# 3ickey/ConsensusML

Measured on AMD Instinct MI355X. Metric: samples/sec ResNet-50 + Krum at 1/2/4/8 MI355X; agg overhead vs all-reduce, higher is better.
Workload: dtype bf16

## Files before the change

### consensusml_amd/models/resnet.py

```python
from __future__ import annotations

from typing import List, Optional

import torch
import torch.nn as nn
import torch.nn.functional as F

from ..ops import conv as fconv
from ..ops.bn import BatchNormAct2d, ResidualLink, bn_add_bn_relu, fused_ok, link_tap
from ..ops.pool import bn_relu_max_pool2d, max_pool2d
from ..ops.stem import stem_conv_bn_relu_pool, stem_ok

from ..perf import policy as _P


def recompute_tail_policy(planes: int) -> bool:
    p = _P()
    return (p.recompute_tail and planes <= p.recompute_tail_max_planes
            and fconv.recompute_tail_ok(planes))


def fused_bn3_bwd_policy(planes: int) -> bool:
    from ..ops import conv as _c
    p = _P()
    return p.fused_bn3_bwd and planes <= p.fused_bn3_bwd_max_planes and _c.res_tail_ok(planes)


def fused_conv1x1_policy(cin: int, cout: int, hw_out: int, stride: int, prologue: bool) -> bool:
    if not _P().fused_conv1x1:
        return False
    if prologue:
        return True
    return hw_out >= 784


def conv1x1_policy(cin: int, cout: int, hw: int):
    mode = _P().conv1x1_gemm
    if mode is True or mode == "gemm":
        return True, True
    if mode is False or mode == "miopen":
        return False, False
    if cin == 64 and cout == 64 and _P().c1_dgrad64_gemm:
        return False, True
    return cin >= 1024, (cout < cin) or hw <= 196


class _Conv1x1Fn(torch.autograd.Function):

    @staticmethod
    def forward(ctx, x, w, link, fwd_gemm, dgrad_gemm, own_wgrad=False):
        ctx.save_for_backward(x, w)
        ctx.link = link
        ctx.wt = fconv.cached_wt(w)
        ctx.dgrad_gemm = dgrad_gemm
        ctx.own_wgrad = own_wgrad
        N, C, H, W = x.shape
        if fwd_gemm:
            y = fconv.conv_mm(x.permute(0, 2, 3, 1).reshape(N * H * W, C), w.reshape(w.shape[0], C))
            return y.view(N, H, W, w.shape[0]).permute(0, 3, 1, 2)
        return F.conv2d(x, w)

    @staticmethod
    def backward(ctx, dy):
        x, w = ctx.saved_tensors
        dy = dy.contiguous(memory_format=torch.channels_last)
        N, C, H, W = x.shape
        Co = w.shape[0]
        need_dx = ctx.needs_input_grad[0]
        mio_dx = need_dx and not ctx.dgrad_gemm
        own_dw = ctx.own_wgrad and ctx.needs_input_grad[1]
        mio_dw = ctx.needs_input_grad[1] and not own_dw
        dx_m, dw, h = None, None, None
        if own_dw:
            from ..ops.native import lib
            dw, h = fconv._wgrad_fork(lambda d, a, b: lib().wgrad1x1(d, a, b.dtype).view_as(b),
                                      dy, x, w, conv1x1=True)
        if mio_dx or mio_dw:
            dx_m, dw_m, _ = torch.ops.aten.convolution_backward(
                dy, x, w, None, [1, 1], [0, 0], [1, 1], False, [0, 0], 1,
                [mio_dx, mio_dw, False])
            if mio_dw:
                dw = dw_m
        dx = dx_m if mio_dx else None
        if need_dx and ctx.dgrad_gemm:
            dy2 = dy.permute(0, 2, 3, 1).reshape(N * H * W, Co)
            w2 = w.reshape(Co, C)
            link = ctx.link
            g = link.take() if link is not None else None
            if isinstance(g, fconv.MaskedGrad):
                dx = fconv.masked_link_dgrad(dy, w, g, link, ctx.wt)
                return dx, fconv._wgrad_join(dw, h), None, None, None, None
            if isinstance(g, fconv.S2Grad):
                g = g.materialize()
            w_nk = fconv.dgrad_wnk(dy2, w2, ctx.wt)
            if g is not None:
                dres = g.permute(0, 2, 3, 1).reshape(N * H * W, C) if g.dim() == 4 else g
                if dres.data_ptr() == g.data_ptr() and dres.is_contiguous():
                    d2 = fconv.conv_mm(dy2, w_nk, acc=dres)
                else:
                    d2 = torch.addmm(dres, dy2, w2)
            else:
                d2 = fconv.conv_mm(dy2, w_nk)
            dx = d2.view(N, H, W, C).permute(0, 3, 1, 2)
        return dx, fconv._wgrad_join(dw, h), None, None, None, None


_CORE = {(128, 512), (512, 128), (256, 1024), (512, 2048), (2048, 512)}
_ALL = _CORE | {(256, 128), (512, 256), (1024, 256), (1024, 512)}
_WIDE = _ALL | {(1024, 2048)}
_SETS = {"core": _CORE, "all": _ALL, "wide": _WIDE}


def own_wgrad_ok(cin: int, cout: int) -> bool:
    p = _P()
    return p.own_wgrad1x1 and (cin, cout) in _SETS[p.wgrad1x1_set]


class Conv1x1(nn.Conv2d):

    def __init__(self, cin: int, cout: int, stride: int = 1):
        super().__init__(cin, cout, 1, stride=stride, bias=False)

    def _policy(self, x: torch.Tensor):
        if not (self.stride == (1, 1) and x.is_cuda and x.dim() == 4
                and x.is_contiguous(memory_format=torch.channels_last)):
            return False, False
        return conv1x1_policy(self.in_channels, self.out_channels, x.shape[2] * x.shape[3])

    def link_ok(self, x: torch.Tensor) -> bool:
        return self._policy(x)[1]

    def forward(self, x: torch.Tensor, res_link: Optional[ResidualLink] = None) -> torch.Tensor:
        fwd_gemm, dgrad_gemm = self._policy(x)
        own = (self.stride == (1, 1) and x.is_cuda and x.dtype == torch.bfloat16
               and self.weight.dtype in (torch.bfloat16, torch.float32)
               and x.is_contiguous(memory_format=torch.channels_last)
               and own_wgrad_ok(self.in_channels, self.out_channels))
        if fwd_gemm or dgrad_gemm or own:
            return _Conv1x1Fn.apply(x, self.weight, res_link if dgrad_gemm else None, fwd_gemm,
                                    dgrad_gemm, own)
        return super().forward(x)


class _GlobalAvgPoolFn(torch.autograd.Function):

    @staticmethod
    def forward(ctx, x):
        ctx.shape = x.shape
        return torch.flatten(F.adaptive_avg_pool2d(x, 1), 1)

    @staticmethod
    def backward(ctx, g):
        N, C, H, W = ctx.shape
        if g.is_cuda and g.dtype == torch.bfloat16 and C % 8 == 0:
            from ..ops.native import lib
            return lib().avgpool_bwd(g, H, W)
        gs = (g.float() / (H * W)).to(g.dtype).contiguous()
        return torch.cat([gs] * (H * W), dim=1).view(N, H, W, C).permute(0, 3, 1, 2)


def global_avg_pool(x: torch.Tensor) -> torch.Tensor:
    if _P().nhwc_avgpool and x.is_cuda and x.dim() == 4 \
            and x.is_contiguous(memory_format=torch.channels_last):
        return _GlobalAvgPoolFn.apply(x)
    return torch.flatten(F.adaptive_avg_pool2d(x, 1), 1)


class Bottleneck(nn.Module):
    expansion = 4

    def __init__(self, inplanes: int, planes: int, stride: int = 1, downsample: bool = False):
        super().__init__()
        self.conv1 = Conv1x1(inplanes, planes)
        self.bn1 = BatchNormAct2d(planes, relu=True)
        self.conv2 = nn.Conv2d(planes, planes, 3, stride=stride, padding=1, bias=False)
        self.bn2 = BatchNormAct2d(planes, relu=True)
        self.conv3 = Conv1x1(planes, planes * 4)
        self.bn3 = BatchNormAct2d(planes * 4, relu=True)
        if downsample:
            self.down_conv = Conv1x1(inplanes, planes * 4, stride=stride)
            self.down_bn = BatchNormAct2d(planes * 4, relu=False)
        else:
            self.down_conv = None

    def _conv2(self, x: torch.Tensor) -> torch.Tensor:
        if _P().own_dgrad3x3 and self.training:
            return fconv.conv3x3(x, self.conv2)
        return self.conv2(x)

    def _down_s2_compact_ok(self, x: torch.Tensor, dlink) -> bool:
        c = self.down_conv
        return (dlink is not None and _P().down_s2_compact and c.stride == (2, 2)
                and x.is_cuda and x.dtype == torch.bfloat16 and x.shape[1] % 8 == 0
                and x.shape[2] % 2 == 0 and x.shape[3] % 2 == 0
                and x.is_contiguous(memory_format=torch.channels_last))

    def _down_conv_s2_compact(self, x: torch.Tensor, dlink) -> torch.Tensor:
        c = self.down_conv
        xs = fconv.subsample2_link(x, dlink)
        fwd, dg = conv1x1_policy(c.in_channels, c.out_channels, xs.shape[2] * xs.shape[3])
        return _Conv1x1Fn.apply(xs, c.weight, None, fwd, dg,
                                own_wgrad_ok(c.in_channels, c.out_channels))

    def _fused_ok(self, x: torch.Tensor) -> bool:
        return (_P().fused_conv1x1 and self.training and torch.is_grad_enabled()
                and fconv.fused_conv_ok(x, self.conv1.weight)
                and fused_ok(x, self.bn3.weight))

    def _conv_bn(self, x, conv: "Conv1x1", bn, link=None):
        st = conv.stride[0]
        hw = (x.shape[2] // st) * (x.shape[3] // st)
        if fused_conv1x1_policy(conv.in_channels, conv.out_channels, hw, st, False):
            dg = st == 1 and conv1x1_policy(conv.in_channels, conv.out_channels, hw)[1]
            own = own_wgrad_ok(conv.in_channels, conv.out_channels) if st == 1 else True
            z, m, i = fconv.conv1x1_bn_stats(x, conv, bn, st, dg, own, link if dg else None)
            return z, (m, i)
        if st == 1:
            return conv(x, res_link=link if conv.link_ok(x) else None), None
        return conv(x), None

    def _tap(self, x: torch.Tensor, dlink, use_links: bool) -> torch.Tensor:
        tlink = dlink if dlink is not None else \
            (getattr(x, "_cml_pool_link", None) if use_links else None)
        return link_tap(x, tlink) if tlink is not None else x

    def _head(self, x: torch.Tensor, use_links: bool):
        link = dlink = None
        if self.down_conv is None:
            link = getattr(x, "_cml_link", None) if use_links else None
        elif use_links and self.conv1.link_ok(x):
            dlink = ResidualLink()
        z1, st1 = self._conv_bn(x, self.conv1, self.bn1, link if dlink is None else dlink)
        return z1, st1, link, dlink

    def _conv2_fused(self, z1: torch.Tensor, st1, fuse3: bool):
        pol = _P()
        s1 = self.conv2.stride == (1, 1)
        on = (pol.conv3x3_bn_stats and pol.own_dgrad3x3) if s1 else pol.own_conv3x3_s2
        own3 = fuse3 and on and fconv.conv3x3_ok(z1, self.conv2)
        pro = (own3 and pol.bn1_dgrad_sums and self.bn1.training
               and fused_ok(z1, self.bn1.weight))
        if pro and s1 and st1 is None and pol.bn1_sums_lib_conv1:
            st1 = fconv.bn_stats(z1, self.bn1)
        if pro and st1 is not None:
            return fconv.bnrelu_conv3x3_bn_stats(z1, self.bn1, st1, self.conv2, self.bn2)
        out = self.bn1(z1, stats=st1)
        if own3:
            return fconv.conv3x3_bn_stats(out, self.conv2, self.bn2)
        z2 = self._conv2(out)
        return z2, (fconv.bn_stats(z2, self.bn2) if fuse3 else None)

    def _tail_fused(self, x, z2, st2, fuse3: bool, hw2: int, link, dlink, use_links: bool,
                    out_link) -> torch.Tensor:
        planes = self.conv3.in_channels
        down = self.down_conv
        if not fuse3:
            z, st3 = self.conv3(self.bn2(z2)), None
        else:
            if down is None:
                rec = recompute_tail_policy(planes)
                if rec or fused_bn3_bwd_policy(planes):
                    tail = fconv.bnrelu_conv1x1_bn_res_recompute if rec \
                        else fconv.bnrelu_conv1x1_bn_res
                    return tail(z2, self.bn2, st2, self.conv3, self.bn3, x, link, out_link)
            elif _P().recompute_down_tail and self.bn3.eps == self.down_bn.eps:
                xd = None
                if fconv.down_tail_recompute_s2_ok(x, planes, down):
                    xd = fconv.subsample2_link(x, dlink)
                elif fconv.down_tail_recompute_ok(x, planes, down):
                    xd = self._tap(x, dlink, use_links)
                if xd is not None:
                    return fconv.down_tail_recompute(z2, self.bn2, st2, self.conv3, self.bn3, xd,
                                                     down, self.down_bn, out_link)
            dg = conv1x1_policy(planes, planes * 4, hw2)[1]
            z, m3, i3 = fconv.bnrelu_conv1x1_bn_stats(z2, self.bn2, st2, self.conv3, self.bn3, dg,
                                                      own_wgrad_ok(planes, planes * 4)
                                                      or planes == 64)
            st3 = (m3, i3)
        if down is None:
            return self.bn3(z, residual=x, res_link=link, out_link=out_link, stats=st3)
        if self._down_s2_compact_ok(x, dlink):
            zd, std = self._down_conv_s2_compact(x, dlink), None
        else:
            zd, std = self._conv_bn(self._tap(x, dlink, use_links), down, self.down_bn)
        if (st3 is None) != (std is None):
            return self.bn3(z, residual=self.down_bn(zd, stats=std), out_link=out_link, stats=st3)
        stats = None if st3 is None else st3 + std
        return bn_add_bn_relu(z, self.bn3, zd, self.down_bn, out_link, stats=stats)

    def _forward_fused(self, x: torch.Tensor, use_links: bool) -> torch.Tensor:
        z1, st1, link, dlink = self._head(x, use_links)
        planes, s = self.conv3.in_channels, self.conv2.stride[0]
        hw2 = (z1.shape[2] // s) * (z1.shape[3] // s)
        fuse3 = fused_conv1x1_policy(planes, planes * 4, hw2, 1, True)
        z2, st2 = self._conv2_fused(z1, st1, fuse3)
        out_link = ResidualLink() if use_links else None
        y = self._tail_fused(x, z2, st2, fuse3, hw2, link, dlink, use_links, out_link)
        if out_link is not None:
            y._cml_link = out_link
        return y

    def forward(self, x: torch.Tensor) -> torch.Tensor:
        use_links = _P().residual_link and torch.is_grad_enabled() and self.training
        if self._fused_ok(x):
            return self._forward_fused(x, use_links)
        if self.down_conv is None:
            link = getattr(x, "_cml_link", None) if use_links else None
            out = self.bn1(self.conv1(x, res_link=link if self.conv1.link_ok(x) else None))
            out = self.bn2(self._conv2(out))
            z = self.conv3(out)
            fused = fused_ok(z, self.bn3.weight)
            out_link = ResidualLink() if use_links and fused else None
            y = self.bn3(z, residual=x, res_link=link if fused else None, out_link=out_link)
        else:
            dlink = ResidualLink() if use_links and self.conv1.link_ok(x) else None
            out = self.bn1(self.conv1(x, res_link=dlink))
            out = self.bn2(self._conv2(out))
            z = self.conv3(out)
            zd = self.down_conv(self._tap(x, dlink, use_links))
            out_link = ResidualLink() if use_links and fused_ok(z, self.bn3.weight) else None
            y = bn_add_bn_relu(z, self.bn3, zd, self.down_bn, out_link) if _P().fuse_down_bn \
                else self.bn3(z, residual=self.down_bn(zd), out_link=out_link)
        if out_link is not None:
            y._cml_link = out_link
        return y


class ResNet(nn.Module):
    def __init__(self, layers: List[int], num_classes: int = 1000, width: int = 64):
        super().__init__()
        self.inplanes = width
        self.conv1 = nn.Conv2d(3, width, 7, stride=2, padding=3, bias=False)
        self.bn1 = BatchNormAct2d(width, relu=True)
        self.layer1 = self._make(width, layers[0], 1)
        self.layer2 = self._make(width * 2, layers[1], 2)
        self.layer3 = self._make(width * 4, layers[2], 2)
        self.layer4 = self._make(width * 8, layers[3], 2)
        self.fc = nn.Linear(width * 8 * 4, num_classes)
        for m in self.modules():
            if isinstance(m, nn.Conv2d):
                nn.init.kaiming_normal_(m.weight, mode="fan_out", nonlinearity="relu")
        for m in self.modules():
            if isinstance(m, Bottleneck):
                nn.init.zeros_(m.bn3.weight)

    def stem(self, x: torch.Tensor) -> torch.Tensor:
        w = self.conv1.weight
        if (_P().stem_pad4 and x.is_cuda and x.dtype == torch.bfloat16 and x.shape[1] == 3
                and x.is_contiguous(memory_format=torch.channels_last) and not x.requires_grad):
            from ..ops.native import lib
            x4 = lib().pad_c4(x)
            w4 = F.pad(w, (0, 0, 0, 0, 0, 1)).contiguous(memory_format=torch.channels_last)
            return F.conv2d(x4, w4, stride=2, padding=3)
        return self.conv1(x)

    def _make(self, planes: int, blocks: int, stride: int) -> nn.Sequential:
        down = stride != 1 or self.inplanes != planes * 4
        mods = [Bottleneck(self.inplanes, planes, stride, down)]
        self.inplanes = planes * 4
        mods += [Bottleneck(self.inplanes, planes) for _ in range(1, blocks)]
        return nn.Sequential(*mods)

    def forward(self, x: torch.Tensor) -> torch.Tensor:
        pol = _P()
        if pol.fuse_stem_conv and stem_ok(x, self.conv1, self.bn1):
            plink = ResidualLink() if (pol.pool_link and pol.residual_link and self.training
                                       and torch.is_grad_enabled()) else None
            x = stem_conv_bn_relu_pool(x, self.conv1, self.bn1, plink)
            if plink is not None:
                x._cml_pool_link = plink
        elif pol.fuse_stem_pool:
            x = bn_relu_max_pool2d(self.stem(x), self.bn1, 3, 2, 1)
        else:
            x = max_pool2d(self.bn1(self.stem(x)), 3, 2, 1)
        blocks = [b for layer in (self.layer1, self.layer2, self.layer3, self.layer4)
                  for b in layer]
        ws = [b.conv2.weight for b in blocks] + [b.conv1.weight for b in blocks]
        batched = (pol.batch_wlayouts and self.training and torch.is_grad_enabled()
                   and not fconv.params_pending(self, ws) and fconv.prefetch_wlayouts(ws))
        try:
            x = self.layer4(self.layer3(self.layer2(self.layer1(x))))
        finally:
            if batched:
                fconv.clear_wlayouts()
        return self.fc(global_avg_pool(x))


def resnet50(num_classes: int = 1000) -> ResNet:
    return ResNet([3, 4, 6, 3], num_classes)


def resnet_tiny(num_classes: int = 10) -> ResNet:
    return ResNet([1, 1, 1, 1], num_classes, width=8)
```

### consensusml_amd/ops/bn.py

```python
from __future__ import annotations

from typing import Optional

import torch
import torch.nn as nn
import torch.nn.functional as F

from ..perf import policy as _P
from .native import lib


class ResidualLink:
    __slots__ = ("grad", "closed", "bn_ctx", "sums")

    def __init__(self):
        self.grad = None
        self.closed = False
        self.bn_ctx = None
        self.sums = None

    def take(self):
        g, self.grad = self.grad, None
        self.closed = True
        return g

    def take_tensor(self):
        g = self.take()
        return g.materialize() if hasattr(g, "materialize") else g


class MaskedGrad:
    __slots__ = ("g", "mask")

    def __init__(self, g: torch.Tensor, mask: torch.Tensor):
        self.g = g
        self.mask = mask

    def materialize(self) -> torch.Tensor:
        g = self.g
        N, C, H, W = g.shape
        shifts = torch.arange(8, device=g.device, dtype=torch.uint8)
        bits = (self.mask.view(-1, C // 8, 1) >> shifts) & 1
        rows = g.permute(0, 2, 3, 1).reshape(-1, C) * bits.view(-1, C).to(g.dtype)
        return rows.view(N, H, W, C).permute(0, 3, 1, 2)


TAP_STATS = {"parked": 0, "fallback": 0}


class _LinkTapFn(torch.autograd.Function):

    @staticmethod
    def forward(ctx, x, link):
        ctx.link = link
        return x.view_as(x)

    @staticmethod
    def backward(ctx, g):
        link = ctx.link
        if link.closed or link.grad is not None:
            TAP_STATS["fallback"] += 1
            return g, None
        TAP_STATS["parked"] += 1
        link.grad = g.contiguous(memory_format=torch.channels_last) if g.dim() == 4 else g.contiguous()
        return None, None


def link_tap(x: torch.Tensor, link: "ResidualLink") -> torch.Tensor:
    return _LinkTapFn.apply(x, link)


class _BNActFn(torch.autograd.Function):
    @staticmethod
    def forward(ctx, x, gamma, beta, res, rmean, rvar, mean_in, invstd_in, eps, momentum, relu,
                training, res_link, out_link):
        has_res = res is not None
        want_mask = has_res and relu and any(ctx.needs_input_grad[:4])
        y, mean, invstd, mask = lib().bn_fwd(x, res, gamma, beta, rmean, rvar, mean_in,
                                             invstd_in, eps, momentum, relu, training, want_mask)
        ctx.save_for_backward(x, mask if want_mask else None, gamma, beta, mean, invstd)
        ctx.relu = relu
        ctx.has_res = has_res
        ctx.res_link = res_link
        ctx.out_link = out_link
        return y

    @staticmethod
    def backward(ctx, dy):
        x, mask, gamma, beta, mean, invstd = ctx.saved_tensors
        dy2 = ctx.out_link.take_tensor() if ctx.out_link is not None else None
        dx, dg, db, dres = lib().bn_bwd(dy, dy2, x, mask, gamma, beta, mean, invstd, ctx.relu,
                                        ctx.has_res)
        if ctx.has_res and ctx.res_link is not None:
            ctx.res_link.grad = dres
            dres = None
        return (dx, dg, db, dres if ctx.has_res else None, None, None, None, None, None, None,
                None, None, None, None)


class _BNAddBNActFn(torch.autograd.Function):

    @staticmethod
    def forward(ctx, x1, g1, b1, x2, g2, b2, rm1, rv1, rm2, rv2, stats_in, eps, momentum,
                training, out_link):
        want_mask = any(ctx.needs_input_grad[:6])
        m1 = i1 = m2 = i2 = None
        if not training:
            m1, i1, m2, i2 = stats_in
        y, m1, i1, m2, i2, mask = lib().bn_fwd2(x1, x2, g1, b1, g2, b2, rm1, rv1, rm2, rv2, m1,
                                                i1, m2, i2, eps, momentum, training, want_mask)
        ctx.save_for_backward(x1, x2, mask if want_mask else None, g1, g2, m1, i1, m2, i2)
        ctx.out_link = out_link
        return y

    @staticmethod
    def backward(ctx, dy):
        x1, x2, mask, g1, g2, m1, i1, m2, i2 = ctx.saved_tensors
        dy2 = ctx.out_link.take_tensor() if ctx.out_link is not None else None
        dx1, dg1, db1, dx2, dg2, db2 = lib().bn_bwd2(dy, dy2, x1, x2, mask, g1, g2, m1, i1, m2, i2)
        return (dx1, dg1, db1, dx2, dg2, db2) + (None,) * 9


def bn_add_bn_relu(x1: torch.Tensor, bn1: "BatchNormAct2d", x2: torch.Tensor,
                   bn2: "BatchNormAct2d", out_link: Optional[ResidualLink] = None,
                   stats: Optional[tuple] = None) -> torch.Tensor:
    if (_fused_ok(x1, bn1.weight) and _fused_ok(x2, bn2.weight) and x1.shape == x2.shape
            and not bn2.relu and bn1.relu and bn1.eps == bn2.eps and bn1.momentum == bn2.momentum):
        if stats is not None and bn1.training:
            return _BNAddBNActFn.apply(x1, bn1.weight, bn1.bias, x2, bn2.weight, bn2.bias, None,
                                       None, None, None, tuple(stats), bn1.eps, bn1.momentum,
                                       False, out_link)
        stats = None
        if not bn1.training:
            stats = (bn1.running_mean.float(), torch.rsqrt(bn1.running_var.float() + bn1.eps),
                     bn2.running_mean.float(), torch.rsqrt(bn2.running_var.float() + bn2.eps))
        return _BNAddBNActFn.apply(x1, bn1.weight, bn1.bias, x2, bn2.weight, bn2.bias,
                                   bn1.running_mean if bn1.training else None,
                                   bn1.running_var if bn1.training else None,
                                   bn2.running_mean if bn2.training else None,
                                   bn2.running_var if bn2.training else None, stats, bn1.eps,
                                   bn1.momentum, bn1.training, out_link)
    return bn1(x1, residual=bn2(x2), out_link=out_link)


def fused_ok(x: torch.Tensor, gamma: torch.Tensor) -> bool:
    return _fused_ok(x, gamma)


def _fused_ok(x: torch.Tensor, gamma: torch.Tensor) -> bool:
    if not (x.is_cuda and x.dtype == torch.bfloat16 and gamma.dtype == torch.bfloat16):
        return False
    if not _P().fused_bn:
        return False
    C = x.shape[1]
    if C % 8 or C > 2048 or 256 % (C // 8):
        return False
    return x.dim() == 4 and x.is_contiguous(memory_format=torch.channels_last)


def bn_act(x: torch.Tensor, gamma: torch.Tensor, beta: torch.Tensor,
           running_mean: Optional[torch.Tensor], running_var: Optional[torch.Tensor],
           residual: Optional[torch.Tensor] = None, relu: bool = True, training: bool = True,
           momentum: float = 0.1, eps: float = 1e-5,
           res_link: Optional[ResidualLink] = None,
           out_link: Optional[ResidualLink] = None,
           stats: Optional[tuple] = None) -> torch.Tensor:
    if _fused_ok(x, gamma) and (residual is None or residual.is_contiguous(
            memory_format=torch.channels_last)):
        if training and stats is not None:
            return _BNActFn.apply(x, gamma, beta, residual, None, None, stats[0], stats[1], eps,
                                  momentum, relu, False, res_link, out_link)
        if training:
            return _BNActFn.apply(x, gamma, beta, residual, running_mean, running_var, None, None,
                                  eps, momentum, relu, True, res_link, out_link)
        invstd = torch.rsqrt(running_var.float() + eps)
        return _BNActFn.apply(x, gamma, beta, residual, None, None, running_mean.float(), invstd,
                              eps, momentum, relu, False, res_link, out_link)
    y = F.batch_norm(x, running_mean, running_var, gamma, beta, training, momentum, eps) \
        if running_mean is None or running_mean.dtype == x.dtype else \
        _bn_mixed(x, gamma, beta, running_mean, running_var, training, momentum, eps)
    if residual is not None:
# ... 42 lines not shown
```

### consensusml_amd/ops/conv.py

```python
from __future__ import annotations

import weakref
from typing import Optional, Tuple, Dict

import torch
import torch.nn.functional as F

from ..perf import policy as _P
from .bn import MaskedGrad
from .native import lib


def fused_conv_ok(x: torch.Tensor, w: torch.Tensor) -> bool:
    return (x.is_cuda and x.dtype == torch.bfloat16 and w.dtype == torch.bfloat16 and x.dim() == 4
            and x.is_contiguous(memory_format=torch.channels_last) and x.shape[1] % 64 == 0
            and w.shape[0] % 64 == 0 and w.shape[2] == 1 and w.shape[3] == 1)


def _nt_tile(a: torch.Tensor, M: int, N: int, K: int) -> int:
    if not (_P().own_gemm_conv1x1 and a.is_cuda and a.dtype == torch.bfloat16):
        return 0
    try:
        t = int(lib().gemm_nt_pick(M, N, K))
    except Exception:
        return 0
    if t == 256:
        return 256 if (M // 256) * (N // 256) >= 128 else 0
    return 128 if t == 128 and _P().own_gemm128 else 0


CONV_MM_STATS = {"own": 0, "own128": 0, "blas": 0}


def dgrad_wnk(a: torch.Tensor, w2: torch.Tensor, wt: Optional[torch.Tensor]) -> torch.Tensor:
    if wt is not None and _nt_tile(a, a.shape[0], w2.shape[1], w2.shape[0]):
        return wt
    return w2.t()


def conv_mm(a: torch.Tensor, w_nk: torch.Tensor, acc: Optional[torch.Tensor] = None) -> torch.Tensor:
    M, K = a.shape
    N = w_nk.shape[0]
    tile = _nt_tile(a, M, N, K)
    if (tile and a.is_contiguous() and a.data_ptr() % 16 == 0
            and (acc is None or (acc.is_contiguous() and acc.data_ptr() % 16 == 0))):
        w = (lib().transpose_bf16(w_nk.t()) if (w_nk.stride(0) == 1 and w_nk.dim() == 2)
             else w_nk.contiguous())
        CONV_MM_STATS["own"] += 1
        if tile == 128:
            CONV_MM_STATS["own128"] += 1
        if acc is not None:
            return lib().gemm_nt(a, w, 0, out=acc, cin=acc, tile=tile)
        return lib().gemm_nt(a, w, 0, tile=tile)
    CONV_MM_STATS["blas"] += 1
    if acc is not None:
        return acc.addmm_(a, w_nk.t()) if acc.is_contiguous() else torch.addmm(acc, a, w_nk.t())
    return torch.mm(a, w_nk.t())


def _dgrad(dy: torch.Tensor, x: torch.Tensor, w: torch.Tensor, stride: int, gemm: bool,
           link, wt: Optional[torch.Tensor] = None) -> torch.Tensor:
    N, C, H, W = x.shape
    Co = w.shape[0]
    if gemm and stride == 1:
        dy2 = dy.permute(0, 2, 3, 1).reshape(N * H * W, Co)
        w2 = w.reshape(Co, C)
        g = link.take() if link is not None else None
        if isinstance(g, MaskedGrad):
            return masked_link_dgrad(dy, w, g, link, wt)
        if isinstance(g, S2Grad):
            if (_P().s2_link_dgrad and dy.dtype == torch.bfloat16 and C % 64 == 0 and Co % 64 == 0
                    and g.H == H and g.W == W):
                if wt is None:
                    wt = w.reshape(Co, C).t().contiguous()
                return lib().conv1x1_link_s2(dy.contiguous(memory_format=torch.channels_last), wt,
                                             g.g)
            g = g.materialize()
        w_nk = dgrad_wnk(dy2, w2, wt)
        if (g is not None and g.dim() == 4 and _P().link_dgrad_plain and dy.dtype == torch.bfloat16
                and g.dtype == torch.bfloat16 and C % 64 == 0 and Co % 64 == 0
                and g.is_contiguous(memory_format=torch.channels_last)
                and not _nt_tile(dy2, N * H * W, C, Co)):
            wt2 = wt if wt is not None else w2.t().contiguous()
            return lib().conv1x1_link(dy.contiguous(memory_format=torch.channels_last), wt2, g,
                                      None)[0]
        if g is not None:
            dres = g.permute(0, 2, 3, 1).reshape(N * H * W, C) if g.dim() == 4 else g
            if dres.data_ptr() == g.data_ptr() and dres.is_contiguous():
                d2 = conv_mm(dy2, w_nk, acc=dres)
            else:
                d2 = torch.addmm(dres, dy2, w2)
        else:
            d2 = conv_mm(dy2, w_nk)
        return d2.view(N, H, W, C).permute(0, 3, 1, 2)
    dx, _, _ = torch.ops.aten.convolution_backward(
        dy, x, w, None, [stride, stride], [0, 0], [1, 1], False, [0, 0], 1, [True, False, False])
    return dx


def masked_link_dgrad(dy: torch.Tensor, w: torch.Tensor, mg: MaskedGrad, link,
                      wt: Optional[torch.Tensor] = None) -> torch.Tensor:
    Co, Ci = w.shape[0], w.shape[1]
    if wt is None:
        wt = w.reshape(Co, Ci).t().contiguous()
    bctx = link.bn_ctx if link is not None else None
    if bctx is not None:
        z, mask, mean, invstd = bctx
        dx, sdz, sdzx = lib().conv1x1_link(dy, wt, mg.g, mg.mask, z, mask, mean, invstd)
        link.sums = (sdz, sdzx, dx.data_ptr())
        return dx
    return lib().conv1x1_link(dy, wt, mg.g, mg.mask)[0]


def _wgrad(dy: torch.Tensor, x: torch.Tensor, w: torch.Tensor, stride: int, own: bool,
           pro: Optional[Tuple[torch.Tensor, torch.Tensor]] = None) -> torch.Tensor:
    if own and stride == 1:
        sc, bi = pro if pro is not None else (None, None)
        return lib().wgrad1x1(dy, x, w.dtype, sc, bi).view_as(w)
    if pro is not None:
        sc, bi = pro
        x = torch.relu(x.float() * sc.view(1, -1, 1, 1) + bi.view(1, -1, 1, 1)).to(x.dtype)
        x = x.contiguous(memory_format=torch.channels_last)
    N, Ci, H, W = x.shape
    if (own and stride == 2 and _P().own_wgrad1x1_s2 and x.is_cuda
            and dy.dtype == torch.bfloat16 and x.dtype == torch.bfloat16
            and x.is_contiguous(memory_format=torch.channels_last)
            and lib().wgrad3x3s2_ok(N, H, W, dy.shape[1], Ci, 1)):
        return lib().wgrad3x3s2(dy, x, w.dtype, _zero_row(dy.device), taps=1).reshape(w.shape)
    _, dw, _ = torch.ops.aten.convolution_backward(
        dy, x, w, None, [stride, stride], [0, 0], [1, 1], False, [0, 0], 1, [False, True, False])
    return dw


class _Conv1x1BNStatsFn(torch.autograd.Function):
    @staticmethod
    def forward(ctx, x, w, rmean, rvar, stride, eps, momentum, dgrad_gemm, own_wgrad, link,
                aff=None):
        out = lib().conv1x1_bn_fwd(x, w, None, None, rmean, rmean, rvar, stride, True, eps,
                                   momentum, *(aff or (None, None)))
        y, mean, invstd = out[:3]
        if aff is not None:
            _stash_affine(mean, out[3], out[4], aff)
        ctx.wt = cached_wt(w)
        ctx.save_for_backward(x, w)
        ctx.stride, ctx.dgrad_gemm, ctx.own_wgrad, ctx.link = stride, dgrad_gemm, own_wgrad, link
        ctx.mark_non_differentiable(mean, invstd)
        ctx.set_materialize_grads(False)
        return y, mean, invstd

    @staticmethod
    def backward(ctx, dy, _dm, _di):
        x, w = ctx.saved_tensors
        dy = dy.contiguous(memory_format=torch.channels_last)
        dw, h = _wgrad_fork(lambda d, a, b: _wgrad(d, a, b, ctx.stride, ctx.own_wgrad), dy, x, w,
                            conv1x1=True) if ctx.needs_input_grad[1] else (None, None)
        dx = _dgrad(dy, x, w, ctx.stride, ctx.dgrad_gemm, ctx.link, ctx.wt) \
            if ctx.needs_input_grad[0] else None
        dw = _wgrad_join(dw, h)
        return dx, dw, None, None, None, None, None, None, None, None, None


class _BNReLUConv1x1BNStatsFn(torch.autograd.Function):

    @staticmethod
    def forward(ctx, z, gamma, beta, mean, invstd, w, rmean, rvar, eps, momentum, dgrad_gemm,
                own_wgrad):
        sc, bi = _affine(gamma, beta, mean, invstd)
        y, m3, i3 = lib().conv1x1_bn_fwd(z, w, sc, bi, rmean, rmean, rvar, 1, True, eps, momentum)
        ctx.save_for_backward(z, gamma, beta, mean, invstd, w, sc, bi)
        ctx.dgrad_gemm, ctx.own_wgrad = dgrad_gemm, own_wgrad
        ctx.mark_non_differentiable(m3, i3)
        ctx.set_materialize_grads(False)
        return y, m3, i3

    @staticmethod
    def backward(ctx, dz3, _dm, _di):
        z, gamma, beta, mean, invstd, w, sc, bi = ctx.saved_tensors
        dz3 = dz3.contiguous(memory_format=torch.channels_last)
        dw = _wgrad(dz3, z, w, 1, ctx.own_wgrad, (sc, bi)) if ctx.needs_input_grad[5] else None
        dy2 = _dgrad(dz3, z, w, 1, ctx.dgrad_gemm, None)
        dz, dg, db, _ = lib().bn_bwd(dy2, None, z, None, gamma, beta, mean, invstd, True, False)
        return dz, dg, db, None, None, dw, None, None, None, None, None, None


def _take_out_link(ol, gy: torch.Tensor):
    gy = gy.contiguous(memory_format=torch.channels_last)
    sums = None
    if ol is not None:
        extra = ol.take_tensor()
        if ol.sums is not None and extra is None and ol.sums[2] == gy.data_ptr():
            sums = ol.sums
        ol.sums = ol.bn_ctx = None
        if extra is not None:
            gy = (gy + extra).contiguous(memory_format=torch.channels_last)
    return gy, sums


def _park_masked(gy: torch.Tensor, mask: torch.Tensor, res_link) -> Optional[torch.Tensor]:
    mg = MaskedGrad(gy, mask)
    if res_link is not None and not res_link.closed and res_link.grad is None:
        res_link.grad = mg
        return None
    return mg.materialize()


class _BNReLUConv1x1BNResFn(torch.autograd.Function):

    @staticmethod
    def forward(ctx, z, g2, b2, mean2, invstd2, w, g3, b3, res, rmean3, rvar3, eps, momentum,
                res_link, out_link):
        sc, bi = _affine(g2, b2, mean2, invstd2)
        z3, m3, i3 = lib().conv1x1_bn_fwd(z, w, sc, bi, rmean3, rmean3, rvar3, 1, True, eps,
                                          momentum)
        y, _, _, mask = lib().bn_fwd(z3, res, g3, b3, None, None, m3, i3, eps, momentum, True,
                                     False, True)
        ctx.save_for_backward(z, g2, b2, mean2, invstd2, w, sc, bi, z3, mask, g3, b3, m3, i3)
        ctx.res_link, ctx.out_link = res_link, out_link
        if out_link is not None:
            out_link.bn_ctx = (z3, mask, m3, i3)
        return y

    @staticmethod
    def backward(ctx, gy):
        z, g2, b2, mean2, invstd2, w, sc, bi, z3, mask, g3, b3, m3, i3 = ctx.saved_tensors
        gy, sums = _take_out_link(ctx.out_link, gy)
        M = gy.numel() // gy.shape[1]
        if sums is None:
            sums = lib().bn_bwd_sums(gy, None, z3, mask, g3, b3, m3, i3, True)
        ca, cb, cc, dg3, db3 = lib().bn_bwd_coeffs(sums[0], sums[1], g3, m3, i3, M)
        Co, Ci = w.shape[0], w.shape[1]
        dw = None
        if ctx.needs_input_grad[5]:
            dw = lib().wgrad1x1(gy, z, w.dtype, sc, bi, z3, mask, ca, cb, cc).view_as(w)
        dy2 = lib().conv1x1_bnbwd(gy, z3, mask, ca, cb, cc, w.reshape(Co, Ci).t().contiguous())
        dz, dg2, db2, _ = lib().bn_bwd(dy2, None, z, None, g2, b2, mean2, invstd2, True, False)
        dres = _park_masked(gy, mask, ctx.res_link) if ctx.needs_input_grad[8] else None
        return (dz, dg2, db2, None, None, dw, dg3, db3, dres) + (None,) * 6


def _fin_aff(bn):
    g, b = bn.weight, bn.bias
    if (_P().fin_affine and _P().bn_affine_kernel and g is not None and b is not None
            and g.dtype == torch.bfloat16 and b.dtype == torch.bfloat16
            and g.is_contiguous() and b.is_contiguous()):
        return g, b
    return None


def _stash_affine(mean: torch.Tensor, sc: torch.Tensor, bi: torch.Tensor, aff) -> None:
    g, b = aff
    mean._cml_affine = (sc, bi, g.data_ptr(), b.data_ptr(), g._version, b._version)


def _cached_affine(gamma: torch.Tensor, beta: torch.Tensor, mean: torch.Tensor):
    a = getattr(mean, "_cml_affine", None)
    if (a is not None and a[2] == gamma.data_ptr() and a[3] == beta.data_ptr()
            and a[4] == gamma._version and a[5] == beta._version):
        return a[0], a[1]
    return None


def _affine(gamma: torch.Tensor, beta: torch.Tensor, mean: torch.Tensor, invstd: torch.Tensor):
    a = _cached_affine(gamma, beta, mean)
    if a is not None:
        return a
    if not _P().bn_affine_kernel:
        sc = gamma.float() * invstd
        return sc, beta.float() - mean * sc
    ab = lib().bn_affine(gamma, beta, mean, invstd)
    return ab[0], ab[1]


def _stats_gram_affine(L, gram, cy, w, M, rmean, rvar, eps, momentum, gamma, beta):
    if _P().bn_affine_kernel:
        m, i, sc, bi = L.bn_stats_gram(gram, cy, w, M, rmean, rvar, eps, momentum, gamma, beta)
        return m, i, sc, bi
    m, i = L.bn_stats_gram(gram, cy, w, M, rmean, rvar, eps, momentum)
    return (m, i) + _affine(gamma, beta, m, i)


_CONST = {}


def _const(n: int, v: float, device) -> torch.Tensor:
    key = (n, v, device)
    t = _CONST.get(key)
    if t is None:
        t = _CONST[key] = torch.full((n,), v, dtype=torch.float32, device=device)
    return t




def scaled_cat(w1: torch.Tensor, s1: torch.Tensor, w2: torch.Tensor, s2: torch.Tensor):
    k1 = w1.shape[1]
    out = torch.empty(w1.shape[0], k1 + w2.shape[1], dtype=torch.bfloat16, device=w1.device)
    torch.mul(w1, s1[:, None], out=out[:, :k1])
    torch.mul(w2, s2[:, None], out=out[:, k1:])
    return out


def fold_cat(w1: torch.Tensor, a: torch.Tensor, c: torch.Tensor, w2: torch.Tensor):
    w_cat = torch.cat([w1 * a[None, :], w2], 1).to(torch.bfloat16).contiguous()
    return w_cat, torch.mv(w1, c)


def _own_dgb(gamma: torch.Tensor, beta: torch.Tensor) -> bool:
    return (_P().fin_dgamma and gamma.dtype == torch.bfloat16 and beta.dtype == torch.bfloat16
            and gamma.is_contiguous() and beta.is_contiguous())


def _cat_dgrad_bn2(L, gy, mask, z, sc, bi, w_cat, bias, g2, b2, mean2, invstd2):
# ... 244 lines not shown
_ZERO_ROWS = {}


def _zero_row(device: torch.device) -> torch.Tensor:
    z = _ZERO_ROWS.get(device)
    if z is None:
        z = _ZERO_ROWS[device] = torch.zeros(256, dtype=torch.bfloat16, device=device)
    return z


_SIDE_STREAMS: Dict[torch.device, "torch.cuda.Stream"] = {}


def _wgrad_fork(fn, *args, conv1x1: bool = False):
    dev = args[0].device
    pol = _P()
    if not (pol.side_wgrad and dev.type == "cuda" and args[0].shape[0] >= pol.side_wgrad_min_batch
            and (pol.side_wgrad_1x1 or not conv1x1)):
        return fn(*args), None
    side = _SIDE_STREAMS.get(dev)
    if side is None:
        side = _SIDE_STREAMS[dev] = torch.cuda.Stream(device=dev)
    main = torch.cuda.current_stream(dev)
    side.wait_stream(main)
    with torch.cuda.stream(side):
        dw = fn(*args)
    return dw, (main, side)


def _wgrad_join(dw: Optional[torch.Tensor], handle) -> Optional[torch.Tensor]:
    if handle is None:
        return dw
    main, side = handle
    main.wait_stream(side)
    if dw is not None:
        dw.record_stream(main)
    return dw




def _wgrad3x3(dy: torch.Tensor, x: torch.Tensor, w: torch.Tensor) -> torch.Tensor:
    N, Ci, H, W = x.shape
    Co = dy.shape[1]
    if _P().own_wgrad3x3 and lib().wgrad3x3_direct_ok(N, H, W, Co, Ci):
        return lib().wgrad3x3(dy, x, w.dtype, _zero_row(dy.device))
    return torch.ops.aten.convolution_backward(
        dy, x, w, None, [1, 1], [1, 1], [1, 1], False, [0, 0], 1, [False, True, False])[1]


_WL_BATCH = {}


def prefetch_wlayouts(ws) -> bool:
    ws = [w for w in ws if w.is_cuda and w.dtype == torch.bfloat16 and w.dim() == 4
          and w.shape[2] == w.shape[3] and w.shape[2] in (1, 3)]
    if len(ws) < 2:
        return False
    for w, (wf, wr) in zip(ws, lib().conv_wlayouts_multi(ws)):
        _WL_BATCH[id(w)] = (w, wf, wr)
    return True


def clear_wlayouts() -> None:
    _WL_BATCH.clear()


_PENDING_QUERY = weakref.WeakKeyDictionary()


def set_pending_query(model: torch.nn.Module, query) -> None:
    if query is None:
        _PENDING_QUERY.pop(model, None)
    else:
        _PENDING_QUERY[model] = weakref.WeakMethod(query)


def params_pending(model: torch.nn.Module, params) -> bool:
    ref = _PENDING_QUERY.get(model)
    query = ref() if ref is not None else None
    return query is not None and query(params)


def cached_wt(w: torch.Tensor) -> Optional[torch.Tensor]:
    e = _WL_BATCH.get(id(w))
    return e[2] if e is not None and e[0] is w and w.shape[2] == 1 else None


def _w3x3_layouts(w: torch.Tensor, want_wf: bool):
    e = _WL_BATCH.get(id(w))
    if e is not None and e[0] is w:
        return (e[1] if want_wf else None), e[2]
    if w.is_cuda and w.dtype == torch.bfloat16:
        wf, wr = lib().conv3x3_wlayouts(w, want_wf)
        return wf, wr
    Co, Ci = w.shape[0], w.shape[1]
    wf = w.permute(0, 2, 3, 1).reshape(Co, 9 * Ci).contiguous() if want_wf else None
    return wf, w.flip(2, 3).permute(1, 2, 3, 0).reshape(Ci, 9 * Co).contiguous()


class _Conv3x3Fn(torch.autograd.Function):

    @staticmethod
    def forward(ctx, x, w):
        ctx.save_for_backward(x, w)
        return F.conv2d(x, w, padding=1)

    @staticmethod
    def backward(ctx, dy):
        x, w = ctx.saved_tensors
        dy = dy.contiguous(memory_format=torch.channels_last)
        dgrad, wgrad = _BWD3X3[getattr(ctx, "stride", 1)]
        dx = dw = None
        if ctx.needs_input_grad[0]:
            wr = getattr(ctx, "wr", None)
            if wr is None:
                wr = _w3x3_layouts(w, False)[1]
            dx = dgrad(dy, wr)[0]
        if ctx.needs_input_grad[1]:
            dw = wgrad(dy, x, w)
        return dx, dw


class _Conv3x3BNStatsFn(torch.autograd.Function):

    @staticmethod
    def forward(ctx, x, w, rmean, rvar, eps, momentum, stride=1, aff=None):
        wf, wr = _w3x3_layouts(w, True)
        y, mean, invstd = _conv_gemm_bn(x, wf, rmean, rvar, eps, momentum, stride, aff)
        ctx.save_for_backward(x, w)
        ctx.wr, ctx.stride = wr, stride
        ctx.mark_non_differentiable(mean, invstd)
        ctx.set_materialize_grads(False)
        return y, mean, invstd

    @staticmethod
    def backward(ctx, dy, _dm, _di):
        dx, dw = _Conv3x3Fn.backward(ctx, dy)
        return dx, dw, None, None, None, None, None, None


def _conv_gemm_bn(x, wf, rmean, rvar, eps, momentum, stride, aff):
    out = lib().conv_gemm_bn(x, wf, 9, _zero_row(x.device), rmean, rmean, rvar, eps, momentum,
                             stride, *(aff or (None, None)))
    if aff is not None:
        _stash_affine(out[1], out[3], out[4], aff)
    return out[0], out[1], out[2]


class _BNReLUConv3x3BNStatsFn(torch.autograd.Function):

    @staticmethod
    def forward(ctx, z1, g1, b1, mean1, invstd1, eps1, w, rmean, rvar, eps, momentum, stride=1,
                aff=None):
        L = lib()
        y1 = L.bn_fwd(z1, None, g1, b1, None, None, mean1, invstd1, eps1, momentum, True, False,
                      False)[0]
        wf, wr = _w3x3_layouts(w, True)
        z2, m2, i2 = _conv_gemm_bn(y1, wf, rmean, rvar, eps, momentum, stride, aff)
        ctx.save_for_backward(z1, g1, b1, mean1, invstd1, y1, w)
        ctx.wr, ctx.stride = wr, stride
        ctx.aff1 = _cached_affine(g1, b1, mean1)
        ctx.mark_non_differentiable(m2, i2)
        ctx.set_materialize_grads(False)
        return z2, m2, i2

    @staticmethod
    def backward(ctx, dz2, _dm, _di):
        z1, g1, b1, mean1, invstd1, y1, w = ctx.saved_tensors
        dz2 = dz2.contiguous(memory_format=torch.channels_last)
        L = lib()
        dgrad, wgrad = _BWD3X3[ctx.stride]
        dw, h = _wgrad_fork(wgrad, dz2, y1, w) if ctx.needs_input_grad[6] else (None, None)
        sc, bi = ctx.aff1 or _affine(g1, b1, mean1, invstd1)
        bn1 = (z1, sc, bi, mean1, invstd1)
        if _own_dgb(g1, b1):
            dg1, db1 = torch.empty_like(g1), torch.empty_like(b1)
            dy1, s1, q1 = dgrad(dz2, ctx.wr, *bn1, dg1, db1)
        else:
            dy1, s1, q1 = dgrad(dz2, ctx.wr, *bn1)
            M = z1.numel() // z1.shape[1]
            _, _, _, dg1, db1 = L.bn_bwd_coeffs(s1, q1, g1, mean1, invstd1, M)
        dz1 = L.bn_bwd_apply(dy1, z1, g1, b1, mean1, invstd1, s1, q1)
        dw = _wgrad_join(dw, h)
        return dz1, dg1, db1, None, None, None, dw, None, None, None, None, None, None


def _wgrad3x3_s2(dy: torch.Tensor, x: torch.Tensor, w: torch.Tensor) -> torch.Tensor:
    N, Ci, H, W = x.shape
    if (_P().own_wgrad3x3_s2 and Ci >= _P().wgrad3x3_s2_min_ci and x.is_cuda
            and dy.dtype == torch.bfloat16
            and x.dtype == torch.bfloat16
            and lib().wgrad3x3s2_ok(N, H, W, dy.shape[1], Ci)):
        return lib().wgrad3x3s2(dy, x.contiguous(memory_format=torch.channels_last), w.dtype,
                                _zero_row(dy.device))
    return torch.ops.aten.convolution_backward(
        dy, x, w, None, [2, 2], [1, 1], [1, 1], False, [0, 0], 1, [False, True, False])[1]


def _dgrad3x3(dy: torch.Tensor, wr: torch.Tensor, *bn):
    if bn:
        return lib().conv_gemm_bnsums(dy, wr, 9, _zero_row(dy.device), *bn)
    return (lib().conv_gemm(dy, wr, 9, _zero_row(dy.device)),)


def _dgrad3x3_s2(dy: torch.Tensor, wr: torch.Tensor, *bn):
    return lib().conv_gemm_s2dgrad(dy, wr, _zero_row(dy.device), *bn)


_BWD3X3 = {1: (_dgrad3x3, _wgrad3x3), 2: (_dgrad3x3_s2, _wgrad3x3_s2)}




def bnrelu_conv3x3_bn_stats(z1: torch.Tensor, bn_a, stats_a, conv, bn):
    z, m, i = _BNReLUConv3x3BNStatsFn.apply(z1, bn_a.weight, bn_a.bias, stats_a[0], stats_a[1],
                                            bn_a.eps, conv.weight, bn.running_mean, bn.running_var,
                                            bn.eps, bn.momentum, conv.stride[0], _fin_aff(bn))
    return z, (m, i)


def conv3x3_bn_stats(x: torch.Tensor, conv, bn):
    z, m, i = _Conv3x3BNStatsFn.apply(x, conv.weight, bn.running_mean, bn.running_var, bn.eps,
                                      bn.momentum, conv.stride[0], _fin_aff(bn))
    return z, (m, i)


def conv3x3_ok(x: torch.Tensor, conv) -> bool:
    return (x.is_cuda and x.dtype == torch.bfloat16 and conv.weight.dtype == torch.bfloat16
            and x.dim() == 4 and x.is_contiguous(memory_format=torch.channels_last)
            and conv.kernel_size == (3, 3) and conv.padding == (1, 1)
            and (conv.stride == (1, 1) or (conv.stride == (2, 2) and x.shape[2] % 2 == 0
                                           and x.shape[3] % 2 == 0))
            and conv.dilation == (1, 1) and conv.groups == 1 and conv.bias is None
            and conv.in_channels % 64 == 0 and conv.out_channels % 64 == 0)


def conv3x3(x: torch.Tensor, conv) -> torch.Tensor:
    if conv.stride == (1, 1) and conv3x3_ok(x, conv) and torch.is_grad_enabled():
        return _Conv3x3Fn.apply(x, conv.weight)
    return conv(x)


def conv1x1_bn_stats(x: torch.Tensor, conv, bn, stride: int = 1, dgrad_gemm: bool = False,
                     own_wgrad: bool = False, link=None):
    return _Conv1x1BNStatsFn.apply(x, conv.weight, bn.running_mean, bn.running_var, stride,
                                   bn.eps, bn.momentum, dgrad_gemm, own_wgrad, link, _fin_aff(bn))


def bnrelu_conv1x1_bn_stats(z: torch.Tensor, bn_a, stats_a, conv, bn_b, dgrad_gemm: bool = False,
                            own_wgrad: bool = True):
    mean, invstd = stats_a
    return _BNReLUConv1x1BNStatsFn.apply(z, bn_a.weight, bn_a.bias, mean, invstd, conv.weight,
                                         bn_b.running_mean, bn_b.running_var, bn_b.eps,
                                         bn_b.momentum, dgrad_gemm, own_wgrad)


def bn_stats(z: torch.Tensor, bn) -> Tuple[torch.Tensor, torch.Tensor]:
    return tuple(lib().bn_stats(z, bn.running_mean, bn.running_var, bn.eps, bn.momentum))


def reference_conv1x1_bn(x: torch.Tensor, w: torch.Tensor, stride: int = 1,
                         pro: Optional[Tuple[torch.Tensor, torch.Tensor]] = None):
    xf = x.float()
    if pro is not None:
        xf = torch.relu(xf * pro[0].view(1, -1, 1, 1) + pro[1].view(1, -1, 1, 1))
        xf = xf.to(torch.bfloat16).float()
    y = F.conv2d(xf, w.float(), stride=stride)
    yb = y.to(torch.bfloat16).float()
    return y, yb.mean((0, 2, 3)), yb.var((0, 2, 3), unbiased=False)
```

### consensusml_amd/perf.py

```python
from __future__ import annotations

import contextlib
import dataclasses
import os
from dataclasses import dataclass, fields
from typing import Any, Dict, Iterator


def _env_bool(name: str, default: bool) -> bool:
    v = os.environ.get(name)
    return default if v is None else v == "1"


def _env_int(name: str, default: int) -> int:
    v = os.environ.get(name)
    return default if v is None else int(v)


def _env_str(name: str, default: str) -> str:
    return os.environ.get(name, default)


@dataclass
class PerfPolicy:
    fused_bn: bool = True
    residual_link: bool = True
    fuse_stem_conv: bool = True
    fuse_stem_pool: bool = True
    pool_link: bool = True
    stem_pool_gather: bool = True
    stem_pad4: bool = True
    nhwc_avgpool: bool = True
    conv1x1_gemm: str = "auto"
    fused_conv1x1: bool = True
    conv1x1g: str = "auto"
    own_wgrad1x1: bool = True
    wgrad1x1_set: str = "wide"
    fused_bn3_bwd: bool = True
    fused_bn3_bwd_max_planes: int = 128
    recompute_tail: bool = True
    recompute_tail_max_planes: int = 256
    recompute_down_tail: bool = True
    recompute_down_tail_s2: bool = True
    down_tail_s2_max_cin: int = 512
    fuse_down_bn: bool = True
    gram_stats: bool = True
    cat_bnsums: bool = True
    cat_bnsums_maxc: int = 256
    s2_link_dgrad: bool = True
    down_s2_compact: bool = True
    bn_affine_kernel: bool = True
    own_dgrad3x3: bool = True
    conv3x3_bn_stats: bool = True
    bn1_dgrad_sums: bool = True
    bn1_sums_lib_conv1: bool = False
    own_wgrad3x3: bool = True
    own_wgrad3x3_s2: bool = True
    wgrad3x3_s2_min_ci: int = 256
    own_wgrad1x1_s2: bool = True
    c1_dgrad64_gemm: bool = True
    own_conv3x3_s2: bool = True
    side_wgrad: bool = True
    side_wgrad_min_batch: int = 1024
    link_dgrad_plain: bool = True
    side_wgrad_1x1: bool = False
    fin_dgamma: bool = True
    fin_affine: bool = True
    batch_wlayouts: bool = True
    attn_kernel: bool = True
    flash_attn: bool = True
    multi_copy: bool = True
    batched_workers: bool = True
    own_gemm: bool = True
    own_gemm128: bool = True
    fused_ffn: bool = True
    padded_logits: bool = True
    own_gemm_conv1x1: bool = True
    nt_wgrad: bool = True
    own_linear_wgrad: bool = True

    @classmethod
    def from_env(cls) -> "PerfPolicy":
        return cls(
            fused_bn=_env_bool("CML_FUSED_BN", True),
            fuse_stem_conv=_env_bool("CML_FUSE_STEM_CONV", True),
            fuse_stem_pool=_env_bool("CML_FUSE_STEM_POOL", True),
            pool_link=_env_bool("CML_POOL_LINK", True),
            stem_pool_gather=_env_bool("CML_STEM_POOL_GATHER", True),
            stem_pad4=_env_bool("CML_STEM_PAD4", True),
            nhwc_avgpool=_env_bool("CML_NHWC_AVGPOOL", True),
            conv1x1_gemm=_env_str("CML_CONV1X1_GEMM", "auto"),
            fused_conv1x1=_env_bool("CML_FUSED_CONV1X1", True),
            conv1x1g={"0": "regstage", "3": "quad"}.get(os.environ.get("CML_C1G", ""), "auto"),
            own_wgrad1x1=_env_bool("CML_WGRAD1X1", True),
            wgrad1x1_set=_env_str("CML_WGRAD1X1_SET", "wide"),
            fused_bn3_bwd=_env_bool("CML_FUSED_BN3_BWD", True),
            fused_bn3_bwd_max_planes=_env_int("CML_FUSED_BN3_BWD_MAX_PLANES", 128),
            recompute_tail=_env_bool("CML_RECOMPUTE_TAIL", True),
            recompute_tail_max_planes=_env_int("CML_RECOMPUTE_TAIL_MAX_PLANES", 256),
            recompute_down_tail=_env_bool("CML_RECOMPUTE_DOWN_TAIL", True),
            recompute_down_tail_s2=_env_bool("CML_RECOMPUTE_DOWN_TAIL_S2", True),
            down_tail_s2_max_cin=_env_int("CML_DOWN_TAIL_S2_MAX_CIN", 512),
            fuse_down_bn=_env_bool("CML_FUSE_DOWN_BN", True),
            gram_stats=_env_bool("CML_GRAM_STATS", True),
            cat_bnsums=_env_bool("CML_CAT_BNSUMS", True),
            cat_bnsums_maxc=_env_int("CML_CAT_BNSUMS_MAXC", 256),
            s2_link_dgrad=_env_bool("CML_S2_LINK_DGRAD", True),
            down_s2_compact=_env_bool("CML_DOWN_S2_COMPACT", True),
            bn_affine_kernel=_env_bool("CML_BN_AFFINE_KERNEL", True),
            own_dgrad3x3=_env_bool("CML_DGRAD3X3", True),
            conv3x3_bn_stats=_env_bool("CML_CONV3X3_BN_STATS", True),
            bn1_dgrad_sums=_env_bool("CML_BN1_DGRAD_SUMS", True),
            bn1_sums_lib_conv1=_env_bool("CML_BN1_SUMS_LIB_CONV1", False),
            own_wgrad3x3=_env_bool("CML_WGRAD3X3", True),
            own_wgrad3x3_s2=_env_bool("CML_WGRAD3X3_S2", True),
            wgrad3x3_s2_min_ci=int(os.environ.get("CML_WGRAD3X3_S2_MIN_CI", "256")),
            own_wgrad1x1_s2=_env_bool("CML_WGRAD1X1_S2", True),
            c1_dgrad64_gemm=_env_bool("CML_C1_DGRAD64", True),
            own_conv3x3_s2=_env_bool("CML_CONV3X3_S2", True),
            side_wgrad=_env_bool("CML_SIDE_WGRAD", True),
            side_wgrad_min_batch=_env_int("CML_SIDE_WGRAD_MIN_BATCH", 1024),
            side_wgrad_1x1=_env_bool("CML_SIDE_WGRAD_1X1", False),
            link_dgrad_plain=_env_bool("CML_LINK_DGRAD_PLAIN", True),
            fin_dgamma=_env_bool("CML_FIN_DGAMMA", True),
            fin_affine=_env_bool("CML_FIN_AFFINE", True),
            batch_wlayouts=_env_bool("CML_BATCH_WLAYOUTS", True),
            attn_kernel=_env_bool("CML_ATTN_KERNEL", True),
            flash_attn=_env_bool("CML_FLASH_ATTN", True),
            multi_copy=_env_bool("CML_MULTI_COPY", True),
            batched_workers=_env_bool("CML_BATCHED_WORKERS", True),
            own_gemm=_env_bool("CML_OWN_GEMM", True),
            own_gemm128=_env_bool("CML_OWN_GEMM128", True),
            fused_ffn=_env_bool("CML_FUSED_FFN", True),
            own_gemm_conv1x1=_env_bool("CML_OWN_GEMM_CONV1X1", True),
            own_linear_wgrad=_env_bool("CML_OWN_LINEAR_WGRAD", True),
            nt_wgrad=_env_bool("CML_NT_WGRAD", True),
            padded_logits=_env_bool("CML_PADDED_LOGITS", True),
        )

    @classmethod
    def library(cls) -> "PerfPolicy":
        off: Dict[str, Any] = {}
        for f in fields(cls):
            if f.type in ("bool", bool):
                off[f.name] = False
        off.update(conv1x1_gemm="miopen", conv1x1g="regstage")
        return cls(**off)

    def replace(self, **kw) -> "PerfPolicy":
        return dataclasses.replace(self, **kw)

    def to_dict(self) -> Dict[str, Any]:
        return dataclasses.asdict(self)

    def validate(self) -> "PerfPolicy":
        if self.conv1x1_gemm not in ("auto", "gemm", "miopen"):
            raise ValueError(f"conv1x1_gemm must be auto | gemm | miopen, not {self.conv1x1_gemm!r}")
        if self.conv1x1g not in ("auto", "quad", "regstage"):
            raise ValueError(f"conv1x1g must be auto | quad | regstage, not "
                             f"{self.conv1x1g!r}")
        if self.wgrad1x1_set not in ("core", "all", "wide"):
            raise ValueError(f"wgrad1x1_set must be core | all | wide, not "
                             f"{self.wgrad1x1_set!r}")
        return self


_CURRENT = PerfPolicy.from_env().validate()
_NATIVE_SYNCED = None


def env_switches() -> Dict[str, str]:
    return {k: v for k, v in sorted(os.environ.items())
            if k.startswith("CML_") and not k.startswith("CML_BENCH_")}


def policy() -> PerfPolicy:
    return _CURRENT


def _sync_native(p: PerfPolicy) -> None:
    global _NATIVE_SYNCED
    mode = {"regstage": 0, "auto": 2, "quad": 3}[p.conv1x1g]
    if _NATIVE_SYNCED == mode:
        return
    try:
        from .ops.native import lib
        L = lib()
    except Exception:
        return
    L.set_conv1x1g_mode(mode)
    _NATIVE_SYNCED = mode


def set_policy(p: PerfPolicy) -> PerfPolicy:
    global _CURRENT
    prev = _CURRENT
    _CURRENT = p.validate()
    if prev.conv1x1g != p.conv1x1g or _NATIVE_SYNCED is not None:
        _sync_native(p)
    return prev


def ensure_native_synced() -> None:
    _sync_native(_CURRENT)


@contextlib.contextmanager
def use_policy(p: PerfPolicy) -> Iterator[PerfPolicy]:
    prev = set_policy(p)
    try:
        yield p
    finally:
        set_policy(prev)
```

### csrc/bindings.cpp

```cpp
#include <torch/extension.h>
#include <array>
#include <climits>
#include <ATen/hip/HIPContext.h>
#include <c10/core/DeviceGuard.h>

#include "kernels/kernels.h"

namespace {

using at::Tensor;
using c10::optional;

#define CML_CHECK_HIP(expr)                                                               \
  do {                                                                                    \
    hipError_t _e = (expr);                                                               \
    TORCH_CHECK(_e == hipSuccess, "consensusml_amd HIP error: ", hipGetErrorString(_e), " at " \
                #expr " (bindings.cpp:", __LINE__, ")");                                  \
  } while (0)

hipStream_t cur_stream() { return c10::hip::getCurrentHIPStream().stream(); }

int dtype_of(const Tensor& t) {
  if (t.scalar_type() == at::kBFloat16) return cml::DT_BF16;
  TORCH_CHECK(t.scalar_type() == at::kFloat, "expected bf16 or fp32 tensor, got ", t.scalar_type());
// ... 1093 lines not shown
                              M, static_cast<int>(K), static_cast<int>(Co), pro))}, f32);
  CML_CHECK_HIP(cml::launch_conv1x1_bn_fwd(
      x.data_ptr(), w.data_ptr(), nullptr, part.data_ptr<float>(),
      opt_ptr<const float>(pro_sc, at::kFloat, "pro_sc", K),
      opt_ptr<const float>(pro_bi, at::kFloat, "pro_bi", K),
      opt_ptr<const float>(shift, at::kFloat, "shift", Co), M, static_cast<int>(K),
      static_cast<int>(Co), 1, 0, 0, mean.data_ptr<float>(), invstd.data_ptr<float>(),
      opt_ptr<float>(rmean, at::kFloat, "running_mean", Co),
      opt_ptr<float>(rvar, at::kFloat, "running_var", Co), static_cast<float>(eps),
      static_cast<float>(momentum), cur_stream()));
  return {mean, invstd};
}

std::vector<Tensor> conv1x1_bnres(const Tensor& x, const Tensor& w, const Tensor& pro_sc,
                                  const Tensor& pro_bi, const Tensor& ep_sc, const Tensor& ep_bi,
                                  const Tensor& res) {
  check_nhwc(x, "x");
  check_nhwc(res, "res");
  TORCH_CHECK(x.dim() == 4 && w.scalar_type() == at::kBFloat16 && w.dim() == 4 && w.size(2) == 1 &&
                  w.size(3) == 1 && w.size(1) == x.size(1) && w.is_contiguous(),
              "conv1x1_bnres: x NHWC, w contiguous bf16 [Cout, Cin, 1, 1]");
  const int64_t N = x.size(0), K = x.size(1), H = x.size(2), W = x.size(3), Co = w.size(0);
  const int64_t M = N * H * W;
  TORCH_CHECK(res.dim() == 4 && res.size(0) == N && res.size(1) == Co && res.size(2) == H &&
                  res.size(3) == W, "conv1x1_bnres: res shape");
  TORCH_CHECK(K % 64 == 0 && Co % 64 == 0, "conv1x1_bnres: channels multiples of 64");
  const c10::DeviceGuard guard(x.device());
  Tensor y = at::empty({N, Co, H, W}, x.options().memory_format(at::MemoryFormat::ChannelsLast));
  Tensor mask = at::empty({M, Co / 8}, x.options().dtype(at::kByte));
  CML_CHECK_HIP(cml::launch_conv1x1_bnres(
      x.data_ptr(), w.data_ptr(), y.data_ptr(), mask.data_ptr<uint8_t>(),
      opt_ptr<const float>(pro_sc, at::kFloat, "pro_sc", K),
      opt_ptr<const float>(pro_bi, at::kFloat, "pro_bi", K),
      opt_ptr<const float>(ep_sc, at::kFloat, "ep_sc", Co),
      opt_ptr<const float>(ep_bi, at::kFloat, "ep_bi", Co), res.data_ptr(), M,
      static_cast<int>(K), static_cast<int>(Co), cur_stream()));
  return {y, mask};
}

namespace {
std::array<int64_t, 8> cat_shape(const Tensor& x1, const Tensor& x2, const Tensor& w,
                                 const char* what) {
  check_nhwc(x1, "x1");
  check_nhwc(x2, "x2");
  const int64_t N = x1.size(0), K1 = x1.size(1), H = x1.size(2), W = x1.size(3), K2 = x2.size(1);
  TORCH_CHECK(x2.dim() == 4 && x2.size(0) == N && x2.size(2) == H && x2.size(3) == W, what,
              ": x2 shape");
  TORCH_CHECK(w.is_cuda() && w.scalar_type() == at::kBFloat16 && w.dim() == 2 &&
                  w.size(1) == K1 + K2 && w.is_contiguous() && w.size(0) % 64 == 0 &&
                  K1 % 64 == 0 && K2 % 64 == 0,
              what, ": w contiguous bf16 [Cout, K1 + K2], channels multiples of 64");
  return {N, K1, H, W, K2, N * H * W, K1 + K2, w.size(0)};
}
}

std::vector<Tensor> conv1x1_cat_bnres(const Tensor& x1, const Tensor& x2, const Tensor& sc1,
                                      const Tensor& bi1, const optional<Tensor>& sc2,
                                      const optional<Tensor>& bi2, const Tensor& w,
                                      const Tensor& ep_sc, const Tensor& ep_bi) {
  const auto [N, K1, H, W, K2, M, K, Co] = cat_shape(x1, x2, w, "conv1x1_cat_bnres");
  const c10::DeviceGuard guard(x1.device());
  Tensor y = at::empty({N, Co, H, W}, x1.options().memory_format(at::MemoryFormat::ChannelsLast));
  Tensor mask = at::empty({M, Co / 8}, x1.options().dtype(at::kByte));
  CML_CHECK_HIP(cml::launch_conv1x1_cat_bnres(
      x1.data_ptr(), x2.data_ptr(), opt_ptr<const float>(sc1, at::kFloat, "sc1", K1),
      opt_ptr<const float>(bi1, at::kFloat, "bi1", K1),
      opt_ptr<const float>(sc2, at::kFloat, "sc2", K2),
      opt_ptr<const float>(bi2, at::kFloat, "bi2", K2), w.data_ptr(),
      opt_ptr<const float>(ep_sc, at::kFloat, "ep_sc", Co),
      opt_ptr<const float>(ep_bi, at::kFloat, "ep_bi", Co), nullptr, y.data_ptr(),
      mask.data_ptr<uint8_t>(), M, static_cast<int>(K1), static_cast<int>(K),
      static_cast<int>(Co), cur_stream()));
  return {y, mask};
}

Tensor conv1x1_cat(const Tensor& g, const Tensor& mask, const Tensor& x2,
                   const optional<Tensor>& sc2, const optional<Tensor>& bi2, const Tensor& w,
                   const optional<Tensor>& bias) {
  const auto [N, K1, H, W, K2, M, K, Co] = cat_shape(g, x2, w, "conv1x1_cat");
  const c10::DeviceGuard guard(g.device());
  Tensor y = at::empty({N, Co, H, W}, g.options().memory_format(at::MemoryFormat::ChannelsLast));
  CML_CHECK_HIP(cml::launch_conv1x1_cat(
      g.data_ptr(), opt_ptr<const uint8_t>(mask, at::kByte, "mask", M * K1 / 8), x2.data_ptr(),
      opt_ptr<const float>(sc2, at::kFloat, "sc2", K2),
      opt_ptr<const float>(bi2, at::kFloat, "bi2", K2),
      opt_ptr<const float>(bias, at::kFloat, "bias", Co), w.data_ptr(), y.data_ptr(), M,
      static_cast<int>(K1), static_cast<int>(K), static_cast<int>(Co), cur_stream()));
  return y;
}

std::vector<Tensor> conv1x1_cat_bnsums(const Tensor& g, const Tensor& mask, const Tensor& x2,
                                       const Tensor& sc2, const Tensor& bi2, const Tensor& w,
                                       const optional<Tensor>& bias, const Tensor& mean,
                                       const Tensor& invstd, const optional<Tensor>& dgamma_out,
                                       const optional<Tensor>& dbeta_out) {
  const auto [N, K1, H, W, K2, M, K, Co] = cat_shape(g, x2, w, "conv1x1_cat_bnsums");
  TORCH_CHECK(Co == K2, "conv1x1_cat_bnsums: w must be [K2, K1 + K2]");
  const c10::DeviceGuard guard(g.device());
  auto f32 = g.options().dtype(at::kFloat);
  Tensor y = at::empty({N, Co, H, W}, g.options().memory_format(at::MemoryFormat::ChannelsLast));
  Tensor part = at::empty({static_cast<int64_t>(cml::conv1x1_cat_part_floats(M, K, Co))}, f32);
  Tensor sdz = at::empty({Co}, f32), sdzx = at::empty({Co}, f32);
  const auto [dg, db] = dgb_ptrs(dgamma_out, dbeta_out, Co, g, "conv1x1_cat_bnsums");
  CML_CHECK_HIP(cml::launch_conv1x1_cat(
      g.data_ptr(), opt_ptr<const uint8_t>(mask, at::kByte, "mask", M * K1 / 8), x2.data_ptr(),
      opt_ptr<const float>(sc2, at::kFloat, "sc2", K2),
      opt_ptr<const float>(bi2, at::kFloat, "bi2", K2),
      opt_ptr<const float>(bias, at::kFloat, "bias", Co), w.data_ptr(), y.data_ptr(), M,
      static_cast<int>(K1), static_cast<int>(K), static_cast<int>(Co), cur_stream(),
      opt_ptr<const float>(mean, at::kFloat, "mean", Co),
      opt_ptr<const float>(invstd, at::kFloat, "invstd", Co), part.data_ptr<float>(),
      sdz.data_ptr<float>(), sdzx.data_ptr<float>(), dg, db));
  return {y, sdz, sdzx};
}

Tensor bn_affine(const Tensor& gamma, const Tensor& beta, const Tensor& mean, const Tensor& invstd) {
  const int64_t C = gamma.numel();
  TORCH_CHECK(gamma.scalar_type() == at::kBFloat16 && beta.scalar_type() == at::kBFloat16 &&
                  gamma.is_contiguous() && beta.is_contiguous() && beta.numel() == C && C > 0,
              "bn_affine: contiguous bf16 gamma / beta [C]");
  check_dev(gamma, "gamma");
  check_dev(beta, "beta");
  const c10::DeviceGuard guard(gamma.device());
  Tensor out = at::empty({2, C}, gamma.options().dtype(at::kFloat));
  CML_CHECK_HIP(cml::launch_bn_affine(gamma.data_ptr(), beta.data_ptr(),
                                      opt_ptr<const float>(mean, at::kFloat, "mean", C),
                                      opt_ptr<const float>(invstd, at::kFloat, "invstd", C),
                                      static_cast<int>(C), out.data_ptr<float>(),
                                      out.data_ptr<float>() + C, cur_stream()));
  return out;
}

Tensor bn_bwd_apply(const Tensor& dy_in, const Tensor& x, const Tensor& gamma, const Tensor& beta,
                    const Tensor& mean, const Tensor& invstd, const Tensor& sdz,
                    const Tensor& sdzx) {
  check_nhwc(x, "x");
  Tensor dy = x.dim() == 4 ? dy_in.contiguous(at::MemoryFormat::ChannelsLast) : dy_in.contiguous();
  check_nhwc(dy, "dy");
  TORCH_CHECK(dy.sizes() == x.sizes(), "bn_bwd_apply: dy shape mismatch");
  const int64_t C = x.size(1);
  const int64_t M = x.numel() / C;
  TORCH_CHECK(gamma.scalar_type() == at::kBFloat16 && beta.scalar_type() == at::kBFloat16 &&
                  gamma.numel() == C && beta.numel() == C,
              "bn_bwd_apply: bf16 gamma / beta [C]");
  const c10::DeviceGuard guard(x.device());
  Tensor dx = at::empty_like(x);
  CML_CHECK_HIP(cml::launch_bn_bwd_apply(
      dy.data_ptr(), x.data_ptr(), dx.data_ptr(), M, static_cast<int>(C), gamma.data_ptr(),
      beta.data_ptr(), opt_ptr<const float>(mean, at::kFloat, "mean", C),
      opt_ptr<const float>(invstd, at::kFloat, "invstd", C),
      opt_ptr<const float>(sdz, at::kFloat, "sdz", C),
      opt_ptr<const float>(sdzx, at::kFloat, "sdzx", C), cur_stream()));
  return dx;
}

Tensor conv1x1_link_s2(const Tensor& x, const Tensor& w, const Tensor& link_in) {
  check_nhwc(x, "x");
  TORCH_CHECK(x.dim() == 4, "conv1x1_link_s2: 4-D NHWC input");
  const int64_t N = x.size(0), K = x.size(1), H = x.size(2), W = x.size(3);
  check_w2(w, K, "conv1x1_link_s2");
  const int64_t No = w.size(0);
  Tensor link = link_in.contiguous(at::MemoryFormat::ChannelsLast);
  check_nhwc(link, "link");
  TORCH_CHECK(link.dim() == 4 && link.size(0) == N && link.size(1) == No &&
                  link.size(2) == (H + 1) / 2 && link.size(3) == (W + 1) / 2,
              "conv1x1_link_s2: link [N, No, ceil(H/2), ceil(W/2)]");
  const c10::DeviceGuard guard(x.device());
  Tensor y = at::empty({N, No, H, W}, x.options().memory_format(at::MemoryFormat::ChannelsLast));
  CML_CHECK_HIP(cml::launch_conv1x1_link_s2(x.data_ptr(), w.data_ptr(), y.data_ptr(),
                                            link.data_ptr(), static_cast<int>(N),
                                            static_cast<int>(H), static_cast<int>(W),
                                            static_cast<int>(K), static_cast<int>(No),
                                            cur_stream()));
  return y;
}

Tensor subsample2(const Tensor& x) {
  check_nhwc(x, "x");
  TORCH_CHECK(x.dim() == 4 && x.size(1) % 8 == 0, "subsample2: 4-D NHWC, C % 8 == 0");
  const int64_t N = x.size(0), C = x.size(1), H = x.size(2), W = x.size(3);
  const c10::DeviceGuard guard(x.device());
  Tensor y = at::empty({N, C, (H + 1) / 2, (W + 1) / 2},
                       x.options().memory_format(at::MemoryFormat::ChannelsLast));
  CML_CHECK_HIP(cml::launch_subsample2(x.data_ptr(), y.data_ptr(), static_cast<int>(N),
                                       static_cast<int>(H), static_cast<int>(W),
                                       static_cast<int>(C), cur_stream()));
  return y;
}

Tensor upsample2_scatter(const Tensor& g_in, int64_t H, int64_t W) {
  Tensor g = g_in.contiguous(at::MemoryFormat::ChannelsLast);
  check_nhwc(g, "g");
  const int64_t N = g.size(0), C = g.size(1);
  TORCH_CHECK(g.dim() == 4 && C % 8 == 0 && g.size(2) == (H + 1) / 2 && g.size(3) == (W + 1) / 2,
              "upsample2_scatter: g [N, C, ceil(H/2), ceil(W/2)], C % 8 == 0");
  const c10::DeviceGuard guard(g.device());
  Tensor dx = at::empty({N, C, H, W}, g.options().memory_format(at::MemoryFormat::ChannelsLast));
  CML_CHECK_HIP(cml::launch_upsample2_scatter(g.data_ptr(), dx.data_ptr(), static_cast<int>(N),
                                              static_cast<int>(H), static_cast<int>(W),
                                              static_cast<int>(C), cur_stream()));
  return dx;
}


Tensor wgrad3x3(const Tensor& dy_in, const Tensor& x, at::ScalarType dtype,
                const optional<Tensor>& zero_in) {
  check_nhwc(x, "x");
  Tensor dy = dy_in.contiguous(at::MemoryFormat::ChannelsLast);
  check_nhwc(dy, "dy");
  TORCH_CHECK(x.dim() == 4 && dy.dim() == 4 && dy.size(0) == x.size(0) && dy.size(2) == x.size(2) &&
                  dy.size(3) == x.size(3), "wgrad3x3: dy / x shapes");
  TORCH_CHECK(dtype == at::kBFloat16 || dtype == at::kFloat, "wgrad3x3: bf16 or fp32 output");
  const int64_t N = x.size(0), Ci = x.size(1), H = x.size(2), W = x.size(3), Co = dy.size(1);
  const c10::DeviceGuard guard(x.device());
  int S = 1, T = 0;
  TORCH_CHECK(cml::wgrad3x3_direct_plan(static_cast<int>(N), static_cast<int>(H),
                                        static_cast<int>(W), static_cast<int>(Co),
                                        static_cast<int>(Ci), &S, &T),
              "wgrad3x3: no plan for this shape (check wgrad3x3_direct_ok first)");
  Tensor zero;
  if (zero_in.has_value() && zero_in->defined()) {
    zero = *zero_in;
    TORCH_CHECK(zero.is_cuda() && zero.device() == x.device() && zero.scalar_type() == at::kBFloat16 &&
                    zero.is_contiguous() && zero.numel() >= 8, "wgrad3x3: zero must be >= 8 bf16");
  } else {
    zero = at::zeros({64}, x.options());
  }
  Tensor part = at::empty({S, Co, 9, Ci}, x.options().dtype(at::kFloat));
  Tensor dw = at::empty({Co, 3, 3, Ci}, x.options().dtype(dtype));
  CML_CHECK_HIP(cml::launch_wgrad3x3_direct(dy.data_ptr(), x.data_ptr(), zero.data_ptr(),
                                            part.data_ptr<float>(), dw.data_ptr(),
                                            dtype == at::kBFloat16, static_cast<int>(N),
                                            static_cast<int>(H), static_cast<int>(W),
                                            static_cast<int>(Co), static_cast<int>(Ci),
                                            cur_stream()));
  return dw.permute({0, 3, 1, 2});
}

bool wgrad3x3s2_ok(int64_t N, int64_t H, int64_t W, int64_t Co, int64_t Ci, int64_t taps) {
  int S = 0;
  return N < (1 << 30) && H < (1 << 15) && W < (1 << 15) && Co < (1 << 20) && Ci < (1 << 20) &&
         (taps == 9 || taps == 1) &&
         cml::wgrad3x3s2_plan(static_cast<int>(N), static_cast<int>(H), static_cast<int>(W),
                              static_cast<int>(Co), static_cast<int>(Ci), &S, static_cast<int>(taps));
}

Tensor wgrad3x3s2(const Tensor& dy_in, const Tensor& x, at::ScalarType dtype,
                  const optional<Tensor>& zero_in, int64_t taps) {
  check_nhwc(x, "x");
  Tensor dy = dy_in.contiguous(at::MemoryFormat::ChannelsLast);
  check_nhwc(dy, "dy");
  TORCH_CHECK(x.dim() == 4 && dy.dim() == 4 && dy.size(0) == x.size(0) &&
                  x.size(2) % 2 == 0 && x.size(3) % 2 == 0 && dy.size(2) * 2 == x.size(2) &&
                  dy.size(3) * 2 == x.size(3), "wgrad3x3s2: dy [N, Co, H/2, W/2], x [N, Ci, H, W]");
  TORCH_CHECK(dtype == at::kBFloat16 || dtype == at::kFloat, "wgrad3x3s2: bf16 or fp32 output");
  const int64_t N = x.size(0), Ci = x.size(1), H = x.size(2), W = x.size(3), Co = dy.size(1);
  TORCH_CHECK(wgrad3x3s2_ok(N, H, W, Co, Ci, taps),
              "wgrad3x3s2: no plan for this shape (check wgrad3x3s2_ok first)");
  const c10::DeviceGuard guard(x.device());
  int S = 1;
  cml::wgrad3x3s2_plan(static_cast<int>(N), static_cast<int>(H), static_cast<int>(W),
                       static_cast<int>(Co), static_cast<int>(Ci), &S, static_cast<int>(taps));
  Tensor zero;
  if (zero_in.has_value() && zero_in->defined()) {
    zero = *zero_in;
    TORCH_CHECK(zero.is_cuda() && zero.device() == x.device() && zero.scalar_type() == at::kBFloat16 &&
                    zero.is_contiguous() && zero.numel() >= 256 && zero.data_ptr() != nullptr &&
                    reinterpret_cast<uintptr_t>(zero.data_ptr()) % 16 == 0,
                "wgrad3x3s2: zero must be >= 256 contiguous 16-B aligned bf16");
  } else {
    zero = at::zeros({256}, x.options());
  }
  const int64_t k = taps == 1 ? 1 : 3;
  Tensor part = at::empty({S, Co, taps, Ci}, x.options().dtype(at::kFloat));
  Tensor dw = at::empty({Co, k, k, Ci}, x.options().dtype(dtype));
  CML_CHECK_HIP(cml::launch_wgrad3x3s2(dy.data_ptr(), x.data_ptr(), zero.data_ptr(),
                                       part.data_ptr<float>(), dw.data_ptr(),
                                       dtype == at::kBFloat16, static_cast<int>(N),
                                       static_cast<int>(H), static_cast<int>(W),
                                       static_cast<int>(Co), static_cast<int>(Ci), cur_stream(),
                                       static_cast<int>(taps)));
  return dw.permute({0, 3, 1, 2});
}

std::vector<Tensor> conv3x3_wlayouts(const Tensor& w, bool want_wf) {
  TORCH_CHECK(w.is_cuda() && w.scalar_type() == at::kBFloat16 && w.dim() == 4 && w.size(2) == 3 &&
                  w.size(3) == 3, "conv3x3_wlayouts: bf16 [Co, Ci, 3, 3] CUDA weight");
  const int64_t Co = w.size(0), Ci = w.size(1);
  const c10::DeviceGuard guard(w.device());
  Tensor wr = at::empty({Ci, 9 * Co}, w.options().memory_format(at::MemoryFormat::Contiguous));
  Tensor wf;
  if (want_wf) wf = at::empty({Co, 9 * Ci}, w.options().memory_format(at::MemoryFormat::Contiguous));
  CML_CHECK_HIP(cml::launch_conv3x3_wlayouts(w.data_ptr(), static_cast<int>(Co),
                                             static_cast<int>(Ci), w.stride(0), w.stride(1),
                                             w.stride(2), w.stride(3),
                                             want_wf ? wf.data_ptr() : nullptr, wr.data_ptr(),
                                             cur_stream()));
  return {wf, wr};
}

Tensor avgpool_bwd(const Tensor& g_in, int64_t H, int64_t W) {
  Tensor g = g_in.contiguous();
  TORCH_CHECK(g.is_cuda() && g.scalar_type() == at::kBFloat16 && g.dim() == 2 && g.size(1) % 8 == 0,
              "avgpool_bwd: bf16 [N, C] CUDA gradient, C % 8 == 0");
  const c10::DeviceGuard guard(g.device());
  const int64_t N = g.size(0), C = g.size(1);
// ... 1088 lines not shown
void colsum_seg(const Tensor& x_in, int64_t nseg, Tensor& out) {
  Tensor x = x_in.contiguous();
  check_bf16c(x, "x");
  const int64_t N = x.size(-1);
  const int64_t M = x.numel() / N;
  TORCH_CHECK(out.is_cuda() && out.device() == x.device() && out.scalar_type() == at::kBFloat16 &&
                  out.dim() == 2 && out.size(0) == nseg && out.size(1) == N && out.stride(1) == 1,
              "colsum_seg: out must be bf16 [nseg, N] with unit column stride");
  const c10::DeviceGuard guard(x.device());
  Tensor work = at::empty({static_cast<int64_t>(cml::colsum_workspace_bytes(M, static_cast<int>(N)) / 4 + 1)},
                          x.options().dtype(at::kFloat));
  CML_CHECK_HIP(cml::launch_colsum_seg(x.data_ptr(), M, static_cast<int>(N), static_cast<int>(nseg),
                                       out.data_ptr(), out.stride(0), work.data_ptr(), cur_stream()));
}

Tensor norm_bwd_seg(const Tensor& dy_in, const optional<Tensor>& dres_in, const Tensor& x,
                    const Tensor& w, const optional<Tensor>& mean, const Tensor& rstd,
                    int64_t nseg, Tensor& dw_out, const optional<Tensor>& db_out) {
  check_bf16c(x, "x");
  const int64_t D = x.size(-1);
  const int64_t M = x.numel() / D;
  Tensor dy = dy_in.contiguous();
  check_bf16c(dy, "dy");
  TORCH_CHECK(dy.sizes() == x.sizes(), "dy shape mismatch");
  Tensor dres;
  if (dres_in.has_value() && dres_in->defined()) {
    dres = dres_in->contiguous();
    check_bf16c(dres, "dres");
    TORCH_CHECK(dres.sizes() == x.sizes(), "dres shape mismatch");
  }
  check_bf16c(w, "w");
  const bool ln = mean.has_value() && mean->defined();
  TORCH_CHECK(rstd.is_cuda() && rstd.scalar_type() == at::kFloat && rstd.numel() == M, "rstd: fp32 [M]");
  if (ln) TORCH_CHECK(mean->scalar_type() == at::kFloat && mean->numel() == M, "mean: fp32 [M]");
  TORCH_CHECK(D % 8 == 0 && D <= 4096, "norm: D % 8 == 0 and D <= 4096");
  TORCH_CHECK(nseg >= 1 && M % nseg == 0, "norm_bwd_seg: rows must split into nseg equal segments");
  auto chk = [&](const Tensor& o, const char* nm) {
    TORCH_CHECK(o.is_cuda() && o.device() == x.device() && o.scalar_type() == at::kBFloat16 &&
                    o.dim() == 2 && o.size(0) == nseg && o.size(1) == D && o.stride(1) == 1,
                nm, ": bf16 [nseg, D] with unit column stride");
  };
  chk(dw_out, "dw_out");
  void* dbp = nullptr;
  if (ln) {
    TORCH_CHECK(db_out.has_value() && db_out->defined(), "norm_bwd_seg: LayerNorm needs db_out");
    chk(*db_out, "db_out");
    TORCH_CHECK(db_out->stride(0) == dw_out.stride(0), "dw_out / db_out: one row stride");
    dbp = db_out->data_ptr();
  }
  const c10::DeviceGuard guard(x.device());
  Tensor dx = at::empty_like(x);
  Tensor work = at::empty({static_cast<int64_t>(cml::norm_workspace_bytes_seg(M, static_cast<int>(D),
                                                                              static_cast<int>(nseg)) / 4 + 1)},
                          x.options().dtype(at::kFloat));
  CML_CHECK_HIP(cml::launch_norm_bwd_seg(ln ? 1 : 0, dy.data_ptr(), dres.defined() ? dres.data_ptr() : nullptr,
                                         x.data_ptr(), w.data_ptr(), ln ? mean->data_ptr<float>() : nullptr,
                                         rstd.data_ptr<float>(), dx.data_ptr(), dw_out.data_ptr(), dbp,
                                         M, static_cast<int>(D), static_cast<int>(nseg),
                                         dw_out.stride(0), work.data_ptr(), cur_stream()));
  return dx;
}

}

PYBIND11_MODULE(TORCH_EXTENSION_NAME, m) {
  m.doc() = "consensusml_amd native HIP kernels for gfx950 (MI355X)";
  m.def("agg_update", &agg_update, "fused robust aggregation + optimizer update (mix: a linear "
        "pre-mix of the rows ahead of the sorted combine)",
        py::arg("X"), py::arg("n"), py::arg("D"), py::arg("rows"), py::arg("combine"),
        py::arg("lo"), py::arg("cnt"), py::arg("w"), py::arg("opt"), py::arg("master"),
        py::arg("s1"), py::arg("s2"), py::arg("param_out"), py::arg("gout"), py::arg("lr"),
        py::arg("momentum"), py::arg("weight_decay"), py::arg("beta1"), py::arg("beta2"),
        py::arg("eps"), py::arg("step_size"), py::arg("inv_sqrt_bc2"), py::arg("gscale"),
        py::arg("nesterov"), py::arg("first"), py::arg("mix") = py::none(),
        py::arg("keep") = 0);
  m.def("gram_workspace_bytes", &gram_workspace_bytes);
  m.def("gram", &gram, "G = X X^T (fp64) on MFMA; center: rows relative to that row",
        py::arg("X"), py::arg("n"), py::arg("D"), py::arg("rows"), py::arg("work"), py::arg("G"),
        py::arg("accumulate"), py::arg("center") = py::none(), py::arg("grid_cap") = 0);
  m.def("gram_center", &gram_center, "medoid of the finite rows of a Gram matrix");
  m.def("robust_weights", &robust_weights, "robust weights from a Gram matrix (+ selection counts, "
        "next center and the centered-pass guard in the same launch)",
        py::arg("G"), py::arg("rule"), py::arg("n"), py::arg("f"), py::arg("m"), py::arg("iters"),
        py::arg("eps"), py::arg("tol"), py::arg("tau"), py::arg("w"), py::arg("scores"),
        py::arg("sel"), py::arg("guard") = false, py::arg("center_out") = py::none(),
        py::arg("sel_counts") = py::none(), py::arg("pre") = 0, py::arg("mix_out") = py::none());
  m.def("gram_sum", &gram_sum, "sum of per-bucket Gram partials in bucket order");
  m.def("gram_partial", &gram_partial, "Gram stage 1 into a per-bucket workspace (block count)",
        py::arg("X"), py::arg("n"), py::arg("D"), py::arg("work"), py::arg("center") = py::none(),
        py::arg("grid_cap") = 0);
  m.def("gram_reduce_multi", &gram_reduce_multi,
        "reduce several buckets' Gram partials into G in one launch (bucket order)");
  m.def("agg_update_multi", &agg_update_multi,
        "fused robust aggregation + optimizer step over several buckets in one launch",
        py::arg("Xs"), py::arg("Ds"), py::arg("offs"), py::arg("pouts"), py::arg("n"),
        py::arg("rows"), py::arg("combine"), py::arg("lo"), py::arg("cnt"), py::arg("w"),
        py::arg("opt"), py::arg("master"), py::arg("s1"), py::arg("s2"), py::arg("gout"),
        py::arg("lr"), py::arg("momentum"), py::arg("weight_decay"), py::arg("beta1"),
        py::arg("beta2"), py::arg("eps"), py::arg("step_size"), py::arg("inv_sqrt_bc2"),
        py::arg("gscale"), py::arg("nesterov"), py::arg("first"), py::arg("mix") = py::none(),
        py::arg("keep") = 0);
  m.def("gossip_workspace_bytes", &gossip_workspace_bytes);
  m.def("gossip_mix", &gossip_mix, "ring gossip mixing with neighbour clipping");
  m.def("gossip_mix_k", &gossip_mix_k, "k-neighbour gossip mixing with neighbour clipping (optional "
        "second parameter output: the delayed-gossip send buffer)", py::arg("master"),
        py::arg("param_out"), py::arg("nbrs"), py::arg("w"), py::arg("w0"), py::arg("clip"),
        py::arg("work"), py::arg("param_out2") = py::none(), py::arg("grid_cap") = 0);
  m.def("colsum_seg", &colsum_seg, "per-segment column sums into strided rows");
  m.def("norm_bwd_seg", &norm_bwd_seg, "LayerNorm / RMSNorm backward with per-segment dgamma / dbeta");
  m.def("conv1x1g_mode", &cml::conv1x1g_mode, "fused 1x1 kernel family: 0 old, 1 glds, 2 auto");
  m.def("set_conv1x1g_mode", &cml::set_conv1x1g_mode, "select the fused 1x1 kernel family");
  m.def("set_conv1x1g_ablate", &cml::set_conv1x1g_ablate, "diagnostics: quad kernel ablation bits");
  m.def("fault", &fault, "Byzantine fault injection");
  m.def("worker_momentum", &worker_momentum,
        "worker-side momentum: mom <- beta mom + rows, rows <- mom, in place over an [R, L] window",
        py::arg("rows"), py::arg("mom"), py::arg("beta"), py::arg("grid_cap") = 0);
  m.def("sq_norm_workspace", &sq_norm_workspace, "fp64 partials sq_norm writes for these lengths",
        py::arg("bf16_rows"), py::arg("lens"), py::arg("grid_cap") = 0);
  m.def("sq_norm", &sq_norm, "out[0] = sum of (float(x) * scale)^2 over the segments, in fp64",
        py::arg("segments"), py::arg("scale"), py::arg("work"), py::arg("out"),
        py::arg("grid_cap") = 0);
  m.def("clip_coef", &clip_coef, "global-norm clipping coefficient as a device weight + stats",
        py::arg("norm2"), py::arg("max_norm"), py::arg("base"), py::arg("w_out"), py::arg("stats"),
        py::arg("reduced") = py::none());
  m.def("bn_fwd", &bn_fwd, "fused NHWC BatchNorm(+res)(+ReLU) forward");
  m.def("bn_bwd", &bn_bwd, "fused NHWC BatchNorm(+res)(+ReLU) backward");
  m.def("bn_fwd2", &bn_fwd2, "relu(BN(x1) + BN(x2)) forward (downsample-block tail)");
  m.def("bn_bwd2", &bn_bwd2, "relu(BN(x1) + BN(x2)) backward");
  m.def("bn_relu_maxpool_fwd", &bn_relu_maxpool_fwd, "maxpool(relu(BN(x))) forward (stem)");
  m.def("stem_conv_fwd", &stem_conv_fwd, "ResNet stem 7x7/s2 conv + BN statistics (MFMA)");
  m.def("stem_wgrad", &stem_wgrad, "ResNet stem weight gradient through BN (MFMA, one pass)");
  m.def("maxpool_fwd", &maxpool_fwd, "NHWC bf16 max-pool forward (uint8 argmax)");
  m.def("maxpool_bwd", &maxpool_bwd, "NHWC bf16 max-pool backward (gather)");
  m.def("conv1x1_bn_fwd", &conv1x1_bn_fwd, py::arg("x"), py::arg("w"), py::arg("pro_sc"),
        py::arg("pro_bi"), py::arg("shift"), py::arg("running_mean"), py::arg("running_var"),
        py::arg("stride"), py::arg("stats"), py::arg("eps"), py::arg("momentum"),
        py::arg("gamma") = py::none(), py::arg("beta") = py::none(),
        "fused 1x1 conv forward (MFMA) + BN statistics epilogue + optional BN-ReLU prologue "
        "(+ with gamma / beta that BN's affine sc, bi from the statistics' finalize)");
  m.def("bn_stats", &bn_stats, "training BatchNorm statistics (mean, invstd) only");
  m.def("wgrad1x1", &wgrad1x1, py::arg("dy"), py::arg("x"), py::arg("dtype"),
        py::arg("pro_sc") = py::none(), py::arg("pro_bi") = py::none(),
        py::arg("dz_z") = py::none(), py::arg("dz_mask") = py::none(), py::arg("dz_a") = py::none(),
        py::arg("dz_b") = py::none(), py::arg("dz_c") = py::none(), py::arg("out") = py::none(),
        "weight gradient of a stride-1 1x1 conv (MFMA, split-K)");
  m.def("wgrad3x3s2_ok", &wgrad3x3s2_ok, py::arg("N"), py::arg("H"), py::arg("W"),
        py::arg("Co"), py::arg("Ci"), py::arg("taps") = 9);
  m.def("wgrad3x3s2", &wgrad3x3s2, py::arg("dy"), py::arg("x"), py::arg("dtype"),
        py::arg("zero") = py::none(), py::arg("taps") = 9);
  m.def("wgrad3x3", &wgrad3x3, py::arg("dy"), py::arg("x"), py::arg("dtype"),
        py::arg("zero") = py::none(),
        "weight gradient of a 3x3 stride-1 conv (MFMA, split-K, all nine taps per workgroup: "
        "wgrad3x3.hip) for shapes with wgrad3x3_direct_ok");
  m.def("conv1x1_link_s2", &conv1x1_link_s2,
        "1x1 data gradient + a stride-2 conv's compact data gradient at the even pixels");
  m.def("subsample2", &subsample2, "x[:, :, ::2, ::2] of an NHWC bf16 tensor, dense NHWC");
  m.def("upsample2_scatter", &upsample2_scatter, py::arg("g"), py::arg("H"), py::arg("W"),
        "full-resolution NHWC tensor with g at the even pixels, zeros elsewhere");
  m.def("wgrad3x3_direct_ok", [](int64_t B, int64_t H, int64_t W, int64_t Co, int64_t Ci) {
    int S, T;
    return cml::wgrad3x3_direct_plan(static_cast<int>(B), static_cast<int>(H), static_cast<int>(W),
                                     static_cast<int>(Co), static_cast<int>(Ci), &S, &T);
  }, "whether wgrad3x3 takes the nine-tap kernel for this shape");
  m.def("conv_gemm_bnsums", &conv_gemm_bnsums, py::arg("x"), py::arg("w"), py::arg("taps"),
        py::arg("zero"), py::arg("z"), py::arg("sc"), py::arg("bi"), py::arg("mean"),
        py::arg("invstd"), py::arg("dgamma_out") = py::none(), py::arg("dbeta_out") = py::none(),
        "stride-1 conv_gemm + the sums of the BN + ReLU backward its output feeds (+ optionally "
        "that BN's parameter gradients)");
  m.def("conv_gemm_s2dgrad", &conv_gemm_s2dgrad, py::arg("dy"), py::arg("wr"), py::arg("zero"),
        py::arg("z") = py::none(), py::arg("sc") = py::none(), py::arg("bi") = py::none(),
        py::arg("mean") = py::none(), py::arg("invstd") = py::none(),
        py::arg("dgamma_out") = py::none(), py::arg("dbeta_out") = py::none(),
        "stride-2 3x3 data gradient as four parity-class implicit GEMMs (+ BN + ReLU backward sums, "
        "+ optionally that BN's parameter gradients)");
  m.def("conv_gemm", &conv_gemm, py::arg("x"), py::arg("w"), py::arg("taps"),
        py::arg("zero") = py::none(), py::arg("stride") = 1,
        "implicit-GEMM NHWC conv (1x1 / 3x3 padding 1, stride 1 or 2), glds staging");
  m.def("conv1x1_bn_stats_only", &conv1x1_bn_stats_only, py::arg("x"), py::arg("w"),
        py::arg("pro_sc"), py::arg("pro_bi"), py::arg("shift") = py::none(),
        py::arg("running_mean") = py::none(), py::arg("running_var") = py::none(),
        py::arg("eps") = 1e-5, py::arg("momentum") = 0.1,
        "BN statistics of conv1x1(bnrelu(x)) without storing the product");
  m.def("conv1x1_bnres", &conv1x1_bnres, "recomputed conv1x1 + BN apply + residual + ReLU -> {y, mask}");
  m.def("conv1x1_cat_bnres", &conv1x1_cat_bnres,
        "two BN'd 1x1 convs summed + ReLU in one K-concatenated GEMM -> {y, mask}");
  m.def("conv1x1_cat_bnsums", &conv1x1_cat_bnsums, py::arg("g"), py::arg("mask"), py::arg("x2"),
        py::arg("sc2"), py::arg("bi2"), py::arg("w"), py::arg("bias"), py::arg("mean"),
        py::arg("invstd"), py::arg("dgamma_out") = py::none(), py::arg("dbeta_out") = py::none(),
        "conv1x1_cat + the sums of the BN + ReLU backward its output feeds (+ optionally that "
        "BN's parameter gradients)");
  m.def("bn_affine", &bn_affine, "BN affine (gamma invstd, beta - mean sc) of batch statistics");
  m.def("bn_bwd_apply", &bn_bwd_apply, "apply half of a BN + ReLU backward from its sums");
  m.def("split_search_sampled", &split_search_sampled,
        "tree split search with in-kernel candidate sampling, <= 128 bins -> {gain, feature, bin}");
  m.def("tail_bwd_prep", &tail_bwd_prep,
        "recompute-tail backward algebra: {w_cat, bias, dW, dgamma, dbeta}");
  m.def("conv1x1_cat", &conv1x1_cat, "two-source (masked | BN-ReLU or identity) 1x1 conv along K, + bias");
  m.def("split_fold", &split_fold, "fixed-order fold of a split-K partial slab");
  m.def("wgrad1x1_ex", &wgrad1x1_ex, py::arg("dy"), py::arg("x"), py::arg("pro_sc") = py::none(),
        py::arg("pro_bi") = py::none(), py::arg("dmode") = 0, py::arg("dz_mask") = py::none(),
        py::arg("dz_a") = py::none(), py::arg("dz_b") = py::none(), py::arg("dz_c") = py::none(),
        py::arg("colsum") = false, "1x1 weight gradient with dy prologue modes and column sums");
  m.def("conv_gemm_bn", &conv_gemm_bn, py::arg("x"), py::arg("w"), py::arg("taps"),
        py::arg("zero") = py::none(), py::arg("shift") = py::none(),
        py::arg("running_mean") = py::none(), py::arg("running_var") = py::none(),
        py::arg("eps") = 1e-5, py::arg("momentum") = 0.1, py::arg("stride") = 1,
        py::arg("gamma") = py::none(), py::arg("beta") = py::none(),
        "implicit-GEMM conv + BN statistics of the output in the epilogue -> {y, mean, invstd} "
        "(+ sc, bi: the BN's affine from the finalize, with gamma / beta)");
  m.def("conv1x1_bnbwd", &conv1x1_bnbwd, "1x1 data gradient through a BN + ReLU backward prologue");
  m.def("conv1x1_link", &conv1x1_link, py::arg("x"), py::arg("w"), py::arg("link"),
        py::arg("lmask"), py::arg("sz") = py::none(), py::arg("smask") = py::none(),
        py::arg("mean") = py::none(), py::arg("invstd") = py::none(),
        "1x1 data gradient + masked residual gradient (lmask None: plain residual add) (+ the "
        "consumer BN's backward sums)");
  m.def("bn_stats_gram", &bn_stats_gram, py::arg("G"), py::arg("cy"), py::arg("w"), py::arg("M"),
        py::arg("running_mean") = py::none(), py::arg("running_var") = py::none(),
        py::arg("eps") = 1e-5, py::arg("momentum") = 0.1, py::arg("gamma") = py::none(),
        py::arg("beta") = py::none(),
        "BN statistics of a 1x1 conv's output from its input's Gram matrix and column sums "
        "(+ the BN affine sc, bi when gamma / beta are given)");
  m.def("bn_bwd_coeffs", &bn_bwd_coeffs, "BN + ReLU backward coefficients from its sums");
  m.def("bn_bwd_sums", &bn_bwd_sums, "reduction half of a BN (+ ReLU) backward");
  m.def("stem_wgrad_pool", &stem_wgrad_pool, py::arg("dy"), py::arg("idx"), py::arg("dy2"),
        py::arg("z"), py::arg("x"), py::arg("mean"), py::arg("invstd"), py::arg("gamma"),
        py::arg("bf16_out") = false,
        "stem backward (conv weight gradient through BN, dgamma, dbeta) from the pool output "
        "gradient, the pool input gradient gathered inside the kernel");
  m.def("avgpool_bwd", &avgpool_bwd, py::arg("g"), py::arg("H"), py::arg("W"),
        "global-average-pool backward into NHWC in one write-only pass");
  m.def("conv_wlayouts_multi", &conv_wlayouts_multi, py::arg("ws"),
        "GEMM layouts of several 3x3 / 1x1 conv weights in one launch -> [(wf, wr), ...]");
  m.def("scaled_cat_bias", &scaled_cat_bias, py::arg("w1"), py::arg("s1"), py::arg("w2"),
        py::arg("s2"), py::arg("b1"), py::arg("b2"),
        "[diag(s1) w1 | diag(s2) w2] (bf16) and b1 + b2 in one launch");
  m.def("conv3x3_wlayouts", &conv3x3_wlayouts, py::arg("w"), py::arg("want_wf"),
        "forward / data-gradient GEMM layouts of a 3x3 conv weight in one launch");
  m.def("maxpool_bwd_sum", &maxpool_bwd_sum, "3x3/s2 max-pool backward + channel sums of dx",
        py::arg("dy"), py::arg("idx"), py::arg("H"), py::arg("W"), py::arg("dy2") = py::none());
  m.def("multi_copy", &multi_copy, "multi-tensor copy in one launch per 32 tensors");
  m.def("pad_c4", &pad_c4, "NHWC bf16 channel zero-padding to 4");
  m.def("ce_fwd", &ce_fwd, "fused cross-entropy forward over bf16 logits (lse, per-row loss)");
  m.def("ce_bwd", &ce_bwd, py::arg("logits"), py::arg("labels"), py::arg("lse"), py::arg("scale"),
        py::arg("ignore"), py::arg("div") = py::none(),
        "fused cross-entropy backward (bf16 logits gradient; scale / div when div is given)");
  m.def("ce_bwd_cs", &ce_bwd_cs, py::arg("logits"), py::arg("labels"), py::arg("lse"),
        py::arg("scale"), py::arg("ignore"), py::arg("div") = py::none(),
        "cross-entropy backward over row-strided logits + bias-gradient column partials");
  m.def("ce_mean", &ce_mean, py::arg("loss"), py::arg("labels"), py::arg("ignore"),
        "{mean loss, n_valid} from ce_fwd's per-row losses in one launch");
  m.def("transpose_bf16", &transpose_bf16, "w.t().contiguous() (LDS-tiled bf16 transpose)");
  m.def("gelu_bwd", &gelu_bwd, "dh = da * gelu'(h) (erf GELU), bf16");
  m.def("ce_part_fold", &ce_part_fold, "per-segment fold of ce_bwd_cs's column partials");
  m.def("norm_fwd", &norm_fwd, "LayerNorm / RMSNorm (+ residual add) forward");
  m.def("norm_bwd", &norm_bwd, "LayerNorm / RMSNorm backward (+ residual gradient)");
  m.def("rope_fwd", &rope_fwd, "QKV split + RoPE into head-major q / k / v");
  m.def("rope_bwd", &rope_bwd, "inverse of rope_fwd (grp > 1: sums per-query-head dk / dv)",
        py::arg("dq"), py::arg("dk"), py::arg("dv"), py::arg("cos"), py::arg("sin"),
        py::arg("grp") = 1);
  m.def("flash_fwd", &flash_fwd, "flash attention forward, head dim 128, GQA, causal / full",
        py::arg("q"), py::arg("k"), py::arg("v"), py::arg("causal"), py::arg("scale"),
        py::arg("rescale_thr") = 8.0);
  m.def("flash_bwd", &flash_bwd, "flash attention backward (dq, per-query-head dk / dv)");
  m.def("swiglu_fwd", &swiglu_fwd, "silu(a) * b over [a | b]");
  m.def("swiglu_bwd", &swiglu_bwd, "SwiGLU backward");
  m.def("attn_fwd", &attn_fwd, "short-sequence MFMA attention forward (fused qkv in)");
  m.def("attn_bwd", &attn_bwd, "short-sequence MFMA attention backward (fused dqkv out)");
  m.def("split_search", &split_search, "tree-ensemble histogram split search (one level)");
  m.def("svm_smo", &svm_smo, "batched dual C-SVC SMO (one wave per problem)");
  m.def("smo_max_n", &cml::smo_max_n);
  m.def("lasso_resid", &lasso_resid, "batched logistic-lasso residual (+ intercept gradient)");
  m.def("lasso_step", &lasso_step, "batched FISTA prox / restart / momentum step");
  m.def("lasso_slices", &lasso_slices);
  m.def("colsum", &colsum, "column sums of a bf16 matrix (bias gradient)");
  m.def("gemm_nt", &gemm_nt, "NT GEMM with fused epilogues (bias / bias+GELU / GELU backward + "
        "column sums)", py::arg("a"), py::arg("b"), py::arg("ep"), py::arg("bias") = py::none(),
        py::arg("aux") = py::none(), py::arg("out") = py::none(),
        py::arg("colsum_out") = py::none(), py::arg("cin") = py::none(), py::arg("tile") = 0);
  m.def("gemm_w4", &gemm_w4, "GEMM on 4-wave 256 x 256 tiles, any operand layout (mode bit 0: a is "
        "[K, M], bit 1: b is [K, N])", py::arg("a"), py::arg("b"), py::arg("mode") = 0,
        py::arg("out") = py::none(), py::arg("bias") = py::none(), py::arg("cin") = py::none());
  m.def("gemm_nt_ok", &gemm_nt_ok, "shape eligibility of gemm_nt's 256 x 256 kernel");
  m.def("gemm_conv_tm", &gemm_conv_tm, "m-tile of gemm.hip's 3x3 conv mode for M x N, C (256, 512, 0)");
  m.def("gemm_nt_pick", &gemm_nt_pick, "EP_STORE tile choice of gemm_nt: 256, 128 or 0 (none)");
  m.attr("CMB_SORTED") = static_cast<int>(cml::CMB_SORTED);
  m.attr("CMB_WEIGHTED") = static_cast<int>(cml::CMB_WEIGHTED);
  m.attr("OPT_NONE") = static_cast<int>(cml::OPT_NONE);
  m.attr("OPT_SGD") = static_cast<int>(cml::OPT_SGD);
  m.attr("OPT_ADAM") = static_cast<int>(cml::OPT_ADAM);
  m.attr("RULE_MEAN") = static_cast<int>(cml::RULE_MEAN);
  m.attr("RULE_KRUM") = static_cast<int>(cml::RULE_KRUM);
  m.attr("RULE_MULTI_KRUM") = static_cast<int>(cml::RULE_MULTI_KRUM);
  m.attr("RULE_GEOMED") = static_cast<int>(cml::RULE_GEOMED);
  m.attr("RULE_CCLIP") = static_cast<int>(cml::RULE_CCLIP);
  m.attr("RULE_BULYAN_SELECT") = static_cast<int>(cml::RULE_BULYAN_SELECT);
}
```

### csrc/kernels/bn_act.hip

```cpp
#include <cstdlib>

#include "common.h"
#include "kernels.h"

namespace cml {
namespace {

constexpr int kBT = 256;

struct BNGeom {
  int tpr;
  int rpi;
  int nb;
  int64_t rpb;
};

BNGeom geom(int64_t M, int C) {
  BNGeom g;
  g.tpr = C / 8;
  g.rpi = kBT / g.tpr;
  const int64_t iters = (M + g.rpi - 1) / g.rpi;
  int64_t nb = (iters + 15) / 16;
  if (nb > 1024) nb = 1024;
  if (nb < 1) nb = 1;
// ... 18 lines not shown
  }
}
void bn_nt_init() {
  static const bool done = [] {
    const char* e = getenv("CML_BN_NT");
    const int v = e ? atoi(e) : 0;
    if (v) (void)hipMemcpyToSymbol(HIP_SYMBOL(g_bn_nt), &v, sizeof(int));
    return true;
  }();
  (void)done;
}

__device__ __forceinline__ void block_partial(float (&a)[8], float (&b)[8], int tpr, int C,
                                              float* __restrict__ part) {
  __shared__ float sa[kBT * 8];
  __shared__ float sb[kBT * 8];
  const int t = threadIdx.x;
#pragma unroll
  for (int v = 0; v < 8; ++v) {
    sa[t * 8 + v] = a[v];
    sb[t * 8 + v] = b[v];
  }
  __syncthreads();
  const int rpi = kBT / tpr;
  float* pa = part + static_cast<int64_t>(blockIdx.x) * 2 * C;
  float* pb = pa + C;
  for (int c = t; c < C; c += kBT) {
    const int g = c >> 3, v = c & 7;
    float x = 0.f, y = 0.f;
    for (int r = 0; r < rpi; ++r) {
      x += sa[(r * tpr + g) * 8 + v];
      y += sb[(r * tpr + g) * 8 + v];
    }
    pa[c] = x;
    pb[c] = y;
  }
}

__global__ __launch_bounds__(kBT) void bn_stats_kernel(const bf16* __restrict__ x, int64_t M, int C,
                                                      int64_t rpb, float* __restrict__ part) {
  const int tpr = C / 8;
  const int rpi = kBT / tpr;
  const int g = threadIdx.x % tpr;
  const int r0 = threadIdx.x / tpr;
  float sh[8];
  ld8(x + 8 * g, sh);
  float s[8] = {0, 0, 0, 0, 0, 0, 0, 0}, q[8] = {0, 0, 0, 0, 0, 0, 0, 0};
  const int64_t lo = static_cast<int64_t>(blockIdx.x) * rpb;
  const int64_t hi = lo + rpb < M ? lo + rpb : M;
  int64_t r = lo + r0;
  for (; r + 3 * rpi < hi; r += 4 * rpi) {
    float v[4][8];
#pragma unroll
    for (int u = 0; u < 4; ++u) ld8(x + (r + u * rpi) * C + 8 * g, v[u]);
#pragma unroll
    for (int u = 0; u < 4; ++u)
#pragma unroll
      for (int k = 0; k < 8; ++k) {
        const float d = v[u][k] - sh[k];
        s[k] += d;
        q[k] = fmaf(d, d, q[k]);
      }
  }
  for (; r < hi; r += rpi) {
    float v[8];
    ld8(x + r * C + 8 * g, v);
#pragma unroll
    for (int k = 0; k < 8; ++k) {
      const float d = v[k] - sh[k];
      s[k] += d;
      q[k] = fmaf(d, d, q[k]);
    }
  }
  block_partial(s, q, tpr, C, part);
}

constexpr int kFC = 8;
constexpr int kFS = kBT / kFC;
__device__ __forceinline__ bool fold_partials(const float* __restrict__ part, int nb, int C,
                                              double& s_out, double& q_out, int& c_out) {
  __shared__ double ls[kFS][kFC], lq[kFS][kFC];
  const int cl = threadIdx.x % kFC, sl = threadIdx.x / kFC;
  const int c = blockIdx.x * kFC + cl;
  double S = 0.0, Q = 0.0;
  if (c < C) {
    int b = sl;
    for (; b + 7 * kFS < nb; b += 8 * kFS) {
      float s[8], q[8];
#pragma unroll
      for (int u = 0; u < 8; ++u) {
        const float* p = part + static_cast<int64_t>(b + u * kFS) * 2 * C;
        s[u] = p[c];
        q[u] = p[C + c];
      }
#pragma unroll
      for (int u = 0; u < 8; ++u) {
        S += s[u];
        Q += q[u];
      }
    }
    for (; b < nb; b += kFS) {
      const float* p = part + static_cast<int64_t>(b) * 2 * C;
      S += p[c];
      Q += p[C + c];
    }
  }
  ls[sl][cl] = S;
  lq[sl][cl] = Q;
  __syncthreads();
  if (sl != 0 || c >= C) return false;
  S = 0.0;
  Q = 0.0;
#pragma unroll
  for (int k = 0; k < kFS; ++k) {
    S += ls[k][cl];
    Q += lq[k][cl];
  }
  s_out = S;
  q_out = Q;
  c_out = c;
  return true;
}

__global__ __launch_bounds__(kBT) void bn_finalize_kernel(const float* __restrict__ part, int nb,
                                                         const bf16* __restrict__ x, int64_t M,
                                                         int C, float eps, float momentum,
                                                         float* __restrict__ mean,
                                                         float* __restrict__ invstd,
                                                         float* __restrict__ rmean,
                                                         float* __restrict__ rvar) {
  double s, q;
  int c;
  if (!fold_partials(part, nb, C, s, q, c)) return;
  const double ms = s / static_cast<double>(M);
  double var = q / static_cast<double>(M) - ms * ms;
  if (var < 0.0) var = 0.0;
  const double mu = static_cast<double>(bf2f(reinterpret_cast<const uint16_t*>(x)[c])) + ms;
  mean[c] = static_cast<float>(mu);
  invstd[c] = static_cast<float>(1.0 / sqrt(var + static_cast<double>(eps)));
  if (rmean) {
    const double unb = M > 1 ? var * static_cast<double>(M) / static_cast<double>(M - 1) : var;
    rmean[c] = static_cast<float>((1.0 - momentum) * rmean[c] + momentum * mu);
    rvar[c] = static_cast<float>((1.0 - momentum) * rvar[c] + momentum * unb);
  }
}

__device__ __forceinline__ void chan_affine(int g, const float* mean, const float* invstd,
                                            const bf16* gamma, const bf16* beta, float (&sc)[8],
                                            float (&bi)[8]) {
  float ga[8], be[8];
  ld8(gamma + 8 * g, ga);
  ld8(beta + 8 * g, be);
#pragma unroll
  for (int k = 0; k < 8; ++k) {
    sc[k] = invstd[8 * g + k] * ga[k];
    bi[k] = be[k] - mean[8 * g + k] * sc[k];
  }
}

template <bool RES, bool RELU, bool MASK>
__global__ __launch_bounds__(kBT) void bn_apply_kernel(const bf16* __restrict__ x,
                                                      const bf16* __restrict__ res,
                                                      bf16* __restrict__ y,
                                                      uint8_t* __restrict__ mask, int64_t M, int C,
                                                      const float* __restrict__ mean,
                                                      const float* __restrict__ invstd,
                                                      const bf16* __restrict__ gamma,
                                                      const bf16* __restrict__ beta) {
  const int tpr = C / 8;
  const int g = threadIdx.x % tpr;
  float sc[8], bi[8];
  chan_affine(g, mean, invstd, gamma, beta, sc, bi);
  const int64_t rstride = static_cast<int64_t>(gridDim.x) * (kBT / tpr);
  for (int64_t r = static_cast<int64_t>(blockIdx.x) * (kBT / tpr) + threadIdx.x / tpr; r < M;
       r += 2 * rstride) {
    const bool two = r + rstride < M;
    float v[2][8], rv[2][8];
    ld8(x + r * C + 8 * g, v[0]);
    if constexpr (RES) ld8(res + r * C + 8 * g, rv[0]);
    if (two) {
      ld8(x + (r + rstride) * C + 8 * g, v[1]);
      if constexpr (RES) ld8(res + (r + rstride) * C + 8 * g, rv[1]);
    }
#pragma unroll
    for (int u = 0; u < 2; ++u) {
      if (u == 1 && !two) break;
      const int64_t ru = r + u * rstride;
      uint32_t bits = 0;
#pragma unroll
      for (int k = 0; k < 8; ++k) {
        float z = fmaf(v[u][k], sc[k], bi[k]);
        if constexpr (RES) z += rv[u][k];
        if constexpr (MASK) bits |= (z > 0.f ? 1u : 0u) << k;
        if constexpr (RELU) z = fmaxf(z, 0.f);
        v[u][k] = z;
      }
      store_bf16<8>(y + ru * C + 8 * g, v[u]);
      if constexpr (MASK) mask[ru * tpr + g] = static_cast<uint8_t>(bits);
    }
  }
}

enum { RM_NONE = 0, RM_RECOMP = 1, RM_MASK = 2 };

template <int RM, bool DY2>
__device__ __forceinline__ void load_dz(const bf16* __restrict__ dy, const bf16* __restrict__ dy2,
                                        const uint8_t* __restrict__ mask, int64_t r, int C, int g,
                                        const float (&v)[8], const float (&sc)[8],
                                        const float (&bi)[8], float (&dz)[8]) {
  ld8(dy + r * C + 8 * g, dz);
  if constexpr (DY2) {
    float d2[8];
    ld8(dy2 + r * C + 8 * g, d2);
#pragma unroll
    for (int k = 0; k < 8; ++k) dz[k] += d2[k];
  }
  if constexpr (RM == RM_MASK) {
    const uint32_t bits = mask[r * (C / 8) + g];
#pragma unroll
    for (int k = 0; k < 8; ++k) dz[k] = ((bits >> k) & 1u) ? dz[k] : 0.f;
  } else if constexpr (RM == RM_RECOMP) {
#pragma unroll
    for (int k = 0; k < 8; ++k) dz[k] = fmaf(v[k], sc[k], bi[k]) > 0.f ? dz[k] : 0.f;
  }
}

template <int RM, bool DY2>
__global__ __launch_bounds__(kBT) void bn_bwd_reduce_kernel(const bf16* __restrict__ dy,
                                                           const bf16* __restrict__ dy2,
                                                           const bf16* __restrict__ x,
                                                           const uint8_t* __restrict__ mask,
                                                           int64_t M, int C, int64_t rpb,
                                                           const float* __restrict__ mean,
                                                           const float* __restrict__ invstd,
                                                           const bf16* __restrict__ gamma,
                                                           const bf16* __restrict__ beta,
                                                           float* __restrict__ part) {
  const int tpr = C / 8;
  const int rpi = kBT / tpr;
  const int g = threadIdx.x % tpr;
  float sc[8], bi[8], mu[8], is[8];
  chan_affine(g, mean, invstd, gamma, beta, sc, bi);
#pragma unroll
  for (int k = 0; k < 8; ++k) {
    mu[k] = mean[8 * g + k];
    is[k] = invstd[8 * g + k];
  }
  float s[8] = {0, 0, 0, 0, 0, 0, 0, 0}, q[8] = {0, 0, 0, 0, 0, 0, 0, 0};
  const int64_t lo = static_cast<int64_t>(blockIdx.x) * rpb;
  const int64_t hi = lo + rpb < M ? lo + rpb : M;
  int64_t r = lo + threadIdx.x / tpr;
  for (; r + rpi < hi; r += 2 * rpi) {
    float v[2][8], dz[2][8];
    ld8(x + r * C + 8 * g, v[0]);
    ld8(x + (r + rpi) * C + 8 * g, v[1]);
    load_dz<RM, DY2>(dy, dy2, mask, r, C, g, v[0], sc, bi, dz[0]);
    load_dz<RM, DY2>(dy, dy2, mask, r + rpi, C, g, v[1], sc, bi, dz[1]);
#pragma unroll
    for (int u = 0; u < 2; ++u)
#pragma unroll
      for (int k = 0; k < 8; ++k) {
        s[k] += dz[u][k];
        q[k] = fmaf(dz[u][k], (v[u][k] - mu[k]) * is[k], q[k]);
      }
  }
  for (; r < hi; r += rpi) {
    float v[8], dz[8];
    ld8(x + r * C + 8 * g, v);
    load_dz<RM, DY2>(dy, dy2, mask, r, C, g, v, sc, bi, dz);
#pragma unroll
    for (int k = 0; k < 8; ++k) {
      s[k] += dz[k];
      q[k] = fmaf(dz[k], (v[k] - mu[k]) * is[k], q[k]);
    }
  }
  block_partial(s, q, tpr, C, part);
}

__global__ __launch_bounds__(kBT) void bn_bwd_finalize_kernel(const float* __restrict__ part, int nb,
                                                             int C, float* __restrict__ sdz,
                                                             float* __restrict__ sdzx,
                                                             bf16* __restrict__ dgamma,
                                                             bf16* __restrict__ dbeta) {
  double s, q;
  int c;
  if (!fold_partials(part, nb, C, s, q, c)) return;
  sdz[c] = static_cast<float>(s);
  sdzx[c] = static_cast<float>(q);
  reinterpret_cast<uint16_t*>(dbeta)[c] = f2bf(static_cast<float>(s));
  reinterpret_cast<uint16_t*>(dgamma)[c] = f2bf(static_cast<float>(q));
}

template <int RM, bool DRES, bool DY2>
__global__ __launch_bounds__(kBT) void bn_bwd_apply_kernel(const bf16* __restrict__ dy,
                                                          const bf16* __restrict__ dy2,
                                                          const bf16* __restrict__ x,
                                                          const uint8_t* __restrict__ mask,
                                                          bf16* __restrict__ dx,
                                                          bf16* __restrict__ dres, int64_t M, int C,
                                                          const float* __restrict__ mean,
                                                          const float* __restrict__ invstd,
                                                          const bf16* __restrict__ gamma,
                                                          const bf16* __restrict__ beta,
                                                          const float* __restrict__ sdz,
                                                          const float* __restrict__ sdzx) {
  const int tpr = C / 8;
  const int g = threadIdx.x % tpr;
  float sc[8], bi[8], mu[8], is[8], a[8], b[8];
  chan_affine(g, mean, invstd, gamma, beta, sc, bi);
  const float invM = 1.0f / static_cast<float>(M);
#pragma unroll
  for (int k = 0; k < 8; ++k) {
    mu[k] = mean[8 * g + k];
    is[k] = invstd[8 * g + k];
    a[k] = sdz[8 * g + k] * invM;
    b[k] = sdzx[8 * g + k] * invM;
  }
  const int64_t rstride = static_cast<int64_t>(gridDim.x) * (kBT / tpr);
  for (int64_t r = static_cast<int64_t>(blockIdx.x) * (kBT / tpr) + threadIdx.x / tpr; r < M;
       r += 2 * rstride) {
    const bool two = r + rstride < M;
    float v[2][8], dz[2][8];
    ld8(x + r * C + 8 * g, v[0]);
    if (two) ld8(x + (r + rstride) * C + 8 * g, v[1]);
    load_dz<RM, DY2>(dy, dy2, mask, r, C, g, v[0], sc, bi, dz[0]);
    if (two) load_dz<RM, DY2>(dy, dy2, mask, r + rstride, C, g, v[1], sc, bi, dz[1]);
#pragma unroll
    for (int u = 0; u < 2; ++u) {
      if (u == 1 && !two) break;
      const int64_t ru = r + u * rstride;
      float o[8];
#pragma unroll
      for (int k = 0; k < 8; ++k) {
        const float xh = (v[u][k] - mu[k]) * is[k];
        o[k] = sc[k] * (dz[u][k] - a[k] - xh * b[k]);
      }
      store_bf16<8>(dx + ru * C + 8 * g, o);
      if constexpr (DRES) store_bf16<8>(dres + ru * C + 8 * g, dz[u]);
    }
  }
}

template <bool MASK>
__global__ __launch_bounds__(kBT) void bn_apply2_kernel(const bf16* __restrict__ x1,
                                                       const bf16* __restrict__ x2,
                                                       bf16* __restrict__ y,
                                                       uint8_t* __restrict__ mask, int64_t M, int C,
                                                       const float* __restrict__ mean1,
                                                       const float* __restrict__ invstd1,
                                                       const bf16* __restrict__ gamma1,
                                                       const bf16* __restrict__ beta1,
                                                       const float* __restrict__ mean2,
                                                       const float* __restrict__ invstd2,
                                                       const bf16* __restrict__ gamma2,
                                                       const bf16* __restrict__ beta2) {
  const int tpr = C / 8;
  const int g = threadIdx.x % tpr;
  float sc1[8], bi1[8], sc2[8], bi2[8];
  chan_affine(g, mean1, invstd1, gamma1, beta1, sc1, bi1);
  chan_affine(g, mean2, invstd2, gamma2, beta2, sc2, bi2);
#pragma unroll
  for (int k = 0; k < 8; ++k) bi1[k] += bi2[k];
  const int64_t rstride = static_cast<int64_t>(gridDim.x) * (kBT / tpr);
  for (int64_t r = static_cast<int64_t>(blockIdx.x) * (kBT / tpr) + threadIdx.x / tpr; r < M;
       r += 2 * rstride) {
    const bool two = r + rstride < M;
    float a[2][8], b[2][8];
    ld8(x1 + r * C + 8 * g, a[0]);
    ld8(x2 + r * C + 8 * g, b[0]);
    if (two) {
      ld8(x1 + (r + rstride) * C + 8 * g, a[1]);
      ld8(x2 + (r + rstride) * C + 8 * g, b[1]);
    }
#pragma unroll
    for (int u = 0; u < 2; ++u) {
      if (u == 1 && !two) break;
      const int64_t ru = r + u * rstride;
      uint32_t bits = 0;
#pragma unroll
      for (int k = 0; k < 8; ++k) {
        const float z = fmaf(a[u][k], sc1[k], fmaf(b[u][k], sc2[k], bi1[k]));
        if constexpr (MASK) bits |= (z > 0.f ? 1u : 0u) << k;
        a[u][k] = fmaxf(z, 0.f);
      }
      store_bf16<8>(y + ru * C + 8 * g, a[u]);
      if constexpr (MASK) mask[ru * tpr + g] = static_cast<uint8_t>(bits);
    }
  }
}

template <bool DY2>
__global__ __launch_bounds__(kBT) void bn_bwd_reduce2_kernel(const bf16* __restrict__ dy,
                                                            const bf16* __restrict__ dy2,
                                                            const bf16* __restrict__ x1,
                                                            const bf16* __restrict__ x2,
                                                            const uint8_t* __restrict__ mask,
                                                            int64_t M, int C, int64_t rpb,
                                                            const float* __restrict__ mean1,
                                                            const float* __restrict__ invstd1,
                                                            const float* __restrict__ mean2,
                                                            const float* __restrict__ invstd2,
                                                            float* __restrict__ part1,
                                                            float* __restrict__ part2) {
  const int tpr = C / 8;
  const int rpi = kBT / tpr;
  const int g = threadIdx.x % tpr;
  float mu1[8], is1[8], mu2[8], is2[8], dummy[8];
#pragma unroll
  for (int k = 0; k < 8; ++k) {
    mu1[k] = mean1[8 * g + k];
    is1[k] = invstd1[8 * g + k];
    mu2[k] = mean2[8 * g + k];
    is2[k] = invstd2[8 * g + k];
    dummy[k] = 0.f;
  }
  float s[8] = {0, 0, 0, 0, 0, 0, 0, 0}, q1[8] = {0, 0, 0, 0, 0, 0, 0, 0};
  float q2[8] = {0, 0, 0, 0, 0, 0, 0, 0};
  const int64_t lo = static_cast<int64_t>(blockIdx.x) * rpb;
  const int64_t hi = lo + rpb < M ? lo + rpb : M;
  for (int64_t r = lo + threadIdx.x / tpr; r < hi; r += rpi) {
    float a[8], b[8], dz[8];
    ld8(x1 + r * C + 8 * g, a);
    ld8(x2 + r * C + 8 * g, b);
    load_dz<RM_MASK, DY2>(dy, dy2, mask, r, C, g, a, dummy, dummy, dz);
#pragma unroll
    for (int k = 0; k < 8; ++k) {
      s[k] += dz[k];
      q1[k] = fmaf(dz[k], (a[k] - mu1[k]) * is1[k], q1[k]);
      q2[k] = fmaf(dz[k], (b[k] - mu2[k]) * is2[k], q2[k]);
    }
  }
  block_partial(s, q1, tpr, C, part1);
  __syncthreads();
  block_partial(s, q2, tpr, C, part2);
}

template <bool DY2>
__global__ __launch_bounds__(kBT) void bn_bwd_apply2_kernel(const bf16* __restrict__ dy,
                                                           const bf16* __restrict__ dy2,
                                                           const bf16* __restrict__ x1,
                                                           const bf16* __restrict__ x2,
                                                           const uint8_t* __restrict__ mask,
                                                           bf16* __restrict__ dx1,
                                                           bf16* __restrict__ dx2, int64_t M, int C,
                                                           const float* __restrict__ mean1,
                                                           const float* __restrict__ invstd1,
                                                           const bf16* __restrict__ gamma1,
                                                           const float* __restrict__ mean2,
                                                           const float* __restrict__ invstd2,
                                                           const bf16* __restrict__ gamma2,
                                                           const float* __restrict__ sdz,
                                                           const float* __restrict__ sdzx1,
                                                           const float* __restrict__ sdzx2) {
  const int tpr = C / 8;
  const int g = threadIdx.x % tpr;
  const float invM = 1.0f / static_cast<float>(M);
  float g1[8], g2[8], mu1[8], is1[8], mu2[8], is2[8], c1[8], c2[8], av[8], b1[8], b2[8], dummy[8];
  ld8(gamma1 + 8 * g, g1);
  ld8(gamma2 + 8 * g, g2);
#pragma unroll
  for (int k = 0; k < 8; ++k) {
    mu1[k] = mean1[8 * g + k];
    is1[k] = invstd1[8 * g + k];
    mu2[k] = mean2[8 * g + k];
    is2[k] = invstd2[8 * g + k];
    c1[k] = g1[k] * is1[k];
    c2[k] = g2[k] * is2[k];
    av[k] = sdz[8 * g + k] * invM;
    b1[k] = sdzx1[8 * g + k] * invM;
    b2[k] = sdzx2[8 * g + k] * invM;
    dummy[k] = 0.f;
  }
  const int64_t rstride = static_cast<int64_t>(gridDim.x) * (kBT / tpr);
  for (int64_t r = static_cast<int64_t>(blockIdx.x) * (kBT / tpr) + threadIdx.x / tpr; r < M;
       r += rstride) {
    float a[8], b[8], dz[8], o1[8], o2[8];
    ld8(x1 + r * C + 8 * g, a);
    ld8(x2 + r * C + 8 * g, b);
    load_dz<RM_MASK, DY2>(dy, dy2, mask, r, C, g, a, dummy, dummy, dz);
#pragma unroll
    for (int k = 0; k < 8; ++k) {
      const float d0 = dz[k] - av[k];
      o1[k] = c1[k] * (d0 - (a[k] - mu1[k]) * is1[k] * b1[k]);
      o2[k] = c2[k] * (d0 - (b[k] - mu2[k]) * is2[k] * b2[k]);
    }
    store_bf16<8>(dx1 + r * C + 8 * g, o1);
    store_bf16<8>(dx2 + r * C + 8 * g, o2);
  }
}
// ... 237 lines not shown
```

### csrc/kernels/common.h

```cpp
#pragma once
#include <hip/hip_runtime.h>
#include <hip/hip_bf16.h>
#include <stdint.h>

namespace cml {

constexpr int kWave = 64;

using bf16 = __hip_bfloat16;
typedef float f32x4 __attribute__((ext_vector_type(4)));
typedef short bf16x8 __attribute__((ext_vector_type(8)));

__device__ __forceinline__ float bf2f(uint16_t b) {
  return __uint_as_float(static_cast<uint32_t>(b) << 16);
}
__device__ __forceinline__ uint16_t f2bf(float f) {
  bf16 h = __float2bfloat16(f);
  return *reinterpret_cast<uint16_t*>(&h);
}

typedef __bf16 bf16x2_t __attribute__((ext_vector_type(2)));
typedef float f32x2 __attribute__((ext_vector_type(2)));
typedef short i16x2 __attribute__((ext_vector_type(2)));

__device__ __forceinline__ uint32_t pk_bf16(float lo, float hi) {
  const f32x2 v = {lo, hi};
  return __builtin_bit_cast(uint32_t, __builtin_convertvector(v, bf16x2_t));
}
__device__ __forceinline__ uint32_t relu_pk(uint32_t w) {
  const i16x2 z = {0, 0};
  return __builtin_bit_cast(uint32_t, __builtin_elementwise_max(__builtin_bit_cast(i16x2, w), z));
}
__device__ __forceinline__ uint32_t bnrelu_pk(uint32_t w, f32x2 sc, f32x2 bi) {
  const f32x2 x = {__uint_as_float(w << 16), __uint_as_float(w & 0xffff0000u)};
  const f32x2 y = __builtin_elementwise_fma(x, sc, bi);
  return relu_pk(pk_bf16(y.x, y.y));
}
template <int I>
__device__ __forceinline__ uint32_t mask_pk(uint32_t w, uint32_t bits) {
  uint32_t lo, hi, m;
  asm("v_bfe_i32 %0, %1, %2, 1" : "=v"(lo) : "v"(bits), "i"(2 * I));
  asm("v_bfe_i32 %0, %1, %2, 1" : "=v"(hi) : "v"(bits), "i"(2 * I + 1));
  asm("v_bfi_b32 %0, %1, %2, %3" : "=v"(m) : "v"(0xffffu), "v"(lo), "v"(hi));
  return w & m;
}

template <typename T, int VEC>
__device__ __forceinline__ void load_vec(const T* __restrict__ p, float (&out)[VEC]);

template <>
__device__ __forceinline__ void load_vec<bf16, 8>(const bf16* __restrict__ p, float (&o)[8]) {
  uint4 u = *reinterpret_cast<const uint4*>(p);
  uint32_t w[4] = {u.x, u.y, u.z, u.w};
#pragma unroll
  for (int i = 0; i < 4; ++i) {
    o[2 * i] = __uint_as_float(w[i] << 16);
    o[2 * i + 1] = __uint_as_float(w[i] & 0xffff0000u);
  }
}
template <>
__device__ __forceinline__ void load_vec<bf16, 4>(const bf16* __restrict__ p, float (&o)[4]) {
  uint2 u = *reinterpret_cast<const uint2*>(p);
  o[0] = __uint_as_float(u.x << 16);
  o[1] = __uint_as_float(u.x & 0xffff0000u);
  o[2] = __uint_as_float(u.y << 16);
  o[3] = __uint_as_float(u.y & 0xffff0000u);
}
template <>
__device__ __forceinline__ void load_vec<bf16, 2>(const bf16* __restrict__ p, float (&o)[2]) {
  uint32_t u = *reinterpret_cast<const uint32_t*>(p);
  o[0] = __uint_as_float(u << 16);
  o[1] = __uint_as_float(u & 0xffff0000u);
}
template <>
__device__ __forceinline__ void load_vec<bf16, 1>(const bf16* __restrict__ p, float (&o)[1]) {
  o[0] = bf2f(*reinterpret_cast<const uint16_t*>(p));
}
template <>
__device__ __forceinline__ void load_vec<float, 8>(const float* __restrict__ p, float (&o)[8]) {
  float4 a = *reinterpret_cast<const float4*>(p);
  float4 b = *reinterpret_cast<const float4*>(p + 4);
  o[0] = a.x; o[1] = a.y; o[2] = a.z; o[3] = a.w;
  o[4] = b.x; o[5] = b.y; o[6] = b.z; o[7] = b.w;
}
template <>
__device__ __forceinline__ void load_vec<float, 4>(const float* __restrict__ p, float (&o)[4]) {
  float4 a = *reinterpret_cast<const float4*>(p);
  o[0] = a.x; o[1] = a.y; o[2] = a.z; o[3] = a.w;
}
template <>
__device__ __forceinline__ void load_vec<float, 2>(const float* __restrict__ p, float (&o)[2]) {
  float2 a = *reinterpret_cast<const float2*>(p);
  o[0] = a.x; o[1] = a.y;
}
template <>
__device__ __forceinline__ void load_vec<float, 1>(const float* __restrict__ p, float (&o)[1]) {
  o[0] = *p;
}

template <int VEC>
__device__ __forceinline__ void store_f32(float* __restrict__ p, const float (&v)[VEC]) {
  if constexpr (VEC % 4 == 0) {
#pragma unroll
    for (int i = 0; i < VEC; i += 4)
      *reinterpret_cast<float4*>(p + i) = make_float4(v[i], v[i + 1], v[i + 2], v[i + 3]);
  } else if constexpr (VEC == 2) {
    *reinterpret_cast<float2*>(p) = make_float2(v[0], v[1]);
  } else {
#pragma unroll
    for (int i = 0; i < VEC; ++i) p[i] = v[i];
  }
}

template <int VEC>
__device__ __forceinline__ void store_bf16(bf16* __restrict__ p, const float (&v)[VEC]) {
  if constexpr (VEC == 8) {
    uint4 u;
    u.x = f2bf(v[0]) | (uint32_t(f2bf(v[1])) << 16);
    u.y = f2bf(v[2]) | (uint32_t(f2bf(v[3])) << 16);
    u.z = f2bf(v[4]) | (uint32_t(f2bf(v[5])) << 16);
    u.w = f2bf(v[6]) | (uint32_t(f2bf(v[7])) << 16);
    *reinterpret_cast<uint4*>(p) = u;
  } else if constexpr (VEC == 4) {
    uint2 u;
    u.x = f2bf(v[0]) | (uint32_t(f2bf(v[1])) << 16);
    u.y = f2bf(v[2]) | (uint32_t(f2bf(v[3])) << 16);
    *reinterpret_cast<uint2*>(p) = u;
  } else if constexpr (VEC == 2) {
    *reinterpret_cast<uint32_t*>(p) = f2bf(v[0]) | (uint32_t(f2bf(v[1])) << 16);
  } else {
#pragma unroll
    for (int i = 0; i < VEC; ++i) reinterpret_cast<uint16_t*>(p)[i] = f2bf(v[i]);
  }
}

typedef unsigned short u16x2 __attribute__((ext_vector_type(2)));

__device__ __forceinline__ float vmin(float x, float y) { return fminf(x, y); }
__device__ __forceinline__ float vmax(float x, float y) { return fmaxf(x, y); }
__device__ __forceinline__ u16x2 vmin(u16x2 x, u16x2 y) { return __builtin_elementwise_min(x, y); }
__device__ __forceinline__ u16x2 vmax(u16x2 x, u16x2 y) { return __builtin_elementwise_max(x, y); }

template <typename E, int VEC>
__device__ __forceinline__ void cswap(E (&x)[VEC], E (&y)[VEC]) {
#pragma unroll
  for (int v = 0; v < VEC; ++v) {
    E lo = vmin(x[v], y[v]);
    E hi = vmax(x[v], y[v]);
    x[v] = lo;
    y[v] = hi;
  }
}

template <typename E, int NP, int VEC, int LO, int HI, int R>
struct OEMerge {
  static __device__ __forceinline__ void run(E (&a)[NP][VEC]) {
    constexpr int STEP = R * 2;
    if constexpr (STEP < HI - LO) {
      OEMerge<E, NP, VEC, LO, HI, STEP>::run(a);
      OEMerge<E, NP, VEC, LO + R, HI, STEP>::run(a);
#pragma unroll
      for (int i = LO + R; i < HI - R; i += STEP) cswap<E, VEC>(a[i], a[i + R]);
    } else {
      cswap<E, VEC>(a[LO], a[LO + R]);
    }
  }
};

template <typename E, int NP, int VEC, int LO, int HI>
struct OESort {
  static __device__ __forceinline__ void run(E (&a)[NP][VEC]) {
    if constexpr (HI - LO >= 1) {
      constexpr int MID = LO + (HI - LO) / 2;
      OESort<E, NP, VEC, LO, MID>::run(a);
      OESort<E, NP, VEC, MID + 1, HI>::run(a);
      OEMerge<E, NP, VEC, LO, HI, 1>::run(a);
    }
  }
};

template <typename E, int NP, int VEC>
__device__ __forceinline__ void sort_columns(E (&a)[NP][VEC]) {
  OESort<E, NP, VEC, 0, NP - 1>::run(a);
}

constexpr unsigned short kKeyInf = 0xFF01;

__device__ __forceinline__ u16x2 bf16_key(uint32_t w) {
  const u16x2 x = __builtin_bit_cast(u16x2, w);
  typedef short s16x2 __attribute__((ext_vector_type(2)));
  const u16x2 sgn = __builtin_bit_cast(u16x2, __builtin_bit_cast(s16x2, x) >> 15);
  const u16x2 k = (x ^ (sgn | static_cast<unsigned short>(0x8000))) - static_cast<unsigned short>(127);
  return vmin(k, u16x2{kKeyInf, kKeyInf});
}

__device__ __forceinline__ void bf16_unkey(u16x2 k, float& lo, float& hi) {
  typedef short s16x2 __attribute__((ext_vector_type(2)));
// ... 41 lines not shown
```

### csrc/kernels/kernels.h

```cpp
#pragma once
#include <hip/hip_runtime.h>
#include <stdint.h>

namespace cml {

enum DType : int { DT_BF16 = 0, DT_F32 = 1 };
enum Combine : int { CMB_SORTED = 0, CMB_WEIGHTED = 1 };
enum Opt : int { OPT_NONE = 0, OPT_SGD = 1, OPT_ADAM = 2 };
enum Rule : int {
  RULE_MEAN = 0,
  RULE_KRUM = 1,
  RULE_MULTI_KRUM = 2,
  RULE_GEOMED = 3,
  RULE_CCLIP = 4,
  RULE_BULYAN_SELECT = 5,
  RULE_NNM_ONLY = 6,
};

struct SrcArgs {
  const void* X;
  int64_t ld;
  int n;
  int keep;
  const int* rows;
// ... 104 lines not shown
  void* dst[kMaxCopy];
  int64_t bytes[kMaxCopy];
  int64_t vpre[kMaxCopy + 1];
  int bpre[kMaxCopy + 1];
  int n;
  int slice;
};
hipError_t launch_multi_copy(const MultiCopyArgs& args, hipStream_t stream);
hipError_t launch_transpose_bf16(const void* src, void* dst, int R, int C, int64_t lds, int64_t ldd,
                                 hipStream_t stream);

size_t maxpool_bwd_sum_workspace_bytes(int N, int H, int W, int C);
size_t pool_gsum_workspace_floats(int64_t P, int C);
hipError_t launch_pool_gsum(const void* dy, const void* dy2, const void* idx, void* dsum,
                            float* sums, float* work, int64_t P, int C, hipStream_t st);
hipError_t launch_maxpool_bwd_sum(const void* dy, const void* dy2, const void* idx, void* dx,
                                  float* sums, void* work, int N, int H, int W, int C, int OH,
                                  int OW, hipStream_t stream);
hipError_t launch_bn_stats(const void* x, int64_t M, int C, float* mean, float* invstd,
                           float* rmean, float* rvar, float eps, float momentum, void* work,
                           hipStream_t stream);
hipError_t launch_bn_relu_maxpool_fwd(const void* x, const float* mean, const float* invstd,
                                      const void* gamma, const void* beta, void* y, void* idx,
                                      int N, int H, int W, int C, int OH, int OW, int k, int s,
                                      int p, hipStream_t stream);

hipError_t launch_pad_c4(const void* x, void* y, int64_t npix, int C, hipStream_t stream);

hipError_t launch_fault(int dtype, void* g, int64_t D, int kind, float scale, float sigma,
                        uint64_t seed, hipStream_t stream);

hipError_t launch_worker_momentum(int dtype, void* rows, int64_t ldr, float* mom, int64_t ldm,
                                  int R, int64_t L, float beta, int grid_cap, hipStream_t stream);

constexpr int kSqNormMaxSegs = 16;
struct SqNormSeg {
  const void* x;
  int64_t len;
};
int sq_norm_grid(int dtype, int64_t maxlen, int nseg, int grid_cap);
hipError_t launch_sq_norm_partial(int dtype, const SqNormSeg* segs, int nseg, float scale,
                                  double* work, int grid_cap, hipStream_t stream);
constexpr int kClipStats = 4;
hipError_t launch_clip_finalize(const double* partials, int npart, double* norm2,
                                const double* reduced, double max_norm, float base, float* w_out,
                                double* stats, hipStream_t stream);

hipError_t launch_ce_fwd(const void* logits, int64_t R, int V, int64_t ld, const int64_t* labels,
                         int64_t ignore, float* lse, float* loss, hipStream_t stream);
hipError_t launch_ce_bwd(const void* logits, int64_t R, int V, const int64_t* labels,
                         int64_t ignore, const float* lse, const float* scale, void* grad,
                         hipStream_t stream, const float* div = nullptr);
hipError_t launch_ce_mean(const float* loss, const int64_t* labels, int64_t R, int64_t ignore,
                          float* out, float* count, hipStream_t stream);
hipError_t launch_ce_bwd_cs(const void* logits, int64_t R, int V, int64_t ld,
                            const int64_t* labels, int64_t ignore, const float* lse,
                            const float* scale, void* grad, float* part, hipStream_t stream,
                            const float* div = nullptr);
hipError_t launch_ce_part_fold(const float* part, int64_t R, int V, int64_t ld, int nseg, void* out,
                               int64_t ldo, int out_f32, hipStream_t stream);
hipError_t launch_gelu_bwd(const void* da, const void* h, void* dh, int64_t n, hipStream_t stream);
size_t norm_workspace_bytes(int64_t M, int D);
hipError_t launch_norm_fwd(int ln, const void* x, const void* res, const void* w, const void* b,
                           void* y, void* sum, float* mean, float* rstd, int64_t M, int D,
                           float eps, hipStream_t stream);
hipError_t launch_norm_bwd(int ln, const void* dy, const void* dres, const void* x,
                           const void* w, const float* mean, const float* rstd, void* dx,
                           void* dw, void* db, int64_t M, int D, void* work, hipStream_t stream);
size_t norm_workspace_bytes_seg(int64_t M, int D, int nseg);
hipError_t launch_norm_bwd_seg(int ln, const void* dy, const void* dres, const void* x,
                               const void* w, const float* mean, const float* rstd, void* dx,
                               void* dw, void* db, int64_t M, int D, int nseg, int64_t ostride,
                               void* work, hipStream_t stream);
hipError_t launch_rope_fwd(const void* qkv, const float* cosb, const float* sinb, void* q, void* k,
                           void* v, int B, int S, int H, int KV, int hd, hipStream_t stream);
hipError_t launch_rope_bwd(const void* dq, const void* dk, const void* dv, const float* cosb,
                           const float* sinb, void* dqkv, int B, int S, int H, int KV, int hd,
                           hipStream_t stream, int grp = 1);
hipError_t launch_flash_fwd(const void* q, const void* k, const void* v, void* o, float* lse, int B,
                            int H, int KV, int S, float scale, bool causal, hipStream_t stream,
                            float rescale_thr = 8.f);
hipError_t launch_flash_bwd(const void* q, const void* k, const void* v, const void* o,
                            const void* dout, const float* lse, float* dsum, void* dq, void* dk,
                            void* dv, int B, int H, int KV, int S, float scale, bool causal,
                            hipStream_t stream);
hipError_t launch_swiglu_fwd(const void* h, void* y, int64_t M, int F, hipStream_t stream);
hipError_t launch_swiglu_bwd(const void* dy, const void* h, void* dh, int64_t M, int F,
                             hipStream_t stream);
hipError_t launch_attn_fwd(const void* qkv, void* out, float* lse, int B, int S, int H,
                           float scale, hipStream_t stream);
hipError_t launch_attn_bwd(const void* qkv, const void* out, const void* dout, const float* lse,
                           void* dqkv, int B, int S, int H, float scale, hipStream_t stream);
hipError_t launch_split_search(const uint8_t* Xb, const int* node_local, const float* stat,
                               const int* feats, const float* tot, int T, int L, int n, int p,
                               int kk, int B, int crit, float lam, float min_child,
                               float* out_gain, int* out_slot, int* out_bin, hipStream_t stream);
hipError_t launch_split_search_sampled(const uint8_t* Xb, const int* node_local,
                                       const float* stat, const float* tot, int T, int L, int n,
                                       int p, int kk, int B, int crit, float lam, float min_child,
                                       uint64_t seed, float* out_gain, int* out_feat, int* out_bin,
                                       hipStream_t stream);
int lasso_slices(int p);
hipError_t launch_lasso_resid(const float* z, const float* v0, const float* y, const float* M,
                              const float* nb, float* r, float* rsum, int n, int B,
                              hipStream_t stream);
hipError_t launch_lasso_step(float* v, float* beta, const float* g, const float* step,
                             const float* lam, float alpha, float* tk, const float* rsum,
                             float* v0, float* b0, float* nbeta, float* mom, float* part,
                             float* conv_part, int p, int B, hipStream_t stream);
size_t colsum_workspace_bytes(int64_t M, int N);
hipError_t launch_colsum(const void* x, int64_t M, int N, void* out, void* work,
                         hipStream_t stream);
hipError_t launch_colsum_seg(const void* x, int64_t M, int N, int nseg, void* out,
                             int64_t ostride, void* work, hipStream_t stream);

int stem_fwd_grid(int N, int OH, int OW, int C);
int stem_bwd_grid(int N, int OH, int OW, int C);
size_t stem_wgrad_part_floats();
hipError_t launch_stem_conv_fwd(const void* x, const void* wpk, void* z, float* part, int grid,
                                float* mean, float* invstd, float* rmean, float* rvar, float eps,
                                float momentum, int N, int H, int W, int C, int OH, int OW,
                                hipStream_t stream);
hipError_t launch_stem_wgrad(const void* g, const void* z, const void* x, const float* mean,
                             const float* invstd, const void* gamma, const float* gsum,
                             float* part, int grid,
                             double* tot, void* dw, void* dgamma, void* dbeta, int N, int H,
                             int W, int C, int OH, int OW, hipStream_t stream,
                             const uint8_t* pidx = nullptr, float* cola_work = nullptr,
                             bool out_bf16 = false);
size_t stem_wgrad_tot_doubles();
size_t stem_cola_work_floats(int N, int H, int W, int C);

void wgrad1x1_plan(int64_t P, int Co, int Ci, int* splits, int* cps, bool pro = false,
                   int dmode = 0, bool cs = false);
bool wgrad1x1_direct(int64_t P, int Co, int Ci, bool pro = false, int dmode = 0, bool cs = false);
hipError_t launch_wgrad1x1_ex(const void* dy, const void* x, float* part, void* dw, bool dw_bf16,
                              int64_t P, int Co, int Ci, const float* pro_sc, const float* pro_bi,
                              hipStream_t st, int dmode, const void* dz_z, const uint8_t* dz_mask,
                              const float* dz_a, const float* dz_b, const float* dz_c,
                              float* cs_part, float* cs);
hipError_t launch_wgrad1x1(const void* dy, const void* x, float* part, void* dw, bool dw_bf16,
                           int64_t P, int Co, int Ci, const float* pro_sc, const float* pro_bi,
                           hipStream_t stream, const void* dz_z = nullptr,
                           const uint8_t* dz_mask = nullptr, const float* dz_a = nullptr,
                           const float* dz_b = nullptr, const float* dz_c = nullptr);

void gram1x1_plan(int64_t M, int p, int* splits, int* cps);
hipError_t launch_gram1x1(const void* z, float* part, float* G, int64_t M, int p, const float* sc,
                          const float* bi, float* cs_part, float* cy, hipStream_t st);
bool gram1x1_route(const void* dy, const void* x, int Co, int Ci, const float* pro_sc,
                   const float* pro_bi, int dmode, const float* dz_a, const float* dz_b,
                   bool dw_bf16);

bool wgrad3x3s2_plan(int N, int H, int W, int Co, int Ci, int* splits, int taps = 9);
hipError_t launch_wgrad3x3s2(const void* dy, const void* x, const void* zero, float* part,
                             void* dw, bool dw_bf16, int N, int H, int W, int Co, int Ci,
                             hipStream_t st, int taps = 9);
hipError_t launch_wgrad_fold(const float* part, int S, int64_t n, void* out, bool out_bf16,
                             hipStream_t st);
bool wgrad3x3_direct_plan(int B, int H, int W, int Co, int Ci, int* splits, int* tci);
hipError_t launch_wgrad3x3_direct(const void* dy, const void* x, const void* zero, float* part,
                                  void* dw, bool dw_bf16, int B, int H, int W, int Co, int Ci,
                                  hipStream_t st);

size_t conv1x1_bn_part_floats(int64_t M, int K, int N, bool pro);
struct BnAffineOut {
  const void* gamma;
  const void* beta;
  float* sc;
  float* bi;
};
hipError_t launch_conv1x1_bn_fwd(const void* x, const void* w, void* y, float* part,
                                 const float* pro_sc, const float* pro_bi, const float* shift,
                                 int64_t M, int K, int N, int stride, int H, int W, float* mean,
                                 float* invstd, float* rmean, float* rvar, float eps,
                                 float momentum, hipStream_t st, const BnAffineOut* aff = nullptr);

size_t conv_gemm_part_floats(int64_t M, int N);
hipError_t launch_conv_gemm_bnsums(const void* x, const void* w, void* y, const void* zero,
                                   int Nimg, int H, int W, int C, int N, int taps, const void* z,
                                   const float* sc, const float* bi, const float* mean,
                                   const float* invstd, float* part, float* sdz, float* sdzx,
                                   hipStream_t st, void* dgamma = nullptr, void* dbeta = nullptr);
hipError_t launch_bnbwd_sums_finalize(const float* part, int R, int BN, int N, const float* invstd,
                                      float* sdz, float* sdzx, hipStream_t st, float* fold,
                                      void* dgamma = nullptr, void* dbeta = nullptr);
size_t conv_gemm_s2dgrad_part_floats(int64_t Mc, int N);
hipError_t launch_conv_gemm_s2dgrad(const void* dy, const void* wr, void* dx, const void* zero,
                                    int Nimg, int Ho, int Wo, int Co, int Ci, const void* z,
                                    const float* sc, const float* bi, const float* mean,
                                    const float* invstd, float* part, float* sdz, float* sdzx,
                                    hipStream_t st, void* dgamma = nullptr, void* dbeta = nullptr);
hipError_t launch_conv3x3_wlayouts(const void* w, int Co, int Ci, int64_t s0, int64_t s1,
                                   int64_t s2, int64_t s3, void* wf, void* wr, hipStream_t st);
struct WlDesc {
  const void* w;
  void* wf;
  void* wr;
  int64_t s0, s1, s2, s3;
  int Co, Ci, taps;
};
constexpr int kWlMax = 24;
hipError_t launch_conv3x3_wlayouts_multi(const WlDesc* d, int n, hipStream_t st);
bool conv3x3p_eligible(int Nimg, int H, int W, int C, int N, int taps, int stride);
size_t conv3x3p_part_floats();
hipError_t launch_conv3x3p(const void* x, const void* w, void* y, const void* zero, int Nimg, int H,
                           int ep, float* part, const float* shift, const void* z, const float* sc,
                           const float* bi, hipStream_t st, int* rows);
hipError_t launch_conv_gemm(const void* x, const void* w, void* y, const void* zero, int Nimg,
                            int H, int W, int C, int N, int taps, hipStream_t st,
                            float* part = nullptr, const float* shift = nullptr,
                            float* mean = nullptr, float* invstd = nullptr,
                            float* rmean = nullptr, float* rvar = nullptr, float eps = 1e-5f,
                            float momentum = 0.1f, int stride = 1,
                            const BnAffineOut* aff = nullptr);
int bn_part_fold_slices(int R, int ntn);
hipError_t launch_bn_stats_finalize(const float* part, int R, int BN, int N, int64_t M,
                                   const float* shift, float eps, float momentum, float* mean,
                                   float* invstd, float* rmean, float* rvar, hipStream_t st,
                                   float* fold = nullptr, const BnAffineOut* aff = nullptr);

size_t conv1x1_link_part_floats(int64_t M, int K, int N);

hipError_t launch_conv1x1_bnres(const void* x, const void* w, void* y, uint8_t* ymask,
                                const float* pro_sc, const float* pro_bi, const float* ep_sc,
                                const float* ep_bi, const void* res, int64_t M, int K, int N,
                                hipStream_t st);
hipError_t launch_conv1x1_cat_bnres(const void* x1, const void* x2, const float* sc1,
                                    const float* bi1, const float* sc2, const float* bi2,
                                    const void* w, const float* ep_sc, const float* ep_bi,
                                    const void* res, void* y, uint8_t* ymask, int64_t M, int K1,
                                    int K, int N, hipStream_t st);
hipError_t launch_conv1x1_cat(const void* g, const uint8_t* mask, const void* x2, const float* sc2,
                              const float* bi2, const float* bias, const void* w, void* y,
                              int64_t M, int K1, int K, int N, hipStream_t st,
                              const float* mean = nullptr, const float* invstd = nullptr,
                              float* part = nullptr, float* sdz = nullptr, float* sdzx = nullptr,
                              void* dgamma = nullptr, void* dbeta = nullptr);
size_t conv1x1_cat_part_floats(int64_t M, int K, int N);
hipError_t launch_conv1x1_bnbwd(const void* g, const void* z, const uint8_t* mask, const float* ca,
                                const float* cb, const float* cc, const void* w, void* y,
                                int64_t M, int K, int N, hipStream_t st);
hipError_t launch_conv1x1_link(const void* x, const void* w, void* y, const void* link,
                               const uint8_t* lm, const void* sz, const uint8_t* sm,
                               const float* mean, const float* invstd, float* part, float* sdz,
                               float* sdzx, int64_t M, int K, int N, hipStream_t st);
hipError_t launch_conv1x1_link_s2(const void* x, const void* w, void* y, const void* link,
                                  int Nimg, int H, int W, int K, int N, hipStream_t st);
hipError_t launch_bn_stats_gram(const float* G, const float* cy, const void* w, int P, int Co,
                                int64_t M, float eps, float momentum, float* mean, float* invstd,
                                float* rmean, float* rvar, double* part, hipStream_t st,
                                const void* gamma = nullptr, const void* beta = nullptr,
                                float* sc = nullptr, float* bi = nullptr);
hipError_t launch_tail_bwd_prep(const void* W, const float* P, const float* s, const float* gram,
                                const float* cy, const void* gamma, const float* mean,
                                const float* invstd, int Co, int p, int64_t M, float* work,
                                void* dW, void* wcat, float* bias, void* dgamma, void* dbeta,
                                hipStream_t st);
size_t tail_bwd_prep_work_floats(int Co, int p);
hipError_t launch_scaled_cat_bias(const void* w1, const float* s1, int k1, const void* w2,
                                  const float* s2, int k2, const float* b1, const float* b2,
                                  int Co, void* out, float* bias, hipStream_t st);
hipError_t launch_bn_bwd_coeffs(const float* sdz, const float* sdzx, const void* gamma,
                                const float* mean, const float* invstd, int C, int64_t M,
                                float* ca, float* cb, float* cc, void* dgamma, void* dbeta,
                                hipStream_t st);

int smo_max_n();
hipError_t launch_smo(const double* K, const double* y, const int* ns, int B, int nmax,
                      const double* C, double tol, int max_iter, double* alpha, double* grad,
                      int* iters, hipStream_t stream);

enum { EP_STORE = 0, EP_GELU = 1, EP_DGELU = 2, EP_CONV_ST = 3, EP_CONV_BB = 4 };
struct GemmArgs {
  const uint16_t* a;
  const uint16_t* b;
  uint16_t* y;
  uint16_t* aux;
  const uint16_t* bias;
  float* part;
  const uint16_t* cin;
  int64_t M, N, K;
  int64_t lda, ldb, ldy;
  int conv, C, H, W;
  int s2, IH, IW;
  int gm;
  const uint16_t* zero;
  const float* shift;
  const uint16_t* sz;
  const float* ep_sc;
  const float* ep_bi;
};
bool gemm_nt_eligible(int64_t M, int64_t N, int64_t K);
hipError_t launch_gemm_nt(const GemmArgs& a, int ep, hipStream_t st);
bool gemm128_eligible(int64_t M, int64_t N, int64_t K);
hipError_t launch_gemm128_nt(const GemmArgs& a, hipStream_t st);
bool gemm_conv_eligible(int64_t M, int N, int C);
int gemm_conv_tm(int64_t M, int N, int C);
hipError_t launch_gemm_conv(const GemmArgs& a, int ep, hipStream_t st);
bool gemm_w4_eligible(int64_t M, int64_t N, int64_t K, int mode);
hipError_t launch_gemm_w4(const GemmArgs& a, int mode, hipStream_t st);
hipError_t launch_colsum_fold(const float* part, int64_t M, int N, int nseg, void* out, int64_t ldo,
                              int out_f32, hipStream_t st);

}
```

Baseline: 17740.

## Fuse bn1 backward into conv1 1x1 dgrad and wgrad via deferred handoff

```diff
diff --git a/consensusml_amd/models/resnet.py b/consensusml_amd/models/resnet.py
--- a/consensusml_amd/models/resnet.py
+++ b/consensusml_amd/models/resnet.py
@@ -7,7 +7,8 @@
 import torch.nn.functional as F
 
 from ..ops import conv as fconv
-from ..ops.bn import BatchNormAct2d, ResidualLink, bn_add_bn_relu, fused_ok, link_tap
+from ..ops.bn import (BatchNormAct2d, DeferredBN1, ResidualLink, bn_add_bn_relu, fused_ok,
+                      link_tap)
 from ..ops.pool import bn_relu_max_pool2d, max_pool2d
 from ..ops.stem import stem_conv_bn_relu_pool, stem_ok
 
@@ -207,13 +208,13 @@
                 and fconv.fused_conv_ok(x, self.conv1.weight)
                 and fused_ok(x, self.bn3.weight))
 
-    def _conv_bn(self, x, conv: "Conv1x1", bn, link=None):
+    def _conv_bn(self, x, conv: "Conv1x1", bn, link=None, hand=None):
         st = conv.stride[0]
         hw = (x.shape[2] // st) * (x.shape[3] // st)
         if fused_conv1x1_policy(conv.in_channels, conv.out_channels, hw, st, False):
             dg = st == 1 and conv1x1_policy(conv.in_channels, conv.out_channels, hw)[1]
             own = own_wgrad_ok(conv.in_channels, conv.out_channels) if st == 1 else True
-            z, m, i = fconv.conv1x1_bn_stats(x, conv, bn, st, dg, own, link if dg else None)
+            z, m, i = fconv.conv1x1_bn_stats(x, conv, bn, st, dg, own, link if dg else None, hand)
             return z, (m, i)
         if st == 1:
             return conv(x, res_link=link if conv.link_ok(x) else None), None
@@ -226,14 +227,15 @@
 
     def _head(self, x: torch.Tensor, use_links: bool):
         link = dlink = None
+        hand = DeferredBN1() if _P().fused_conv1_bwd else None
         if self.down_conv is None:
             link = getattr(x, "_cml_link", None) if use_links else None
         elif use_links and self.conv1.link_ok(x):
             dlink = ResidualLink()
-        z1, st1 = self._conv_bn(x, self.conv1, self.bn1, link if dlink is None else dlink)
-        return z1, st1, link, dlink
-
-    def _conv2_fused(self, z1: torch.Tensor, st1, fuse3: bool):
+        z1, st1 = self._conv_bn(x, self.conv1, self.bn1, link if dlink is None else dlink, hand)
+        return z1, st1, link, dlink, hand
+
+    def _conv2_fused(self, z1: torch.Tensor, st1, fuse3: bool, hand=None):
         pol = _P()
         s1 = self.conv2.stride == (1, 1)
         on = (pol.conv3x3_bn_stats and pol.own_dgrad3x3) if s1 else pol.own_conv3x3_s2
@@ -243,7 +245,7 @@
         if pro and s1 and st1 is None and pol.bn1_sums_lib_conv1:
             st1 = fconv.bn_stats(z1, self.bn1)
         if pro and st1 is not None:
-            return fconv.bnrelu_conv3x3_bn_stats(z1, self.bn1, st1, self.conv2, self.bn2)
+            return fconv.bnrelu_conv3x3_bn_stats(z1, self.bn1, st1, self.conv2, self.bn2, hand)
         out = self.bn1(z1, stats=st1)
         if own3:
             return fconv.conv3x3_bn_stats(out, self.conv2, self.bn2)
@@ -289,11 +291,11 @@
         return bn_add_bn_relu(z, self.bn3, zd, self.down_bn, out_link, stats=stats)
 
     def _forward_fused(self, x: torch.Tensor, use_links: bool) -> torch.Tensor:
-        z1, st1, link, dlink = self._head(x, use_links)
+        z1, st1, link, dlink, hand = self._head(x, use_links)
         planes, s = self.conv3.in_channels, self.conv2.stride[0]
         hw2 = (z1.shape[2] // s) * (z1.shape[3] // s)
         fuse3 = fused_conv1x1_policy(planes, planes * 4, hw2, 1, True)
-        z2, st2 = self._conv2_fused(z1, st1, fuse3)
+        z2, st2 = self._conv2_fused(z1, st1, fuse3, hand)
         out_link = ResidualLink() if use_links else None
         y = self._tail_fused(x, z2, st2, fuse3, hw2, link, dlink, use_links, out_link)
         if out_link is not None:
diff --git a/consensusml_amd/ops/bn.py b/consensusml_amd/ops/bn.py
--- a/consensusml_amd/ops/bn.py
+++ b/consensusml_amd/ops/bn.py
@@ -27,6 +27,30 @@
     def take_tensor(self):
         g = self.take()
         return g.materialize() if hasattr(g, "materialize") else g
+
+
+class DeferredBN1:
+    __slots__ = ("armed", "rec")
+
+    def __init__(self):
+        self.armed = False
+        self.rec = None
+
+    def clear(self) -> None:
+        self.armed = False
+        self.rec = None
+
+    def take(self):
+        r, self.rec = self.rec, None
+        return r
+
+
+def check_deferred_grad(rec, dy: torch.Tensor) -> None:
+    if dy.data_ptr() != rec[-1] or dy.shape != rec[0].shape:
+        raise RuntimeError(
+            "deferred bn1 backward: conv1 received a gradient that is not the dy1 its 3x3 conv "
+            "left unapplied (z1 has another consumer, or a hook replaced the gradient); refusing "
+            "to treat it as dz1")
 
 
 class MaskedGrad:
diff --git a/consensusml_amd/ops/conv.py b/consensusml_amd/ops/conv.py
--- a/consensusml_amd/ops/conv.py
+++ b/consensusml_amd/ops/conv.py
@@ -7,7 +7,7 @@
 import torch.nn.functional as F
 
 from ..perf import policy as _P
-from .bn import MaskedGrad
+from .bn import MaskedGrad, check_deferred_grad
 from .native import lib
 
 
@@ -132,10 +132,40 @@
     return dw
 
 
+def _conv1_bwd_armed(ctx, x: torch.Tensor, w: torch.Tensor, stride: int, link) -> bool:
+    pol = _P()
+    M = x.shape[0] * x.shape[2] * x.shape[3]
+    return bool(pol.fused_conv1_bwd and stride == 1 and M >= pol.fused_conv1_bwd_min_pixels
+                and ctx.needs_input_grad[0] and ctx.needs_input_grad[1]
+                and (link is None or link.bn_ctx is None)
+                and w.dtype == torch.bfloat16 and x.dtype == torch.bfloat16
+                and lib().conv1_bn_bwd_ok(M, w.shape[0], w.shape[1]))
+
+
+def _conv1_bn_bwd(rec, dy: torch.Tensor, x: torch.Tensor, w: torch.Tensor, link):
+    z1, g1, b1, mean1, invstd1, s1, q1, _ = rec
+    g = link.take() if link is not None else None
+    kw = {}
+    if isinstance(g, MaskedGrad):
+        kw = dict(link=g.g, lmask=g.mask)
+    elif isinstance(g, S2Grad) and g.H == x.shape[2] and g.W == x.shape[3]:
+        kw = dict(link=g.g, link_s2=True)
+    elif g is not None:
+        link.grad = g
+        return None
+    dx, dw = lib().conv1_bn_bwd(dy, z1, g1, b1, mean1, invstd1, s1, q1, x, w.reshape(w.shape[0], -1),
+                                w.dtype, **kw)
+    return dx, dw.view_as(w)
+
+
 class _Conv1x1BNStatsFn(torch.autograd.Function):
     @staticmethod
     def forward(ctx, x, w, rmean, rvar, stride, eps, momentum, dgrad_gemm, own_wgrad, link,
-                aff=None):
+                aff=None, hand=None):
+        if hand is not None:
+            hand.clear()
+            hand.armed = _conv1_bwd_armed(ctx, x, w, stride, link)
+        ctx.hand = hand
         out = lib().conv1x1_bn_fwd(x, w, None, None, rmean, rmean, rvar, stride, True, eps,
                                    momentum, *(aff or (None, None)))
         y, mean, invstd = out[:3]
@@ -152,12 +182,19 @@
     def backward(ctx, dy, _dm, _di):
         x, w = ctx.saved_tensors
         dy = dy.contiguous(memory_format=torch.channels_last)
+        rec = ctx.hand.take() if ctx.hand is not None else None
+        if rec is not None:
+            check_deferred_grad(rec, dy)
+            out = _conv1_bn_bwd(rec, dy, x, w, ctx.link)
+            if out is not None:
+                return out + (None,) * 10
+            dy = lib().bn_bwd_apply(dy, *rec[:7])
         dw, h = _wgrad_fork(lambda d, a, b: _wgrad(d, a, b, ctx.stride, ctx.own_wgrad), dy, x, w,
                             conv1x1=True) if ctx.needs_input_grad[1] else (None, None)
         dx = _dgrad(dy, x, w, ctx.stride, ctx.dgrad_gemm, ctx.link, ctx.wt) \
             if ctx.needs_input_grad[0] else None
         dw = _wgrad_join(dw, h)
-        return dx, dw, None, None, None, None, None, None, None, None, None
+        return dx, dw, None, None, None, None, None, None, None, None, None, None
 
 
 class _BNReLUConv1x1BNStatsFn(torch.autograd.Function):
@@ -708,8 +745,9 @@
 
     @staticmethod
     def forward(ctx, z1, g1, b1, mean1, invstd1, eps1, w, rmean, rvar, eps, momentum, stride=1,
-                aff=None):
+                aff=None, hand=None):
         L = lib()
+        ctx.hand = hand
         y1 = L.bn_fwd(z1, None, g1, b1, None, None, mean1, invstd1, eps1, momentum, True, False,
                       False)[0]
         wf, wr = _w3x3_layouts(w, True)
@@ -737,9 +775,15 @@
             dy1, s1, q1 = dgrad(dz2, ctx.wr, *bn1)
             M = z1.numel() // z1.shape[1]
             _, _, _, dg1, db1 = L.bn_bwd_coeffs(s1, q1, g1, mean1, invstd1, M)
-        dz1 = L.bn_bwd_apply(dy1, z1, g1, b1, mean1, invstd1, s1, q1)
+        hand = ctx.hand
+        if hand is not None and hand.armed and ctx.needs_input_grad[0]:
+            dy1 = dy1.contiguous(memory_format=torch.channels_last)
+            hand.rec = (z1, g1, b1, mean1, invstd1, s1, q1, dy1.data_ptr())
+            dz1 = dy1
+        else:
+            dz1 = L.bn_bwd_apply(dy1, z1, g1, b1, mean1, invstd1, s1, q1)
         dw = _wgrad_join(dw, h)
-        return dz1, dg1, db1, None, None, None, dw, None, None, None, None, None, None
+        return dz1, dg1, db1, None, None, None, dw, None, None, None, None, None, None, None
 
 
 def _wgrad3x3_s2(dy: torch.Tensor, x: torch.Tensor, w: torch.Tensor) -> torch.Tensor:
@@ -769,10 +813,11 @@
 
 
 
-def bnrelu_conv3x3_bn_stats(z1: torch.Tensor, bn_a, stats_a, conv, bn):
+def bnrelu_conv3x3_bn_stats(z1: torch.Tensor, bn_a, stats_a, conv, bn, hand=None):
     z, m, i = _BNReLUConv3x3BNStatsFn.apply(z1, bn_a.weight, bn_a.bias, stats_a[0], stats_a[1],
                                             bn_a.eps, conv.weight, bn.running_mean, bn.running_var,
-                                            bn.eps, bn.momentum, conv.stride[0], _fin_aff(bn))
+                                            bn.eps, bn.momentum, conv.stride[0], _fin_aff(bn),
+                                            hand)
     return z, (m, i)
 
 
@@ -799,9 +844,10 @@
 
 
 def conv1x1_bn_stats(x: torch.Tensor, conv, bn, stride: int = 1, dgrad_gemm: bool = False,
-                     own_wgrad: bool = False, link=None):
+                     own_wgrad: bool = False, link=None, hand=None):
     return _Conv1x1BNStatsFn.apply(x, conv.weight, bn.running_mean, bn.running_var, stride,
-                                   bn.eps, bn.momentum, dgrad_gemm, own_wgrad, link, _fin_aff(bn))
+                                   bn.eps, bn.momentum, dgrad_gemm, own_wgrad, link, _fin_aff(bn),
+                                   hand)
 
 
 def bnrelu_conv1x1_bn_stats(z: torch.Tensor, bn_a, stats_a, conv, bn_b, dgrad_gemm: bool = False,
diff --git a/consensusml_amd/perf.py b/consensusml_amd/perf.py
--- a/consensusml_amd/perf.py
+++ b/consensusml_amd/perf.py
@@ -50,6 +50,8 @@
     s2_link_dgrad: bool = True
     down_s2_compact: bool = True
     bn_affine_kernel: bool = True
+    fused_conv1_bwd: bool = True
+    fused_conv1_bwd_min_pixels: int = 65536
     own_dgrad3x3: bool = True
     conv3x3_bn_stats: bool = True
     bn1_dgrad_sums: bool = True
@@ -108,6 +110,8 @@
             s2_link_dgrad=_env_bool("CML_S2_LINK_DGRAD", True),
             down_s2_compact=_env_bool("CML_DOWN_S2_COMPACT", True),
             bn_affine_kernel=_env_bool("CML_BN_AFFINE_KERNEL", True),
+            fused_conv1_bwd=_env_bool("CML_FUSED_CONV1_BWD", True),
+            fused_conv1_bwd_min_pixels=_env_int("CML_FUSED_CONV1_BWD_MIN_PIXELS", 65536),
             own_dgrad3x3=_env_bool("CML_DGRAD3X3", True),
             conv3x3_bn_stats=_env_bool("CML_CONV3X3_BN_STATS", True),
             bn1_dgrad_sums=_env_bool("CML_BN1_DGRAD_SUMS", True),
diff --git a/csrc/bindings.cpp b/csrc/bindings.cpp
--- a/csrc/bindings.cpp
+++ b/csrc/bindings.cpp
@@ -1269,6 +1269,88 @@
       opt_ptr<const float>(sdz, at::kFloat, "sdz", C),
       opt_ptr<const float>(sdzx, at::kFloat, "sdzx", C), cur_stream()));
   return dx;
+}
+
+bool conv1_bn_bwd_ok(int64_t M, int64_t p, int64_t Cin) {
+  int S;
+  return cml::conv1_bwd_plan(M, static_cast<int>(p), static_cast<int>(Cin), &S);
+}
+
+std::vector<Tensor> conv1_bn_bwd(const Tensor& dy_in, const Tensor& z, const Tensor& gamma,
+                                 const Tensor& beta, const Tensor& mean, const Tensor& invstd,
+                                 const Tensor& sdz, const Tensor& sdzx, const Tensor& x,
+                                 const Tensor& w, at::ScalarType dtype,
+                                 const optional<Tensor>& link_in,
+                                 const optional<Tensor>& lmask, bool link_s2, bool want_dz,
+                                 int64_t splits) {
+  check_nhwc(x, "x");
+  check_nhwc(z, "z");
+  TORCH_CHECK(x.dim() == 4 && z.dim() == 4, "conv1_bn_bwd: 4-D NHWC x / z");
+  Tensor dy = dy_in.contiguous(at::MemoryFormat::ChannelsLast);
+  check_nhwc(dy, "dy");
+  const int64_t N = x.size(0), Cin = x.size(1), H = x.size(2), W = x.size(3), M = N * H * W;
+  const int64_t p = z.size(1);
+  TORCH_CHECK(dy.sizes() == z.sizes() && z.size(0) == N && z.size(2) == H && z.size(3) == W,
+              "conv1_bn_bwd: dy / z / x shapes");
+  check_dev(w, "w");
+  TORCH_CHECK(w.scalar_type() == at::kBFloat16 && w.is_contiguous() && w.numel() == p * Cin &&
+                  w.size(0) == p, "conv1_bn_bwd: w must be contiguous bf16 [p, Cin]");
+  TORCH_CHECK(gamma.is_cuda() && beta.is_cuda() && gamma.scalar_type() == at::kBFloat16 &&
+                  beta.scalar_type() == at::kBFloat16 && gamma.is_contiguous() &&
+                  beta.is_contiguous() && gamma.numel() == p && beta.numel() == p,
+              "conv1_bn_bwd: bf16 gamma / beta [p]");
+  TORCH_CHECK(dtype == at::kBFloat16 || dtype == at::kFloat, "conv1_bn_bwd: bf16 or fp32 dw");
+  TORCH_CHECK(splits >= 0 && splits <= 4096, "conv1_bn_bwd: splits out of range");
+  int S = 0;
+  TORCH_CHECK(cml::conv1_bwd_plan(M, static_cast<int>(p), static_cast<int>(Cin), &S,
+                                  static_cast<int>(splits)),
+              "conv1_bn_bwd: p in {64, 128} and Cin in {256, 512} only");
+  const bool has_link = link_in.has_value() && link_in->defined();
+  int kind = 0;
+  Tensor link;
+  const uint8_t* lm = nullptr;
+  if (has_link && link_s2) {
+    kind = 2;
+    link = link_in->contiguous(at::MemoryFormat::ChannelsLast);
+    check_nhwc(link, "link");
+    TORCH_CHECK(link.dim() == 4 && link.size(0) == N && link.size(1) == Cin &&
+                    link.size(2) == (H + 1) / 2 && link.size(3) == (W + 1) / 2,
+                "conv1_bn_bwd: link [N, Cin, ceil(H/2), ceil(W/2)]");
+    TORCH_CHECK(!(lmask.has_value() && lmask->defined()), "conv1_bn_bwd: no mask with link_s2");
+  } else if (has_link) {
+    kind = 1;
+    link = *link_in;
+    check_nhwc(link, "link");
+    TORCH_CHECK(link.sizes() == x.sizes(), "conv1_bn_bwd: link shape");
+    lm = opt_ptr<const uint8_t>(lmask, at::kByte, "lmask", M * Cin / 8);
+    TORCH_CHECK(lm != nullptr, "conv1_bn_bwd: a full-resolution link needs its bit mask");
+  } else {
+    TORCH_CHECK(!link_s2, "conv1_bn_bwd: link_s2 without a link");
+  }
+  const float* mu = opt_ptr<const float>(mean, at::kFloat, "mean", p);
+  const float* is = opt_ptr<const float>(invstd, at::kFloat, "invstd", p);
+  const float* s1 = opt_ptr<const float>(sdz, at::kFloat, "sdz", p);
+  const float* q1 = opt_ptr<const float>(sdzx, at::kFloat, "sdzx", p);
+  TORCH_CHECK(mu && is && s1 && q1, "conv1_bn_bwd: mean, invstd, sdz, sdzx are required");
+  for (const Tensor* t : {static_cast<const Tensor*>(&dy), &z, &x})
+    TORCH_CHECK(reinterpret_cast<uintptr_t>(t->data_ptr()) % 16 == 0,
+                "conv1_bn_bwd: 16-B aligned activations");
+  TORCH_CHECK(!has_link || reinterpret_cast<uintptr_t>(link.data_ptr()) % 16 == 0,
+              "conv1_bn_bwd: 16-B aligned link");
+  const c10::DeviceGuard guard(x.device());
+  Tensor dx = at::empty_like(x);
+  Tensor dw = at::empty({p, Cin, 1, 1}, x.options().dtype(dtype));
+  Tensor part = at::empty({S, p, Cin}, x.options().dtype(at::kFloat));
+  Tensor dz;
+  if (want_dz) dz = at::empty_like(z);
+  CML_CHECK_HIP(cml::launch_conv1_bwd(
+      dy.data_ptr(), z.data_ptr(), gamma.data_ptr(), beta.data_ptr(), mu, is, s1, q1, x.data_ptr(),
+      w.data_ptr(), has_link ? link.data_ptr() : nullptr, lm, kind, static_cast<int>(N),
+      static_cast<int>(H), static_cast<int>(W), dx.data_ptr(), part.data_ptr<float>(), S,
+      dw.data_ptr(), dtype == at::kBFloat16, want_dz ? dz.data_ptr() : nullptr, M,
+      static_cast<int>(p), static_cast<int>(Cin), cur_stream()));
+  if (want_dz) return {dx, dw, dz};
+  return {dx, dw};
 }
 
 Tensor conv1x1_link_s2(const Tensor& x, const Tensor& w, const Tensor& link_in) {
@@ -2663,6 +2745,14 @@
         py::arg("zero") = py::none(),
         "weight gradient of a 3x3 stride-1 conv (MFMA, split-K, all nine taps per workgroup: "
         "wgrad3x3.hip) for shapes with wgrad3x3_direct_ok");
+  m.def("conv1_bn_bwd_ok", &conv1_bn_bwd_ok, py::arg("M"), py::arg("p"), py::arg("Cin"),
+        "whether conv1_bn_bwd takes the shape");
+  m.def("conv1_bn_bwd", &conv1_bn_bwd, py::arg("dy"), py::arg("z"), py::arg("gamma"),
+        py::arg("beta"), py::arg("mean"), py::arg("invstd"), py::arg("sdz"), py::arg("sdzx"),
+        py::arg("x"), py::arg("w"), py::arg("dtype"), py::arg("link") = py::none(),
+        py::arg("lmask") = py::none(), py::arg("link_s2") = false, py::arg("want_dz") = false,
+        py::arg("splits") = 0,
+        "conv1's data and weight gradients with bn1's backward apply formed on chip");
   m.def("conv1x1_link_s2", &conv1x1_link_s2,
         "1x1 data gradient + a stride-2 conv's compact data gradient at the even pixels");
   m.def("subsample2", &subsample2, "x[:, :, ::2, ::2] of an NHWC bf16 tensor, dense NHWC");
diff --git a/csrc/kernels/bn_act.hip b/csrc/kernels/bn_act.hip
--- a/csrc/kernels/bn_act.hip
+++ b/csrc/kernels/bn_act.hip
@@ -194,10 +194,8 @@
   ld8(gamma + 8 * g, ga);
   ld8(beta + 8 * g, be);
 #pragma unroll
-  for (int k = 0; k < 8; ++k) {
-    sc[k] = invstd[8 * g + k] * ga[k];
-    bi[k] = be[k] - mean[8 * g + k] * sc[k];
-  }
+  for (int k = 0; k < 8; ++k)
+    bn_chan_affine(mean[8 * g + k], invstd[8 * g + k], ga[k], be[k], sc[k], bi[k]);
 }
 
 template <bool RES, bool RELU, bool MASK>
@@ -263,7 +261,7 @@
     for (int k = 0; k < 8; ++k) dz[k] = ((bits >> k) & 1u) ? dz[k] : 0.f;
   } else if constexpr (RM == RM_RECOMP) {
 #pragma unroll
-    for (int k = 0; k < 8; ++k) dz[k] = fmaf(v[k], sc[k], bi[k]) > 0.f ? dz[k] : 0.f;
+    for (int k = 0; k < 8; ++k) dz[k] = bn_relu_keep(dz[k], v[k], sc[k], bi[k]);
   }
 }
 
@@ -373,10 +371,8 @@
       const int64_t ru = r + u * rstride;
       float o[8];
 #pragma unroll
-      for (int k = 0; k < 8; ++k) {
-        const float xh = (v[u][k] - mu[k]) * is[k];
-        o[k] = sc[k] * (dz[u][k] - a[k] - xh * b[k]);
-      }
+      for (int k = 0; k < 8; ++k)
+        o[k] = bn_bwd_elem(dz[u][k], v[u][k], mu[k], is[k], sc[k], a[k], b[k]);
       store_bf16<8>(dx + ru * C + 8 * g, o);
       if constexpr (DRES) store_bf16<8>(dres + ru * C + 8 * g, dz[u]);
     }
diff --git a/csrc/kernels/common.h b/csrc/kernels/common.h
--- a/csrc/kernels/common.h
+++ b/csrc/kernels/common.h
@@ -43,6 +43,20 @@
   asm("v_bfe_i32 %0, %1, %2, 1" : "=v"(hi) : "v"(bits), "i"(2 * I + 1));
   asm("v_bfi_b32 %0, %1, %2, %3" : "=v"(m) : "v"(0xffffu), "v"(lo), "v"(hi));
   return w & m;
+}
+
+__device__ __forceinline__ void bn_chan_affine(float mean, float invstd, float gamma, float beta,
+                                               float& sc, float& bi) {
+  sc = invstd * gamma;
+  bi = fmaf(-mean, sc, beta);
+}
+__device__ __forceinline__ float bn_relu_keep(float dy, float z, float sc, float bi) {
+  return fmaf(z, sc, bi) > 0.f ? dy : 0.f;
+}
+__device__ __forceinline__ float bn_bwd_elem(float dy, float z, float mu, float is, float sc,
+                                             float a, float b) {
+  const float xh = (z - mu) * is;
+  return sc * fmaf(-xh, b, dy - a);
 }
 
 template <typename T, int VEC>
diff --git a/csrc/kernels/conv1_bwd.hip b/csrc/kernels/conv1_bwd.hip
--- /dev/null
+++ b/csrc/kernels/conv1_bwd.hip
@@ -0,0 +1,307 @@
+#include "common.h"
+#include "kernels.h"
+#include "wgrad_frag.h"
+
+namespace cml {
+namespace {
+
+constexpr int kTP = 64;
+constexpr int kNT = 512;
+constexpr int kSL = 256;
+
+enum { LK_NONE = 0, LK_MASK = 1, LK_S2 = 2 };
+
+struct C1BArgs {
+  const uint16_t *dy, *z, *x, *w, *g;
+  const uint8_t* gm;
+  const uint16_t *gamma, *beta;
+  const float *mean, *invstd, *sdz, *sdzx;
+  uint16_t *dx, *dz;
+  float* part;
+  int M, Cin, tpw, slices;
+  int W, HW, OW, OHW;
+};
+
+template <int ROWB>
+__device__ __forceinline__ bf16x8_t frag32(const char* img, int c0, int ks, int lane) {
+  const int h = lane >> 5, gi = lane & 15, grp = lane >> 4, q = gi >> 2, pq = gi & 3;
+  const int r0 = 16 * ks + 8 * h + q;
+  const int ch = c0 + 2 * (grp & 1) + (pq >> 1);
+  return cat(ld_tr(img + img_off<ROWB>(r0, ch) + 8 * (pq & 1)),
+             ld_tr(img + img_off<ROWB>(r0 + 4, ch) + 8 * (pq & 1)));
+}
+
+__device__ __forceinline__ uint4 add_link8(uint4 v, uint4 l, uint32_t lb) {
+  const uint32_t l4[4] = {l.x, l.y, l.z, l.w};
+  uint32_t w4[4] = {v.x, v.y, v.z, v.w};
+#pragma unroll
+  for (int q = 0; q < 4; ++q) {
+    const float lo = __uint_as_float(w4[q] << 16) +
+                     (((lb >> (2 * q)) & 1u) ? __uint_as_float(l4[q] << 16) : 0.f);
+    const float hi = __uint_as_float(w4[q] & 0xffff0000u) +
+                     (((lb >> (2 * q + 1)) & 1u) ? __uint_as_float(l4[q] & 0xffff0000u) : 0.f);
+    w4[q] = pk_bf16(lo, hi);
+  }
+  return make_uint4(w4[0], w4[1], w4[2], w4[3]);
+}
+
+template <int P, int LK>
+__global__ __launch_bounds__(kNT) void conv1_bwd_kernel(const C1BArgs a) {
+  constexpr int ZROWB = 2 * P, XROWB = 2 * kSL;
+  constexpr int CA = P / 8;
+  constexpr int ZU = kTP * CA / kNT;
+  constexpr int XU = kTP * (kSL / 8) / kNT;
+  static_assert(kTP * CA % kNT == 0 && kNT % CA == 0 && kNT % 32 == 0, "whole items per thread");
+  extern __shared__ __attribute__((aligned(16))) char smem[];
+  char* const ximg = smem;
+  char* const oimg = ximg + kTP * XROWB;
+  char* const zimg = oimg + kTP * XROWB;
+  float* const cst = reinterpret_cast<float*>(zimg + kTP * ZROWB);
+  const int tid = threadIdx.x, lane = tid & 63;
+  const int cw = __builtin_amdgcn_readfirstlane(tid >> 6);
+  const int h = lane >> 5, r = lane & 31;
+  const int b = blockIdx.x;
+  const int slice = a.slices == 2 ? (b >> 3) & 1 : 0;
+  const int range = a.slices == 2 ? ((b >> 4) << 3) | (b & 7) : b;
+  const int Cin = a.Cin, M = a.M;
+  const int cin0 = slice * kSL;
+  const int ntile = (M + kTP - 1) / kTP;
+  const int t_lo = min(ntile, range * a.tpw);
+  const int t_hi = min(ntile, t_lo + a.tpw);
+
+  bf16x8_t wf[P / 16];
+#pragma unroll
+  for (int ks = 0; ks < P / 16; ++ks) {
+    bf16x8 t;
+#pragma unroll
+    for (int j = 0; j < 8; ++j)
+      t[j] = static_cast<short>(
+          a.w[static_cast<int64_t>(16 * ks + 8 * h + j) * Cin + cin0 + 32 * cw + r]);
+    wf[ks] = __builtin_bit_cast(bf16x8_t, t);
+  }
+  if (tid < P) {
+    const float invM = 1.0f / static_cast<float>(static_cast<int64_t>(M));
+    const float m = a.mean[tid], i = a.invstd[tid];
+    float s, o;
+    bn_chan_affine(m, i, bf2f(a.gamma[tid]), bf2f(a.beta[tid]), s, o);
+    cst[tid] = s;
+    cst[P + tid] = o;
+    cst[2 * P + tid] = m;
+    cst[3 * P + tid] = i;
+    cst[4 * P + tid] = a.sdz[tid] * invM;
+    cst[5 * P + tid] = a.sdzx[tid] * invM;
+  }
+  __syncthreads();
+  const int zr = tid / CA, cz = tid % CA;
+  const int xr = tid >> 5, cx = tid & 31;
+
+  uint4 xv[XU], gv[XU], dyv[ZU], zv[ZU];
+  uint32_t gb[XU];
+  auto fetch = [&](int t) {
+#pragma unroll
+    for (int j = 0; j < XU; ++j) {
+      const int p = min(t * kTP + xr + (kNT / 32) * j, M - 1);
+      const int64_t e0 = static_cast<int64_t>(p) * Cin + cin0 + 8 * cx;
+      xv[j] = *reinterpret_cast<const uint4*>(a.x + e0);
+      if constexpr (LK == LK_MASK) {
+        gv[j] = *reinterpret_cast<const uint4*>(a.g + e0);
+        gb[j] = a.gm[e0 >> 3];
+      } else if constexpr (LK == LK_S2) {
+        const int img = p / a.HW, rem = p - img * a.HW;
+        const int hh = rem / a.W, ww = rem - hh * a.W;
+        const bool ev = !((hh | ww) & 1);
+        const int64_t lrow =
+            ev ? static_cast<int64_t>(img) * a.OHW + (hh >> 1) * a.OW + (ww >> 1) : 0;
+        gv[j] = *reinterpret_cast<const uint4*>(a.g + lrow * Cin + cin0 + 8 * cx);
+        gb[j] = ev ? 0xffu : 0u;
+      }
+    }
+#pragma unroll
+    for (int u = 0; u < ZU; ++u) {
+      const int p = min(t * kTP + zr + (kNT / CA) * u, M - 1);
+      dyv[u] = *reinterpret_cast<const uint4*>(a.dy + static_cast<int64_t>(p) * P + 8 * cz);
+      zv[u] = *reinterpret_cast<const uint4*>(a.z + static_cast<int64_t>(p) * P + 8 * cz);
+    }
+  };
+  uint4 gc[XU];
+  uint32_t gcb[XU];
+  auto stage = [&](int t) {
+#pragma unroll
+    for (int j = 0; j < XU; ++j) {
+      const int row = xr + (kNT / 32) * j;
+      *reinterpret_cast<uint4*>(ximg + img_off<XROWB>(row, cx)) =
+          keep_if(t * kTP + row < M, xv[j]);
+      if constexpr (LK != LK_NONE) {
+        gc[j] = gv[j];
+        gcb[j] = gb[j];
+      }
+    }
+    uint32_t o4[ZU][4];
+#pragma unroll
+    for (int q = 0; q < 4; ++q) {
+      const float2 sc = *reinterpret_cast<const float2*>(cst + 8 * cz + 2 * q);
+      const float2 bi = *reinterpret_cast<const float2*>(cst + P + 8 * cz + 2 * q);
+      const float2 mu = *reinterpret_cast<const float2*>(cst + 2 * P + 8 * cz + 2 * q);
+      const float2 is = *reinterpret_cast<const float2*>(cst + 3 * P + 8 * cz + 2 * q);
+      const float2 ca = *reinterpret_cast<const float2*>(cst + 4 * P + 8 * cz + 2 * q);
+      const float2 cb = *reinterpret_cast<const float2*>(cst + 5 * P + 8 * cz + 2 * q);
+#pragma unroll
+      for (int u = 0; u < ZU; ++u) {
+        const uint32_t dw = q == 0 ? dyv[u].x : q == 1 ? dyv[u].y : q == 2 ? dyv[u].z : dyv[u].w;
+        const uint32_t zw = q == 0 ? zv[u].x : q == 1 ? zv[u].y : q == 2 ? zv[u].z : zv[u].w;
+        const float d0 = __uint_as_float(dw << 16), d1 = __uint_as_float(dw & 0xffff0000u);
+        const float z0 = __uint_as_float(zw << 16), z1 = __uint_as_float(zw & 0xffff0000u);
+        const float o0 =
+            bn_bwd_elem(bn_relu_keep(d0, z0, sc.x, bi.x), z0, mu.x, is.x, sc.x, ca.x, cb.x);
+        const float o1 =
+            bn_bwd_elem(bn_relu_keep(d1, z1, sc.y, bi.y), z1, mu.y, is.y, sc.y, ca.y, cb.y);
+        o4[u][q] = pk_bf16(o0, o1);
+      }
+    }
+#pragma unroll
+    for (int u = 0; u < ZU; ++u) {
+      const int row = zr + (kNT / CA) * u;
+      const bool live = t * kTP + row < M;
+      const uint4 v = keep_if(live, make_uint4(o4[u][0], o4[u][1], o4[u][2], o4[u][3]));
+      *reinterpret_cast<uint4*>(zimg + img_off<ZROWB>(row, cz)) = v;
+      if (a.dz != nullptr && live && slice == 0)
+        *reinterpret_cast<uint4*>(a.dz + static_cast<int64_t>(t * kTP + row) * P + 8 * cz) = v;
+    }
+  };
+
+  f32x16 accw[P / 32] = {};
+  if (t_lo < t_hi) fetch(t_lo);
+  for (int t = t_lo; t < t_hi; ++t) {
+    stage(t);
+    fetch(t + 1 < t_hi ? t + 1 : t);
+    __syncthreads();
+#pragma unroll
+    for (int ks = 0; ks < kTP / 16; ++ks) {
+      const bf16x8_t B = frag32<XROWB>(ximg, 4 * cw, ks, lane);
+#pragma unroll
+      for (int i = 0; i < P / 32; ++i)
+        accw[i] = mfma(frag32<ZROWB>(zimg, 4 * i, ks, lane), B, accw[i]);
+    }
+#pragma unroll
+    for (int ph = 0; ph < kTP / 32; ++ph) {
+      f32x16 accx = {};
+#pragma unroll
+      for (int ks = 0; ks < P / 16; ++ks) {
+        const bf16x8_t B = *reinterpret_cast<const bf16x8_t*>(
+            zimg + img_off<ZROWB>(32 * ph + r, 2 * ks + h));
+        accx = mfma(wf[ks], B, accx);
+      }
+#pragma unroll
+      for (int g = 0; g < 4; ++g)
+        *reinterpret_cast<uint2*>(oimg + img_off<XROWB>(32 * ph + r, 4 * cw + g) + 8 * h) =
+            make_uint2(pk_bf16(accx[4 * g], accx[4 * g + 1]),
+                       pk_bf16(accx[4 * g + 2], accx[4 * g + 3]));
+    }
+    __syncthreads();
+#pragma unroll
+    for (int j = 0; j < XU; ++j) {
+      const int row = xr + (kNT / 32) * j;
+      uint4 v = *reinterpret_cast<const uint4*>(oimg + img_off<XROWB>(row, cx));
+      if constexpr (LK != LK_NONE) v = add_link8(v, gc[j], gcb[j]);
+      const int p = t * kTP + row;
+      if (p < M)
+        *reinterpret_cast<uint4*>(a.dx + static_cast<int64_t>(p) * Cin + cin0 + 8 * cx) = v;
+    }
+  }
+  float* pw = a.part + static_cast<int64_t>(range) * P * Cin + cin0 + 32 * cw + r;
+#pragma unroll
+  for (int i = 0; i < P / 32; ++i)
+#pragma unroll
+    for (int k = 0; k < 16; ++k)
+      pw[static_cast<int64_t>(32 * i + (k & 3) + 8 * (k >> 2) + 4 * h) * Cin] = accw[i][k];
+}
+
+template <int P, int LK>
+hipError_t launch_k(const C1BArgs& a, int S, hipStream_t st) {
+  constexpr int LDS = 2 * kTP * 2 * kSL + kTP * 2 * P + 6 * P * 4;
+  const hipError_t e =
+      hipFuncSetAttribute(reinterpret_cast<const void*>(&conv1_bwd_kernel<P, LK>),
+                          hipFuncAttributeMaxDynamicSharedMemorySize, LDS);
+  if (e != hipSuccess) return e;
+  conv1_bwd_kernel<P, LK><<<S * a.slices, kNT, LDS, st>>>(a);
+  return hipGetLastError();
+}
+
+template <int P>
+hipError_t launch_p(const C1BArgs& a, int kind, int S, hipStream_t st) {
+  if (kind == LK_MASK) return launch_k<P, LK_MASK>(a, S, st);
+  if (kind == LK_S2) return launch_k<P, LK_S2>(a, S, st);
+  return launch_k<P, LK_NONE>(a, S, st);
+}
+
+}
+
+bool conv1_bwd_plan(int64_t M, int p, int Cin, int* splits, int want) {
+  if ((p != 64 && p != 128) || (Cin != 256 && Cin != 512)) return false;
+  if (M < 1 || M >= (1ll << 31) - 2 * kTP || want < 0 || want > 4096) return false;
+  const int slices = Cin / kSL;
+  const int ntile = static_cast<int>((M + kTP - 1) / kTP);
+  int S = want ? want : 256 / slices;
+  const int tpw = (ntile + S - 1) / S;
+  if (!want) S = (ntile + tpw - 1) / tpw;
+  if (slices == 2) S = (S + 7) / 8 * 8;
+  *splits = S;
+  return true;
+}
+
+hipError_t launch_conv1_bwd(const void* dy, const void* z, const void* gamma, const void* beta,
+                            const float* mean, const float* invstd, const float* sdz,
+                            const float* sdzx, const void* x, const void* w, const void* link,
+                            const uint8_t* lmask, int link_kind, int Nimg, int H, int W, void* dx,
+                            float* part, int splits, void* dw, bool dw_bf16, void* dz_out,
+                            int64_t M, int p, int Cin, hipStream_t st) {
+  int S;
+  if (!conv1_bwd_plan(M, p, Cin, &S, 0) || splits < 1 || splits > 4096)
+    return hipErrorInvalidValue;
+  const int slices = Cin / kSL;
+  if (slices == 2 && splits % 8) return hipErrorInvalidValue;
+  if (!dy || !z || !gamma || !beta || !mean || !invstd || !sdz || !sdzx || !x || !w || !dx ||
+      !part || !dw)
+    return hipErrorInvalidValue;
+  if (link_kind < LK_NONE || link_kind > LK_S2 || (link_kind != LK_NONE && !link) ||
+      (link_kind == LK_MASK) != (lmask != nullptr))
+    return hipErrorInvalidValue;
+  if (link_kind == LK_S2 && (Nimg < 1 || H < 1 || W < 1 || static_cast<int64_t>(Nimg) * H * W != M))
+    return hipErrorInvalidValue;
+  for (const void* q : {dy, z, x, link, static_cast<const void*>(dx),
+                        static_cast<const void*>(dz_out)})
+    if (reinterpret_cast<uintptr_t>(q) % 16) return hipErrorInvalidValue;
+  C1BArgs a{};
+  a.dy = reinterpret_cast<const uint16_t*>(dy);
+  a.z = reinterpret_cast<const uint16_t*>(z);
+  a.x = reinterpret_cast<const uint16_t*>(x);
+  a.w = reinterpret_cast<const uint16_t*>(w);
+  a.g = reinterpret_cast<const uint16_t*>(link);
+  a.gm = lmask;
+  a.gamma = reinterpret_cast<const uint16_t*>(gamma);
+  a.beta = reinterpret_cast<const uint16_t*>(beta);
+  a.mean = mean;
+  a.invstd = invstd;
+  a.sdz = sdz;
+  a.sdzx = sdzx;
+  a.dx = reinterpret_cast<uint16_t*>(dx);
+  a.dz = reinterpret_cast<uint16_t*>(dz_out);
+  a.part = part;
+  a.M = static_cast<int>(M);
+  a.Cin = Cin;
+  a.slices = slices;
+  const int ntile = static_cast<int>((M + kTP - 1) / kTP);
+  a.tpw = (ntile + splits - 1) / splits;
+  if (link_kind == LK_S2) {
+    a.W = W;
+    a.HW = H * W;
+    a.OW = (W + 1) / 2;
+    a.OHW = ((H + 1) / 2) * a.OW;
+  }
+  const hipError_t e =
+      p == 64 ? launch_p<64>(a, link_kind, splits, st) : launch_p<128>(a, link_kind, splits, st);
+  if (e != hipSuccess) return e;
+  return launch_wgrad_fold(part, splits, static_cast<int64_t>(p) * Cin, dw, dw_bf16, st);
+}
+
+}
diff --git a/csrc/kernels/kernels.h b/csrc/kernels/kernels.h
--- a/csrc/kernels/kernels.h
+++ b/csrc/kernels/kernels.h
@@ -280,6 +280,14 @@
                    const float* pro_bi, int dmode, const float* dz_a, const float* dz_b,
                    bool dw_bf16);
 
+bool conv1_bwd_plan(int64_t M, int p, int Cin, int* splits, int want = 0);
+hipError_t launch_conv1_bwd(const void* dy, const void* z, const void* gamma, const void* beta,
+                            const float* mean, const float* invstd, const float* sdz,
+                            const float* sdzx, const void* x, const void* w, const void* link,
+                            const uint8_t* lmask, int link_kind, int Nimg, int H, int W, void* dx,
+                            float* part, int splits, void* dw, bool dw_bf16, void* dz_out,
+                            int64_t M, int p, int Cin, hipStream_t st);
+
 bool wgrad3x3s2_plan(int N, int H, int W, int Co, int Ci, int* splits, int taps = 9);
 hipError_t launch_wgrad3x3s2(const void* dy, const void* x, const void* zero, float* part,
                              void* dw, bool dw_bf16, int N, int H, int W, int Co, int Ci,
```

Result: faster. 18510 (median of 6 runs) (+4.4%).
